# Nicholasli1995/SNVC

Measured on AMD Instinct MI355X. Metric: stereo-pairs/sec (cost-volume build + 3D CNN fwd), higher is better.
Workload: dtype f32 (split f16x3 operands, fp32 accumulate)

## Files before the change

snvc_amd/csrc/conv3d_f16.hip:

```cpp
#include <type_traits>

#include "common.hpp"
#include "elementwise_internal.hpp"
#include "snvc_fused.h"
#include "snvc_dedup.h"

namespace snvc {
namespace {

typedef _Float16 h8 __attribute__((ext_vector_type(8)));
typedef float f32x16 __attribute__((ext_vector_type(16)));
typedef float f32x4 __attribute__((ext_vector_type(4)));

__device__ const unsigned g_zero16h[4] __attribute__((aligned(16))) = {0u, 0u, 0u, 0u};

struct F16Args {
    const _Float16 *x;
    const _Float16 *wp;
    const float *scale, *bias;
    const _Float16 *res;
    _Float16 *y;
    float *y_f32;
    const _Float16 *x_lo, *res_lo;
    _Float16 *y_lo;
    const float *head;
    float *y_head;
    float head_mul;
    float res_mul;
    int *overflow;
    const _Float16 *tail_w;
    float *t_out;
    float tail_mul;
    int64_t t_bs;
    const float *res_f32;
    double *stats;
    const float *x_mul;
    int CGin;
    int Cout;
    int Din, Hin, Win;
    int Dout, Hout, Wout;
    int nd, nh, nw;
    int osd, osh, osw, offd, offh, offw;
    int pad_d, pad_h, pad_w;
    int isd, ish, iod, ioh;
    int tiles_d, tiles_h, tiles_w;
    int nchunks, flags;
    int N, cls_mode;
    int64_t cls_wstride;
    int64_t x_bs, y_bs, r_bs, yf_bs;
};

template <class I>
__host__ __device__ __forceinline__ I il_index(int mode, I oc, I C, I H, I pitch, I lp, I cls0, I h, I x) {
    const I cls = mode ? oc % 3 : oc / C, co = mode ? oc / 3 : oc % C, groups = (C + 7) / 8;
    return ((((cls0 + cls) * groups + (co >> 3)) * H + h) * pitch + lp + x) * 8 + (co & 7);
}

struct F16IlArgs : F16Args {
    float *y_il;
    int64_t il_bs;
    int il_mode, il_C, il_pitch, il_lp, il_cls0;
};

struct F16SrcArgs : F16Args {
    const float *gi;
    const float *p_il;
    const float *v_scale, *v_bias;
    int64_t gi_bs;
    int v_pitch, v_lp, v_q, v_m0, v_off, v_off2, v_flags;
};
constexpr int SRC_DEDUP = 1 << 30;

__host__ __device__ __forceinline__ bool wedge_tile_pure(int D, int W, int q, int m0, int off, int d0, int w0) {
    return d0 >= 2 && d0 + 3 <= D - 3 && w0 + 32 < W - 1 && q * (w0 + 32) - (d0 - 1) - m0 + off < 0;
}
__host__ __device__ __forceinline__ bool wedge_tile_duplicate(int D, int W, int q, int m0, int off, int d0, int w0) {
    return wedge_tile_pure(D, W, q, m0, off, d0, w0) && wedge_tile_pure(D, W, q, m0, off, d0 - 4, w0);
}


template <int KD_, int KH_, int KW_, int STRIDE_, int DIL_, int MI_, int TD_, int TH_, int KCG_, int MODE_, bool DB_, int OCC_,
          int DILW_ = DIL_, int PL_ = 1, bool DYN_ = false>
struct F16Cfg {
    static constexpr bool DYN = DYN_;
    static constexpr int PL = PL_;
    static constexpr bool SPLIT = PL_ >= 2, SERIAL = PL_ == 3;
    static constexpr int RES_PL = PL_ == 2 ? 2 : 1;
    static constexpr int PASSES = SERIAL ? 2 : 1;
    static constexpr int PF = DYN_ ? 2 : (SPLIT ? 3 : 6);
    static constexpr int KD = KD_, KH = KH_, KW = KW_, STRIDE = STRIDE_, DIL = DIL_, DILW = DILW_, MI = MI_, TD = TD_, TH = TH_;
    static constexpr int KCG = KCG_, MODE = MODE_, OCC = OCC_;
    static constexpr bool DB = DB_;
    static constexpr int IN_D = (TD - 1) * STRIDE + (KD - 1) * DIL + 1;
    static constexpr int IN_H = (TH - 1) * STRIDE + (KH - 1) * DIL + 1;
    static constexpr int IN_W = 31 * STRIDE + (KW - 1) * DILW + 1;
    static constexpr int VOX = IN_D * IN_H * IN_W;
    static constexpr int GB = VOX * 16;
    static constexpr int ITEMS = RES_PL * KCG * VOX;
    static constexpr int PLANE_BYTES = KCG * GB;
    static constexpr int NIT = (ITEMS + 255) / 256;
    static constexpr int IMG_BYTES = NIT * 256 * 16;
    static constexpr int LDS_BYTES = IMG_BYTES * (DB ? 2 : 1);
    static constexpr int NB = TD * TH / 4;
    static constexpr bool UNROLL_D = KD <= 3;
    static constexpr int SEGS = UNROLL_D ? 1 : KD;
    static constexpr int TSEG = UNROLL_D ? KD * KH * KW : KH * KW;
    static constexpr int NPS = (TSEG + 1) / 2;
    static constexpr int NS = MODE == 0 ? TSEG * (KCG / 2) : NPS * KCG;
    static constexpr int STEPS = SEGS * NS;
    static constexpr int SEG_BYTES = DIL * IN_H * IN_W * 16;
    static_assert(TD * TH % 4 == 0, "rows split over 4 waves");
    static_assert(MODE == 1 || KCG % 2 == 0, "MODE 0 pairs channel groups");
    static_assert(NIT <= 32, "validity mask is one register");
    static_assert((TD * TH / 4) * 4 == TD * TH, "whole rows per wave");
    static constexpr int tapoff(int t) {
        const int kd = UNROLL_D ? t / (KH * KW) : 0, kh = (t / KW) % KH, kw = t % KW;
        return ((kd * DIL) * IN_H + kh * DIL) * IN_W + kw * DILW;
    }
};

__host__ __device__ constexpr int f16_row_channel(int i) { return 16 * ((i >> 2) & 1) + 4 * (i >> 3) + (i & 3); }

__device__ __forceinline__ int xcd_remap16(int b, int n) {
    const int q = n >> 3, r = n & 7, xcd = b & 7, k = b >> 3;
    const int base = xcd < r ? xcd * (q + 1) : r * (q + 1) + (xcd - r) * q;
    return base + k;
}

template <class Cfg, int EPI>
__global__ void __launch_bounds__(256, Cfg::OCC)
conv3d_f16_kernel(const F16Args a_) {
    F16Args a = a_;
    int cls = blockIdx.z / a.N;
    int tile_raw = blockIdx.x, tiles_launch = a.tiles_d * a.tiles_h * a.tiles_w;
    if (a.cls_mode == 1) {
        tiles_launch *= 2;
        tile_raw = xcd_remap16(blockIdx.x, tiles_launch);
        cls = (cls << 1) | (tile_raw & 1);
        tile_raw >>= 1;
        a.offd = (cls >> 2) & 1; a.offh = (cls >> 1) & 1; a.offw = cls & 1;
        a.wp += cls * a.cls_wstride;
    } else if (a.cls_mode == 2) {
        const int pd = (cls >> 1) & 1, ph = cls & 1;
        a.offd = a.iod = pd; a.offh = a.ioh = ph;
        a.nd = (a.Dout - pd + 1) / 2; a.nh = (a.Hout - ph + 1) / 2;
    }
    constexpr int S = Cfg::STRIDE, MI = Cfg::MI, TD = Cfg::TD, TH = Cfg::TH, NB = Cfg::NB, KCG = Cfg::KCG;
    constexpr int IN_H = Cfg::IN_H, IN_W = Cfg::IN_W, VOX = Cfg::VOX, GB = Cfg::GB, NIT = Cfg::NIT, ITEMS = Cfg::ITEMS;
    constexpr int PF = Cfg::PF, PL = Cfg::PL;
    constexpr bool SPLIT = Cfg::SPLIT, SERIAL = Cfg::SERIAL;
    extern __shared__ __attribute__((aligned(16))) char lds[];

    const int tid = threadIdx.x, lane = tid & 63, wave = tid >> 6, half = lane >> 5;
    const int ntiles = a.tiles_d * a.tiles_h * a.tiles_w;
    const int t = a.cls_mode == 1 ? tile_raw : xcd_remap16(blockIdx.x, ntiles);
    const int tw = t % a.tiles_w, th = (t / a.tiles_w) % a.tiles_h, td = t / (a.tiles_w * a.tiles_h);
    const int cb = blockIdx.y;
    const int64_t n = blockIdx.z % a.N;
    const int od0 = td * TD, oh0 = th * TH, ow0 = tw * 32;
    if (od0 >= a.nd || oh0 >= a.nh) return;
    const int id0 = od0 * S - a.pad_d, ih0 = oh0 * S - a.pad_h, iw0 = ow0 * S - a.pad_w;

    f32x16 acc[NB][MI];
#pragma unroll
    for (int nb = 0; nb < NB; ++nb)
#pragma unroll
        for (int m = 0; m < MI; ++m)
#pragma unroll
            for (int r = 0; r < 16; ++r) acc[nb][m][r] = 0.0f;

    const int in_hw = a.Hin * a.Win, in_dhw = in_hw * a.Din;
    unsigned off[NIT];
    unsigned vmask = 0, gmask = 0, pmask = 0;
#pragma unroll
    for (int it = 0; it < NIT; ++it) {
        const int i = it * 256 + tid;
        const int pg = i / VOX, r = i - pg * VOX;
        const int plane = pg / KCG, g = pg - plane * KCG;
        gmask |= (unsigned)(g & 1) << it;
        pmask |= (unsigned)(plane & 1) << it;
        const int dd = r / (IN_H * IN_W), r2 = r - dd * (IN_H * IN_W);
        const int hh = r2 / IN_W, ww = r2 - hh * IN_W;
        const int gd = (id0 + dd) * a.isd + a.iod, gh = (ih0 + hh) * a.ish + a.ioh, gw = iw0 + ww;
        const bool ok = i < ITEMS && (unsigned)gd < (unsigned)a.Din && (unsigned)gh < (unsigned)a.Hin &&
                        (unsigned)gw < (unsigned)a.Win;
        off[it] = ok ? (unsigned)(g * in_dhw + gd * in_hw + gh * a.Win + gw) : 0u;
        vmask |= (ok ? 1u : 0u) << it;
    }
    static_assert(KCG <= 2, "gmask holds one bit per piece");
    const _Float16 *xn = a.x + n * a.x_bs, *xn_lo = SPLIT ? a.x_lo + n * a.x_bs : nullptr;
    const int wbase = tid & ~63;
    auto issue = [&](int pass, int buf) {
        const int chunk = SERIAL ? pass >> 1 : pass;
        const bool lo_pass = SERIAL && (pass & 1);
        const int64_t coff = (int64_t)chunk * KCG * in_dhw * 8;
        const int cg_left = a.CGin - chunk * KCG;
        char *const ibuf = lds + buf * Cfg::IMG_BYTES;
#pragma unroll
        for (int it = 0; it < NIT; ++it) {
            const int i = it * 256 + tid;
            const bool ok = ((vmask >> it) & 1u) && (KCG == 1 || (int)((gmask >> it) & 1u) < cg_left);
            const _Float16 *xc = (((PL == 2 && ((pmask >> it) & 1u)) || lo_pass) ? xn_lo : xn) + coff;
            const void *src = ok ? static_cast<const void *>(xc + (size_t)off[it] * 8) : static_cast<const void *>(g_zero16h);
            if (ITEMS % 256 == 0 || i < ITEMS)
                __builtin_amdgcn_global_load_lds(static_cast<const float *>(src),
                                                 reinterpret_cast<float *>(ibuf + (it * 256 + wbase) * 16), 16, 0, 0);
        }
    };

    const int lanebase = (lane & 31) * S * 16;
    int rowoff[NB];
#pragma unroll
    for (int nb = 0; nb < NB; ++nb) {
        const int row = wave * NB + nb;
        rowoff[nb] = ((row / TH) * S * IN_H + (row % TH) * S) * IN_W * 16;
    }
    constexpr int D_SAME = Cfg::DILW;
    constexpr int D_ROW = Cfg::DIL * IN_W - (Cfg::KW - 1) * Cfg::DILW;
    constexpr int D_SLICE = Cfg::DIL * IN_H * IN_W - (Cfg::KH - 1) * Cfg::DIL * IN_W - (Cfg::KW - 1) * Cfg::DILW;
    const int b_grp = lanebase + half * GB;
    const int b_same = lanebase + half * D_SAME * 16;
    const int b_row = lanebase + half * D_ROW * 16;
    const int b_slice = lanebase + half * D_SLICE * 16;
    const int b_none = lanebase;

    constexpr int MA = MI * (SPLIT ? 2 : 1);
    int dyn_np = 0, dyn_toff[4] = {0, 0, 0, 0}, dyn_base[4] = {0, 0, 0, 0};
    if constexpr (Cfg::DYN) {
        const int nw = 1 + (cls & 1), nh = 1 + ((cls >> 1) & 1), ndp = 1 + ((cls >> 2) & 1);
        const int T = nw * nh * ndp;
        dyn_np = T > 1 ? T / 2 : 1;
// ... 882 lines not shown
        const bool ok = i < ITEMS && (unsigned)gh < (unsigned)a.Hin && (unsigned)gw < (unsigned)a.Win;
        off[it] = ok ? (unsigned)(gh * a.Win + gw) : 0u;
        vmask |= (ok ? 1u : 0u) << it;
    }
    const _Float16 *xn = a.x + n * a.x_bs, *xn_lo = a.x_lo + n * a.x_bs;
    const int wbase = tid & ~63;
    auto issue = [&](int chunk, int buf) {
        const int64_t coff = (int64_t)chunk * in_hw * 8;
        char *const ibuf = lds + buf * Cfg::IMG_BYTES;
#pragma unroll
        for (int it = 0; it < NIT; ++it) {
            const _Float16 *xc = (((pmask >> it) & 1u) ? xn_lo : xn) + coff;
            const void *src = ((vmask >> it) & 1u) ? static_cast<const void *>(xc + (size_t)off[it] * 8) : static_cast<const void *>(g_zero16h);
            __builtin_amdgcn_global_load_lds(static_cast<const float *>(src), reinterpret_cast<float *>(ibuf + (it * 256 + wbase) * 16), 16, 0, 0);
        }
    };
    int qoff[NQ];
#pragma unroll
    for (int q = 0; q < NQ; ++q) {
        int tp = 4 * q + kb;
        tp = tp < Cfg::TAPS ? tp : Cfg::TAPS - 1;
        qoff[q] = ((tp / Cfg::KW) * IN_W + tp % Cfg::KW + col) * 16;
    }
    int rowoff[NB];
#pragma unroll
    for (int nb = 0; nb < NB; ++nb) rowoff[nb] = (wave * NB + nb) * IN_W * 16;
    const int64_t steps_total = (int64_t)a.nchunks * NQ;
    const h8 *wq = reinterpret_cast<const h8 *>(a.wp) + ((int64_t)cb * steps_total * 4) * 64 + lane;
    h8 q_[PF][4];
#pragma unroll
    for (int i = 0; i < PF; ++i) {
#pragma unroll
        for (int m = 0; m < 4; ++m) q_[i][m] = wq[m * 64];
        wq += 4 * 64;
    }

    const unsigned lds_base = (unsigned)(uintptr_t)(__attribute__((address_space(3))) char *)lds;
    issue(0, 0);
    __syncthreads();
    for (int chunk = 0; chunk < a.nchunks; ++chunk) {
        const unsigned img = lds_base + (unsigned)((chunk & 1) * Cfg::IMG_BYTES);
        const bool more = chunk + 1 < a.nchunks;
        h8 bfr[2][8];
        auto load_b = [&](int buf, int hs) {
#pragma unroll
            for (int rr = 0; rr < 2; ++rr) {
                const unsigned addr = img + (unsigned)(qoff[hs >> 1] + rowoff[2 * (hs & 1) + rr]);
                lds_read_b128_to<0>(bfr[buf][rr * 4 + 0], addr);
                lds_read_b128_to<Cfg::PLANE_BYTES>(bfr[buf][rr * 4 + 1], addr);
                lds_read_b128_to<256>(bfr[buf][rr * 4 + 2], addr);
                lds_read_b128_to<Cfg::PLANE_BYTES + 256>(bfr[buf][rr * 4 + 3], addr);
            }
        };
        load_b(0, 0);
        h8 af[4];
#pragma unroll
        for (int hs = 0; hs < 2 * NQ; ++hs) {
            const int cur = hs & 1, nx = cur ^ 1;
            if ((hs & 1) == 0) {
                if (hs == 2 * Cfg::FILL_STEP) {
#pragma unroll
                    for (int i = 0; i < PF; ++i) asm volatile("" ::"v"(q_[i][0]), "v"(q_[i][1]), "v"(q_[i][2]), "v"(q_[i][3]));
                    if (more) issue(chunk + 1, (chunk + 1) & 1);
                }
#pragma unroll
                for (int m = 0; m < 4; ++m) af[m] = q_[0][m];
#pragma unroll
                for (int i = 0; i + 1 < PF; ++i)
#pragma unroll
                    for (int m = 0; m < 4; ++m) q_[i][m] = q_[i + 1][m];
#pragma unroll
                for (int m = 0; m < 4; ++m) q_[PF - 1][m] = wq[m * 64];
                wq += 4 * 64;
            }
            if (hs + 1 < 2 * NQ) {
                load_b(nx, hs + 1);
                wait_lgkm_for<8>(bfr[cur]);
            } else {
                wait_lgkm_for<0>(bfr[cur]);
            }
            __builtin_amdgcn_sched_barrier(0);
#pragma unroll
            for (int term = 0; term < 3; ++term)
#pragma unroll
                for (int rr = 0; rr < 2; ++rr)
#pragma unroll
                    for (int ph = 0; ph < 2; ++ph)
#pragma unroll
                        for (int h = 0; h < 2; ++h) {
                            const h8 aw = term == 0 ? af[2 * h + 1] : af[2 * h];
                            const h8 bx = bfr[cur][rr * 4 + ph * 2 + (term == 1 ? 1 : 0)];
                            acc[2 * (hs & 1) + rr][ph][h] =
                                __builtin_amdgcn_mfma_f32_16x16x32_f16(aw, bx, acc[2 * (hs & 1) + rr][ph][h], 0, 0, 0);
                        }
            __builtin_amdgcn_sched_barrier(0);
        }
        __syncthreads();
    }

    const int64_t out_hw = (int64_t)a.Hout * a.Wout;
    const bool relu = (a.flags & SNVC_EPI_RELU) != 0;
    const int c0 = cb * 32 + 8 * kb;
    const float xm = a.x_mul ? a.head_mul / a.x_mul[0] : a.head_mul;
    float sc[8], bi[8];
#pragma unroll
    for (int e = 0; e < 8; ++e) {
        sc[e] = (a.scale ? a.scale[c0 + e] : 1.0f) * xm;
        bi[e] = a.scale ? a.bias[c0 + e] : 0.0f;
    }
    float *yn = a.y_f32 + n * a.yf_bs + (int64_t)c0 * out_hw;
#pragma unroll
    for (int nb = 0; nb < NB; ++nb) {
        const int phh = oh0 + wave * NB + nb;
#pragma unroll
        for (int ph = 0; ph < 2; ++ph) {
            const int pw = ow0 + 16 * ph + col;
            if (phh < a.nh && pw < a.nw) {
                float *yp = yn + (int64_t)phh * a.Wout + pw;
                float v8[8];
#pragma unroll
                for (int e = 0; e < 8; ++e) {
                    float v = __builtin_fmaf(acc[nb][ph][e >> 2][e & 3], sc[e], bi[e]);
                    if (relu) v = __builtin_fmaxf(v, 0.0f);
                    yp[e * out_hw] = v;
                    v8[e] = v;
                }
                if constexpr (IL == 1) {
                    float *il = a.y_il + n * a.il_bs;
                    if (a.il_mode == 0) {
                        float *dst = il + il_index<int>(0, c0, a.il_C, a.Hout, a.il_pitch, a.il_lp, a.il_cls0, phh, pw);
                        *reinterpret_cast<f32x4q *>(dst) = f32x4q{v8[0], v8[1], v8[2], v8[3]};
                        *reinterpret_cast<f32x4q *>(dst + 4) = f32x4q{v8[4], v8[5], v8[6], v8[7]};
                    } else {
#pragma unroll
                        for (int e = 0; e < 8; ++e) il[il_index<int>(1, c0 + e, a.il_C, a.Hout, a.il_pitch, a.il_lp, a.il_cls0, phh, pw)] = v8[e];
                    }
                }
            }
        }
    }
}

struct X3S2Cfg {
    static constexpr int TD = 2, TH = 4, NB = 2, IN_D = 5, IN_H = 9, IN_W = 65, VOX = IN_D * IN_H * IN_W;
    static constexpr int THREADS = 512, NIT = (VOX + THREADS - 1) / THREADS, SLOT_BYTES = NIT * THREADS * 16, LDS_BYTES = 3 * SLOT_BYTES;
    static constexpr int NQ = 7;
};

template <int N>
__device__ __forceinline__ void wait_lgkm_for4(h8 (&b)[4]) {
    asm volatile("s_waitcnt lgkmcnt(%4)" : "+v"(b[0]), "+v"(b[1]), "+v"(b[2]), "+v"(b[3]) : "n"(N) : "memory");
}

__global__ void __launch_bounds__(512, 1)
conv3d_x3s2q_kernel(const F16Args a, const int total_jobs) {
    using Cfg = X3S2Cfg;
    constexpr int NB = Cfg::NB, TH = Cfg::TH, IN_H = Cfg::IN_H, IN_W = Cfg::IN_W, VOX = Cfg::VOX, NIT = Cfg::NIT, NQ = Cfg::NQ;
    extern __shared__ __attribute__((aligned(16))) char lds[];
    const int tid = threadIdx.x, lane = tid & 63, wave = (tid >> 6) & 3, chalf = tid >> 8, kb = lane >> 4, col = lane & 15;
    const int ntiles = a.tiles_d * a.tiles_h * a.tiles_w, cblocks = a.Cout >> 6;
    const int in_hw = a.Hin * a.Win, in_dhw = in_hw * a.Din;
    const int wbase = tid & ~63;

    struct Job { int od0, oh0, ow0, cb; int64_t n; };
    auto decode = [&](int b) {
        const int j = xcd_remap16(b, total_jobs);
        const int cb = j % cblocks, r = j / cblocks, t = r % ntiles;
        Job jb;
        jb.n = r / ntiles; jb.cb = cb;
        const int tw = t % a.tiles_w, th = (t / a.tiles_w) % a.tiles_h, td = t / (a.tiles_w * a.tiles_h);
        jb.od0 = td * Cfg::TD; jb.oh0 = th * TH; jb.ow0 = tw * 32;
        return jb;
    };
    unsigned off[NIT];
    unsigned vmask = 0;
    auto geometry = [&](const Job &jb) {
        const int id0 = 2 * jb.od0 - a.pad_d, ih0 = 2 * jb.oh0 - a.pad_h, iw0 = 2 * jb.ow0 - a.pad_w;
        vmask = 0;
        int tid_ = tid;
        asm volatile("" : "+v"(tid_));
#pragma unroll
        for (int it = 0; it < NIT; ++it) {
            const int i = it * 512 + tid_;
            const int dd = i / (IN_H * IN_W), r2 = i - dd * (IN_H * IN_W);
            const int hh = r2 / IN_W, pp = r2 - hh * IN_W;
            const int blk = pp >> 5, rr_ = pp & 31;
            const int ww = pp == 64 ? 64 : (rr_ < 16 ? 2 * (16 * blk + rr_) : 2 * (16 * blk + rr_ - 16) + 1);
            const int gd = id0 + dd, gh = ih0 + hh, gw = iw0 + ww;
            const bool ok = i < VOX && (unsigned)gd < (unsigned)a.Din && (unsigned)gh < (unsigned)a.Hin && (unsigned)gw < (unsigned)a.Win;
            off[it] = ok ? (unsigned)(gd * in_hw + gh * a.Win + gw) : 0u;
            vmask |= (ok ? 1u : 0u) << it;
        }
    };
    auto issue = [&](int64_t n, int chunk, bool lo_plane, int slot) {
        const _Float16 *xc = (lo_plane ? a.x_lo : a.x) + n * a.x_bs + (int64_t)chunk * in_dhw * 8;
        char *const ibuf = lds + slot * Cfg::SLOT_BYTES;
#pragma unroll
        for (int it = 0; it < NIT; ++it) {
            const void *src = ((vmask >> it) & 1u) ? static_cast<const void *>(xc + (size_t)off[it] * 8) : static_cast<const void *>(g_zero16h);
            __builtin_amdgcn_global_load_lds(static_cast<const float *>(src), reinterpret_cast<float *>(ibuf + (it * 512 + wbase) * 16), 16, 0, 0);
        }
    };
    int qoff[NQ];
#pragma unroll
    for (int q = 0; q < NQ; ++q) {
        int tp = 4 * q + kb;
        tp = tp < 27 ? tp : 26;
        const int kd = tp / 9, kh = (tp / 3) % 3, kw = tp % 3;
        const int pos = kw == 0 ? col : (kw == 1 ? 16 + col : (col == 15 ? 32 : col + 1));
        qoff[q] = ((kd * IN_H + kh) * IN_W + pos) * 16;
    }
    int rowoff[NB];
#pragma unroll
    for (int nb = 0; nb < NB; ++nb) {
        const int row = wave * NB + nb;
        rowoff[nb] = ((2 * (row / TH)) * IN_H + 2 * (row % TH)) * IN_W * 16;
    }
    const h8 *const wall = reinterpret_cast<const h8 *>(a.wp);
    const int64_t wchunk = (int64_t)NQ * 8 * 64;

    int b = blockIdx.x;
    Job cur = decode(b);
    geometry(cur);
    h8 WH[NQ][2], WL[NQ][2];
    {
        const h8 *wc = wall + (int64_t)cur.cb * a.nchunks * wchunk;
#pragma unroll
        for (int q = 0; q < NQ; ++q)
#pragma unroll
            for (int h = 0; h < 2; ++h) {
                WH[q][h] = wc[(q * 8 + (2 * chalf + h) * 2) * 64 + lane];
                WL[q][h] = wc[(q * 8 + (2 * chalf + h) * 2 + 1) * 64 + lane];
            }
    }
    f32x4q acc[NB][2][2];
#pragma unroll
    for (int nb = 0; nb < NB; ++nb)
#pragma unroll
        for (int ph = 0; ph < 2; ++ph)
#pragma unroll
            for (int h = 0; h < 2; ++h) acc[nb][ph][h] = f32x4q{0.0f, 0.0f, 0.0f, 0.0f};

    const unsigned lds_base = (unsigned)(uintptr_t)(__attribute__((address_space(3))) char *)lds;
    int s_hi = 0, s_sp = 2;
    issue(cur.n, 0, false, 0);
    issue(cur.n, 0, true, 1);
    __syncthreads();
    const int gstride = gridDim.x;
    constexpr float kHalfMax = 65504.0f;
    const bool has_aff = a.scale != nullptr;
    float vmax = 0.0f;
    int chunk = 0;
    while (true) {
        const bool last_chunk = chunk + 1 == a.nchunks;
        const bool next_job = last_chunk && b + gstride < total_jobs;
        const bool more = !last_chunk || next_job;
        Job nxt = cur;
        if (next_job) {
            nxt = decode(b + gstride);
            geometry(nxt);
        }
        const int nchunk = last_chunk ? 0 : chunk + 1;
        if (more) issue(nxt.n, nchunk, false, s_sp);
        h8 bfr[2][4];
        auto load_b = [&](int buf, unsigned img, int q) {
#pragma unroll
            for (int rr = 0; rr < 2; ++rr) {
                const unsigned addr = img + (unsigned)(qoff[q] + rowoff[rr]);
                lds_read_b128_to<0>(bfr[buf][rr * 2 + 0], addr);
                lds_read_b128_to<512>(bfr[buf][rr * 2 + 1], addr);
            }
        };
        {
            const unsigned img = lds_base + (unsigned)Cfg::SLOT_BYTES;
            load_b(0, img, 0);
#pragma unroll
            for (int q = 0; q < NQ; ++q) {
                const int cb_ = q & 1, nx = cb_ ^ 1;
                if (q + 1 < NQ) {
                    load_b(nx, img, q + 1);
                    wait_lgkm_for4<4>(bfr[cb_]);
                } else {
                    wait_lgkm_for4<0>(bfr[cb_]);
                }
                __builtin_amdgcn_sched_barrier(0);
#pragma unroll
                for (int rr = 0; rr < 2; ++rr)
#pragma unroll
                    for (int ph = 0; ph < 2; ++ph)
#pragma unroll
                        for (int h = 0; h < 2; ++h)
                            acc[rr][ph][h] = __builtin_amdgcn_mfma_f32_16x16x32_f16(WH[q][h], bfr[cb_][rr * 2 + ph], acc[rr][ph][h], 0, 0, 0);
                __builtin_amdgcn_sched_barrier(0);
            }
        }
        asm volatile("s_waitcnt lgkmcnt(0)\n\ts_barrier" ::: "memory");
        if (more) issue(nxt.n, nchunk, true, 1);
        {
            const h8 *wn = wall + ((int64_t)nxt.cb * a.nchunks + nchunk) * wchunk;
            const unsigned img = lds_base + (unsigned)(s_hi * Cfg::SLOT_BYTES);
            load_b(0, img, 0);
#pragma unroll
            for (int q = 0; q < NQ; ++q) {
                const int cb_ = q & 1, nx = cb_ ^ 1;
                if (q + 1 < NQ) {
                    load_b(nx, img, q + 1);
                    wait_lgkm_for4<4>(bfr[cb_]);
                } else {
                    wait_lgkm_for4<0>(bfr[cb_]);
                }
                __builtin_amdgcn_sched_barrier(0);
#pragma unroll
                for (int term = 0; term < 2; ++term)
#pragma unroll
                    for (int rr = 0; rr < 2; ++rr)
#pragma unroll
                        for (int ph = 0; ph < 2; ++ph)
#pragma unroll
                            for (int h = 0; h < 2; ++h)
                                acc[rr][ph][h] = __builtin_amdgcn_mfma_f32_16x16x32_f16(term == 0 ? WL[q][h] : WH[q][h], bfr[cb_][rr * 2 + ph],
                                                                                        acc[rr][ph][h], 0, 0, 0);
                __builtin_amdgcn_sched_barrier(0);
                if (more) {
#pragma unroll
                    for (int h = 0; h < 2; ++h) {
                        WH[q][h] = wn[(q * 8 + (2 * chalf + h) * 2) * 64 + lane];
                        WL[q][h] = wn[(q * 8 + (2 * chalf + h) * 2 + 1) * 64 + lane];
                    }
                }
            }
        }
        __syncthreads();
        { const int o = s_hi; s_hi = s_sp; s_sp = o; }
        if (!last_chunk) { ++chunk; continue; }

        {
            const int out_hw = a.Hout * a.Wout;
            const int64_t out_dhw = (int64_t)out_hw * a.Dout;
            const bool relu = (a.flags & SNVC_EPI_RELU) != 0;
            const float lo_bound = relu ? 0.0f : -kHalfMax;
            {
                const int bb = chalf;
                const int c0 = cur.cb * 64 + bb * 32 + 8 * kb;
// ... 269 lines not shown
                    o[e] = (_Float16)v;
                    if constexpr (SPLIT) ol[e] = (_Float16)(v - (float)o[e]);
                }
                if (ok) {
                    *reinterpret_cast<h8 *>(yn + sp * 8) = o;
                    if constexpr (SPLIT) *reinterpret_cast<h8 *>(yn_lo + sp * 8) = ol;
                }
            }
        }
    }
    if constexpr (SPLIT) {
        if (vmax >= kHalfMax && a.overflow) atomicOr(a.overflow, 1);
    }
}

__global__ void pack_q16s_weights_kernel(const float *__restrict__ w, _Float16 *__restrict__ out, int Cout, int Cin, int K3, int NSEG, int NT,
                                         int NQ, int nchunks, int NH, int NPL, int PASSES, float wmul, int64_t total) {
    const int64_t i = (int64_t)blockIdx.x * blockDim.x + threadIdx.x;
    if (i >= total) return;
    int64_t r = i;
    const int e = (int)(r % 8); r /= 8;
    const int lane = (int)(r % 64); r /= 64;
    const int pl = (int)(r % NPL); r /= NPL;
    const int h = (int)(r % NH); r /= NH;
    const int q = (int)(r % NQ); r /= NQ;
    const int kd = (int)(r % NSEG); r /= NSEG;
    r /= PASSES;
    const int chunk = (int)(r % nchunks); r /= nchunks;
    const int cb = (int)r;
    const int row = lane & 15, kb = lane >> 4;
    const int co = (cb * (NH / 2) + (h >> 1)) * 32 + 8 * (row >> 2) + 4 * (h & 1) + (row & 3);
    const int ci = chunk * 8 + e;
    const int tp = 4 * q + kb;
    float v = 0.0f;
    if (tp < NT && kd * NT + tp < K3 && co < Cout && ci < Cin) v = w[((int64_t)co * Cin + ci) * K3 + kd * NT + tp] * wmul;
    const _Float16 hi = (_Float16)v;
    out[i] = pl == 0 ? hi : (_Float16)(v - (float)hi);
}

struct PackArgs {
    const float *w;
    _Float16 *out;
    int Cout, Cin, K;
    int transposed, pd, ph, pw;
    int KD, KH, KW, KCG, MODE, MI, SEGS, TSEG, NPS, NS, unroll_d;
    int nchunks, cblocks;
    int PL;
    int PASSES;
    int dyn;
    float wmul;
    int64_t total;
};

__global__ void pack_f16_weights_kernel(const PackArgs p) {
    const int64_t i = (int64_t)blockIdx.x * blockDim.x + threadIdx.x;
    if (i >= p.total) return;
    int64_t r = i;
    const int e = (int)(r % 8); r /= 8;
    const int lane = (int)(r % 64); r /= 64;
    const int npl = p.PL >= 2 ? 2 : 1;
    const int pl = (int)(r % npl); r /= npl;
    const int m = (int)(r % p.MI); r /= p.MI;
    const int s = (int)(r % p.NS); r /= p.NS;
    const int seg = (int)(r % p.SEGS); r /= p.SEGS;
    r /= p.PASSES;
    const int chunk = (int)(r % p.nchunks); r /= p.nchunks;
    const int cb = (int)r;
    const int half = lane >> 5;
    const int co = (cb * p.MI + m) * 32 + f16_row_channel(lane & 31);
    int tap, g;
    if (p.dyn) { g = s % p.KCG; tap = 2 * (s / p.KCG) + half; }
    else if (p.MODE == 0) { tap = s / (p.KCG / 2); g = 2 * (s % (p.KCG / 2)) + half; }
    else { g = s / p.NPS; tap = 2 * (s % p.NPS) + half; }
    const int ci = (chunk * p.KCG + g) * 8 + e;
    float v = 0.0f;
    if (p.dyn) {
        const int nw = 1 + p.pw, nh = 1 + p.ph, ndp = 1 + p.pd;
        if (tap < nw * nh * ndp && co < p.Cout && ci < p.Cin) {
            const int b[3] = {tap / (nw * nh), (tap / nw) % nh, tap % nw}, par[3] = {p.pd, p.ph, p.pw};
            int k3[3];
            for (int d = 0; d < 3; ++d) k3[d] = par[d] == 0 ? 1 : (b[d] == 0 ? 2 : 0);
            v = p.w[((((int64_t)ci * p.Cout + co) * 3 + k3[0]) * 3 + k3[1]) * 3 + k3[2]];
        }
    } else if (tap < p.TSEG && co < p.Cout && ci < p.Cin) {
        const int kd = p.unroll_d ? tap / (p.KH * p.KW) : seg, kh = (tap / p.KW) % p.KH, kw = tap % p.KW;
        if (!p.transposed) {
            v = p.w[((((int64_t)co * p.Cin + ci) * p.K + kd) * p.K + kh) * p.K + kw];
        } else {
            const int par[3] = {p.pd, p.ph, p.pw}, b[3] = {kd, kh, kw};
            int k3[3];
            bool ok = true;
            for (int d = 0; d < 3; ++d) {
                if (par[d] == 0) { ok = ok && b[d] == 0; k3[d] = 1; }
                else k3[d] = b[d] == 0 ? 2 : 0;
            }
            if (ok) v = p.w[((((int64_t)ci * p.Cout + co) * 3 + k3[0]) * 3 + k3[1]) * 3 + k3[2]];
        }
    }
    if (p.PL >= 2) {
        v *= p.wmul;
        const _Float16 hi = (_Float16)v;
        p.out[i] = pl ? (_Float16)(v - (float)hi) : hi;
    } else {
        p.out[i] = (_Float16)v;
    }
}

using F16K1   = F16Cfg<1, 1, 1, 1, 1, 2, 4, 4, 2, 0, true, 2>;
using F16K3   = F16Cfg<3, 3, 3, 1, 1, 2, 4, 4, 2, 0, true, 2>;
using F16K3H  = F16Cfg<3, 3, 3, 1, 1, 1, 4, 4, 2, 0, true, 2>;
using F16K3S2 = F16Cfg<3, 3, 3, 2, 1, 2, 2, 4, 1, 1, false, 2>;
using F16K5   = F16Cfg<5, 5, 5, 1, 1, 2, 4, 4, 1, 1, true, 2>;
using F16K5D2 = F16Cfg<5, 5, 5, 1, 1, 2, 4, 4, 1, 1, false, 2, 2>;
using F16K7   = F16Cfg<7, 7, 7, 1, 1, 2, 4, 4, 1, 1, false, 2>;
using F16DC   = F16Cfg<2, 2, 2, 1, 1, 2, 4, 4, 2, 0, true, 2>;
using F16K1N   = F16Cfg<1, 1, 1, 1, 1, 1, 4, 4, 2, 0, true, 2>;
using F16K3S2N = F16Cfg<3, 3, 3, 2, 1, 1, 2, 4, 1, 1, false, 2>;
using F16K5N   = F16Cfg<5, 5, 5, 1, 1, 1, 4, 4, 1, 1, true, 2>;
using F16K5D2N = F16Cfg<5, 5, 5, 1, 1, 1, 4, 4, 1, 1, false, 2, 2>;
using F16K7N   = F16Cfg<7, 7, 7, 1, 1, 1, 4, 4, 1, 1, false, 2>;
using F16DCN   = F16Cfg<2, 2, 2, 1, 1, 1, 4, 4, 2, 0, true, 2>;

using F16K3X  = F16Cfg<3, 3, 3, 1, 1, 1, 4, 4, 1, 1, false, 2, 1, 2>;
using F16K3X2 = F16Cfg<3, 3, 3, 1, 1, 2, 4, 4, 1, 1, false, 2, 1, 2>;
using F16K3XS  = F16Cfg<3, 3, 3, 1, 1, 1, 4, 4, 1, 1, true, 3, 1, 3>;
using F16K3XT  = F16Cfg<3, 3, 3, 1, 1, 1, 2, 4, 1, 1, false, 4, 1, 2>;
using F16K3X2S = F16Cfg<3, 3, 3, 1, 1, 2, 4, 4, 1, 1, true, 2, 1, 3>;
using F16K3S2X = F16Cfg<3, 3, 3, 2, 1, 2, 2, 4, 1, 1, false, 2, 1, 3>;
using F16DCX  = F16Cfg<2, 2, 2, 1, 1, 2, 4, 4, 2, 1, false, 2, 1, 2, true>;
using F16K3S2XT = F16Cfg<3, 3, 3, 2, 1, 2, 1, 4, 1, 1, false, 3, 1, 3>;
using F16DCXT   = F16Cfg<2, 2, 2, 1, 1, 2, 2, 4, 2, 1, false, 3, 1, 2, true>;

using F16K1X   = F16Cfg<1, 1, 1, 1, 1, 1, 4, 4, 2, 0, true, 3, 1, 2>;
using F16K5X   = F16Cfg<5, 5, 5, 1, 1, 1, 4, 4, 1, 1, false, 3, 1, 3>;
using F16K5D2X = F16Cfg<5, 5, 5, 1, 1, 1, 4, 4, 1, 1, false, 2, 2, 3>;
using F16K7X   = F16Cfg<7, 7, 7, 1, 1, 1, 4, 4, 1, 1, false, 2, 1, 3>;
using F16DCXN  = F16Cfg<2, 2, 2, 1, 1, 1, 4, 4, 2, 1, false, 3, 1, 2, true>;

__global__ void pack_tail_weights_kernel(const float *__restrict__ w, _Float16 *__restrict__ out, int Cin, float wmul, int total) {
    const int i = blockIdx.x * blockDim.x + threadIdx.x;
    if (i >= total) return;
    int r = i;
    const int e = r % 8; r /= 8;
    const int lane = r % 64; r /= 64;
    const int pl = r % 2; r /= 2;
    const int j = r % 2; r /= 2;
    const int m = r;
    const int tap = lane & 31, c = 32 * m + 16 * (lane >> 5) + 8 * j + e;
    const float v = (tap < 27 && c < Cin) ? w[c * 27 + tap] * wmul : 0.0f;
    const _Float16 hi = (_Float16)v;
    out[i] = pl == 0 ? hi : (_Float16)(v - (float)hi);
}

__global__ void __launch_bounds__(256)
deconv_tail_gather_kernel(const float *__restrict__ t, const float *__restrict__ bias, const float *__restrict__ res, float *__restrict__ y,
                          int nd, int nh, int nw, int64_t t_bs, int64_t y_bs, int64_t r_bs) {
    const int OD = 4 * nd, OH = 4 * nh;
    const int64_t total = (int64_t)OD * OH * nw;
    const int64_t i = (int64_t)blockIdx.x * 256 + threadIdx.x;
    if (i >= total) return;
    const int j = (int)(i % nw);
    const int64_t r0 = i / nw;
    const int oh = (int)(r0 % OH), od = (int)(r0 / OH);
    const int64_t n = blockIdx.y;
    const int64_t cls_vox = (int64_t)nd * nh * nw, tap_stride = 8 * cls_vox;
    const float *tn = t + n * t_bs;
    const float b = bias ? bias[0] : 0.0f;
    float o0 = b, o1 = b, o2 = b, o3 = b;
    const int ad = od >> 1, ah = oh >> 1;
    const int ndd = (od & 1) ? 2 : 1, nhh = (oh & 1) ? 2 : 1;
    const bool last_w = j + 1 >= nw;
    for (int a_ = 0; a_ < ndd; ++a_) {
        const int kd = (od & 1) ? (a_ ? 0 : 2) : 1, id = ad + a_;
        if (id >= 2 * nd) continue;
        for (int b_ = 0; b_ < nhh; ++b_) {
            const int kh = (oh & 1) ? (b_ ? 0 : 2) : 1, ih = ah + b_;
            if (ih >= 2 * nh) continue;
            const int cdh = ((id & 1) << 2) | ((ih & 1) << 1);
            const int64_t base = ((int64_t)(id >> 1) * nh + (ih >> 1)) * nw + j;
            const float *t0 = tn + (int64_t)((kd * 3 + kh) * 3) * tap_stride + base;
            const float *c0 = t0 + (int64_t)cdh * cls_vox, *c1 = t0 + (int64_t)(cdh | 1) * cls_vox;
            o0 += c0[tap_stride];
            o1 += c0[2 * tap_stride] + c1[0];
            o2 += c1[tap_stride];
            o3 += c1[2 * tap_stride] + (last_w ? 0.0f : c0[1]);
        }
    }
    const int64_t sp = ((int64_t)od * OH + oh) * (4 * nw) + 4 * j;
    if (res) {
        const f32x4 rv = *reinterpret_cast<const f32x4 *>(res + n * r_bs + sp);
        o0 += rv[0]; o1 += rv[1]; o2 += rv[2]; o3 += rv[3];
    }
    *reinterpret_cast<f32x4 *>(y + n * y_bs + sp) = f32x4{o0, o1, o2, o3};
}

__global__ void __launch_bounds__(256)
split_scale_kernel(const float *__restrict__ x, int64_t n, unsigned *__restrict__ scratch, float *__restrict__ out) {
    float m = 0.0f;
    const int64_t stride = (int64_t)gridDim.x * 256 * 4;
    const int64_t n4 = n & ~(int64_t)3;
    auto amax4 = [](const f32x4 v) {
        return __builtin_fmaxf(__builtin_fmaxf(__builtin_fabsf(v[0]), __builtin_fabsf(v[1])), __builtin_fmaxf(__builtin_fabsf(v[2]), __builtin_fabsf(v[3])));
    };
    int64_t i = ((int64_t)blockIdx.x * 256 + threadIdx.x) * 4;
    for (; i + 3 * stride < n4; i += 4 * stride) {
        const f32x4 v0 = *reinterpret_cast<const f32x4 *>(x + i), v1 = *reinterpret_cast<const f32x4 *>(x + i + stride);
        const f32x4 v2 = *reinterpret_cast<const f32x4 *>(x + i + 2 * stride), v3 = *reinterpret_cast<const f32x4 *>(x + i + 3 * stride);
        m = __builtin_fmaxf(m, __builtin_fmaxf(__builtin_fmaxf(amax4(v0), amax4(v1)), __builtin_fmaxf(amax4(v2), amax4(v3))));
    }
    for (; i < n4; i += stride) m = __builtin_fmaxf(m, amax4(*reinterpret_cast<const f32x4 *>(x + i)));
    if (blockIdx.x == 0 && threadIdx.x < (int)(n - n4)) m = __builtin_fmaxf(m, __builtin_fabsf(x[n4 + threadIdx.x]));
#pragma unroll
    for (int o = 32; o > 0; o >>= 1) m = __builtin_fmaxf(m, __shfl_xor(m, o, 64));
    __shared__ float part[4];
    if ((threadIdx.x & 63) == 0) part[threadIdx.x >> 6] = m;
    __syncthreads();
    if (threadIdx.x == 0) {
        m = __builtin_fmaxf(__builtin_fmaxf(part[0], part[1]), __builtin_fmaxf(part[2], part[3]));
        atomicMax(scratch, __builtin_bit_cast(unsigned, m));
        __threadfence();
        if (atomicAdd(scratch + 1, 1u) == gridDim.x - 1) {
            const float amax = __builtin_bit_cast(float, atomicExch(scratch, 0u));
            atomicExch(scratch + 1, 0u);
            float e = floorf(log2f(16384.0f / amax));
            e = (e == e && __builtin_fabsf(e) < 3.0e38f) ? __builtin_fminf(__builtin_fmaxf(e, -24.0f), 40.0f) : 0.0f;
            out[0] = exp2f(e);
        }
    }
}

struct F16Geom {
    int classes;
    int64_t ntiles;
    int64_t jobs;
    int64_t stats_slots;
    dim3 grid;
};
using F16Launch = void (*)(const F16Args &, const F16Geom &, hipStream_t);

enum F16Call { TO_SRC_HEAD, TO_SRC, TO_TAIL, TO_F32, TO_HEAD, TO_C8, TO_PLANE, F16_CALLS };
enum F16Classes { CLS_ONE = 0, CLS_TRANSPOSED = 1, CLS_SUBGRID = 2 };
enum F16Grid { GRID_TILES, GRID_JOBS, GRID_PERSISTENT };

struct Q16Layout { int K3, NSEG, NQ, NH, NPL, PASSES; };

struct F16Form {
    PackArgs pack;
    Q16Layout q16;
    int MI, KCG;
    int chunk_frags;
    int pad_frags;
    int cls_mode, TD, TH, grid;
    bool split_res, stats;
    const char *unsupported;
    F16Launch launch[F16_CALLS];

    constexpr F16Form on(F16Call c, F16Launch l) const { F16Form f = *this; f.launch[c] = l; return f; }
};

template <class Cfg, int EPI>
void launch_f16(const F16Args &a, const F16Geom &g, hipStream_t st) {
    launch_lds<conv3d_f16_kernel<Cfg, EPI>>(g.grid, 256, Cfg::LDS_BYTES, st, a);
}
template <class Cfg>
void launch_q16s(const F16Args &a, const F16Geom &g, hipStream_t st) {
    launch_lds<conv3d_q16s_kernel<Cfg>>(g.grid, 256, Cfg::LDS_BYTES, st, a);
}
template <int EPI>
void launch_x3q(const F16Args &a, const F16Geom &g, hipStream_t st) {
    launch_lds<conv3d_x3q_kernel<EPI>>(g.grid, 256, X3QCfg::LDS_BYTES, st, a);
}
template <int EPI>
void launch_x3q_src(const F16Args &a, const F16Geom &g, hipStream_t st) {
    launch_lds<conv3d_x3q_kernel<EPI, 1>>(g.grid, 256, X3QCfg::LDS_BYTES, st, static_cast<const F16SrcArgs &>(a));
}
struct WedgeRange { int64_t dups; int td0, td1, ntw; };
WedgeRange wedge_ranges(int D, int W, int q, int m0, int off, int64_t *first_td, int64_t *last_td, int max_tw) {
    WedgeRange r{0, -1, -1, 0};
    const int tiles_d = (D + X3QCfg::TD - 1) / X3QCfg::TD, tiles_w = (W + 31) / 32;
    for (int tw = 0; tw < tiles_w; ++tw) {
        int first = -1, last = -1;
        for (int td = 0; td < tiles_d; ++td) {
            if (!wedge_tile_pure(D, W, q, m0, off, td * X3QCfg::TD, tw * 32)) continue;
            if (first < 0) first = td;
            last = td;
        }
        if (last == first) first = last = -1;
        if (tw < max_tw && first_td && last_td) { first_td[tw] = first; last_td[tw] = last; }
        if (first < 0) continue;
        r.dups += last - first;
        r.ntw = tw + 1;
        if (tw == 0) { r.td0 = first + 1; r.td1 = last; }
    }
    return r;
}
void launch_wedge_copy(const F16SrcArgs &a, hipStream_t st) {
    const WedgeRange r = wedge_ranges(a.Din, a.Win, a.v_q, a.v_m0, a.v_off, nullptr, nullptr, 0);
    if (r.dups == 0) return;
    WedgeCopyArgs w{a.y, a.y_lo, a.y_head, a.y_bs, a.Cout / 8, a.Dout, a.Hout, a.Wout, a.v_q, a.v_m0, a.v_off, r.td0, r.ntw};
    wedge_copy_kernel<<<dim3((unsigned)((r.td1 - r.td0 + 1) * r.ntw), (unsigned)a.tiles_h, (unsigned)a.N), 256, 0, st>>>(w);
}

void launch_x3s2q(const F16Args &a, const F16Geom &g, hipStream_t st) {
    int wg = device_cu_count();
    if (wg <= 0) wg = 256;
    if (g.jobs < wg) wg = g.jobs >= 8 ? (int)(g.jobs & ~(int64_t)7) : (int)g.jobs;
    launch_lds<conv3d_x3s2q_kernel>(dim3((unsigned)wg), X3S2Cfg::THREADS, X3S2Cfg::LDS_BYTES, st, a, (int)g.jobs);
}

template <class Cfg, int... EPI>
constexpr F16Form f16_form(int cls_mode, bool stats = false) {
    constexpr F16Call call_of[5] = {TO_C8, TO_PLANE, TO_F32, TO_HEAD, TO_TAIL};
    constexpr int npl = Cfg::PL >= 2 ? 2 : 1;
    F16Form f{};
    f.pack.KD = Cfg::KD; f.pack.KH = Cfg::KH; f.pack.KW = Cfg::KW; f.pack.KCG = Cfg::KCG; f.pack.MODE = Cfg::MODE; f.pack.MI = Cfg::MI;
    f.pack.SEGS = Cfg::SEGS; f.pack.TSEG = Cfg::TSEG; f.pack.NPS = Cfg::NPS; f.pack.NS = Cfg::NS; f.pack.unroll_d = Cfg::UNROLL_D ? 1 : 0;
    f.pack.PL = Cfg::PL; f.pack.PASSES = Cfg::PASSES; f.pack.dyn = Cfg::DYN ? 1 : 0;
    f.MI = Cfg::MI; f.KCG = Cfg::KCG; f.TD = Cfg::TD; f.TH = Cfg::TH;
    f.chunk_frags = Cfg::PASSES * Cfg::STEPS * Cfg::MI * npl;
    f.pad_frags = Cfg::PF * Cfg::MI * npl;
    f.cls_mode = cls_mode; f.grid = GRID_TILES; f.split_res = true; f.stats = stats;
    f.unsupported = Cfg::PL >= 2 ? "snvc_f16x3_conv3d_forward: no kernel" : "snvc_f16_conv3d_forward: no kernel";
    ((f.launch[call_of[EPI]] = launch_f16<Cfg, EPI>), ...);
    return f;
}

constexpr F16Form q16_form(Q16Layout q, int TD, int TH, int pad_steps, int cls_mode, int grid, bool split_res, bool stats, const char *unsupported) {
    F16Form f{};
    f.q16 = q; f.MI = q.NH / 2; f.KCG = 1; f.TD = TD; f.TH = TH;
    f.chunk_frags = q.PASSES * q.NSEG * q.NQ * q.NH * q.NPL;
    f.pad_frags = pad_steps * q.NH * q.NPL;
    f.cls_mode = cls_mode; f.grid = grid; f.split_res = split_res; f.stats = stats; f.unsupported = unsupported;
    return f;
}
template <class C>
constexpr F16Form q16s_form(F16Call c, const char *unsupported) {
    return q16_form({C::K3, C::KSEG, C::NQ, C::NH, C::SPLIT ? 2 : 1, C::PASSES}, C::TD, C::TH, C::PF, C::DILW == 2 ? CLS_SUBGRID : CLS_ONE, GRID_TILES, true,
                    false, unsupported).on(c, launch_q16s<C>);
}

constexpr const char *kQ16C8 = "snvc_f16_conv3d_forward: the 16x16x32 form writes C8 tensors";
constexpr F16Form FORM_K7QN   = q16s_form<Q16SCfg<7, 1, 1, 1>>(TO_C8, kQ16C8);
constexpr F16Form FORM_K5QN   = q16s_form<Q16SCfg<5, 1, 1, 1>>(TO_C8, kQ16C8);
constexpr F16Form FORM_K5D2QN = q16s_form<Q16SCfg<5, 2, 1, 1>>(TO_C8, kQ16C8);
constexpr F16Form FORM_K7Q    = q16s_form<Q16SCfg<7, 1, 1, 2>>(TO_C8, kQ16C8);
constexpr F16Form FORM_K5Q    = q16s_form<Q16SCfg<5, 1, 1, 2>>(TO_C8, kQ16C8);
constexpr F16Form FORM_K5D2Q  = q16s_form<Q16SCfg<5, 2, 1, 2>>(TO_C8, kQ16C8);
constexpr F16Form FORM_K1     = f16_form<F16K1, 0>(CLS_ONE);
constexpr F16Form FORM_K3     = f16_form<F16K3, 0>(CLS_ONE);
constexpr F16Form FORM_K3H    = f16_form<F16K3H, 1>(CLS_ONE);
constexpr F16Form FORM_K3S2   = f16_form<F16K3S2, 0>(CLS_ONE);
constexpr F16Form FORM_K5     = f16_form<F16K5, 0>(CLS_ONE);
constexpr F16Form FORM_K5D2   = f16_form<F16K5D2, 0>(CLS_SUBGRID);
constexpr F16Form FORM_K7     = f16_form<F16K7, 0>(CLS_ONE);
constexpr F16Form FORM_DC     = f16_form<F16DC, 0>(CLS_TRANSPOSED);
constexpr F16Form FORM_K1N    = f16_form<F16K1N, 0>(CLS_ONE);
constexpr F16Form FORM_K3N    = f16_form<F16K3H, 0>(CLS_ONE);
constexpr F16Form FORM_K3S2N  = f16_form<F16K3S2N, 0>(CLS_ONE);
constexpr F16Form FORM_K5N    = f16_form<F16K5N, 0>(CLS_ONE);
constexpr F16Form FORM_K5D2N  = f16_form<F16K5D2N, 0>(CLS_SUBGRID);
constexpr F16Form FORM_K7N    = f16_form<F16K7N, 0>(CLS_ONE);
constexpr F16Form FORM_DCN    = f16_form<F16DCN, 0>(CLS_TRANSPOSED);
constexpr F16Form FORM_K3X    = f16_form<F16K3X, 0, 3, 2>(CLS_ONE, true);
constexpr F16Form FORM_K3X2   = f16_form<F16K3X2, 0, 2>(CLS_ONE, true);
constexpr F16Form FORM_K3XS   = f16_form<F16K3XS, 0, 3, 2>(CLS_ONE, true);
constexpr F16Form FORM_K3X2S  = f16_form<F16K3X2S, 0, 2>(CLS_ONE, true);
constexpr F16Form FORM_K3XT   = f16_form<F16K3XT, 0, 3, 2>(CLS_ONE, true);
constexpr F16Form FORM_K3S2X  = f16_form<F16K3S2X, 0, 2>(CLS_ONE, true);
constexpr F16Form FORM_K3S2XT = f16_form<F16K3S2XT, 0, 2>(CLS_ONE, true);
constexpr F16Form FORM_DCX    = f16_form<F16DCX, 0, 2, 4>(CLS_TRANSPOSED, true);
constexpr F16Form FORM_DCXT   = f16_form<F16DCXT, 0, 2, 4>(CLS_TRANSPOSED, true);
constexpr F16Form FORM_DCXN   = f16_form<F16DCXN, 0, 2, 4>(CLS_TRANSPOSED, true);
constexpr F16Form FORM_K1X    = f16_form<F16K1X, 0, 2>(CLS_ONE);
constexpr F16Form FORM_K5X    = f16_form<F16K5X, 0, 2>(CLS_ONE);
constexpr F16Form FORM_K5D2X  = f16_form<F16K5D2X, 0, 2>(CLS_SUBGRID);
constexpr F16Form FORM_K7X    = f16_form<F16K7X, 0, 2>(CLS_ONE);
constexpr F16Form FORM_K3XH   = f16_form<F16K3X, 1>(CLS_ONE);
constexpr const char *kQ16Split = "snvc_f16x3_conv3d_forward: the 16x16x32 form writes a split C8 tensor, no side head";
constexpr F16Form FORM_K5XQ   = q16s_form<Q16SCfg<5, 1>>(TO_C8, kQ16Split);
constexpr F16Form FORM_K5D2XQ = q16s_form<Q16SCfg<5, 2>>(TO_C8, kQ16Split);
constexpr F16Form FORM_K7XQ   = q16s_form<Q16SCfg<7, 1>>(TO_C8, kQ16Split);
constexpr F16Form FORM_K3S2XQ =
    q16_form({27, 1, X3S2Cfg::NQ, 4, 2, 1}, X3S2Cfg::TD, X3S2Cfg::TH, X3S2Cfg::NQ, CLS_ONE, GRID_PERSISTENT, false, false,
             "snvc_f16x3_conv3d_forward: the stride-2 16x16x32 form writes a split C8 tensor, no residual / head")
        .on(TO_C8, launch_x3s2q);
constexpr F16Form FORM_K3XQ =
    q16_form({27, 1, X3QCfg::NQ, 2, 2, 1}, X3QCfg::TD, X3QCfg::TH, X3QCfg::PF, CLS_ONE, GRID_JOBS, false, true,
             "snvc_f16x3_conv3d_forward: the 16x16x32 form has no split residual, no side head beside a float32 result")
        .on(TO_SRC_HEAD, launch_x3q_src<3>).on(TO_SRC, launch_x3q_src<0>).on(TO_F32, launch_x3q<2>).on(TO_HEAD, launch_x3q<3>).on(TO_C8, launch_x3q<0>);

struct F16Plan {
    const F16Form *form;
    int nchunks, cblocks;
    int64_t block_halves;
    int64_t class_stride() const { return block_halves + (int64_t)form->pad_frags * 64 * 8; }
};

const F16Form *plain_form(int key, int Cout, int algo) {
    const bool narrow = Cout == 32;
    if (algo & SNVC_ALGO_X3_Q16) {
        const bool two = Cout % 64 == 0;
        if (key == 711) return two ? &FORM_K7Q : &FORM_K7QN;
        if (key == 512) return two ? &FORM_K5D2Q : &FORM_K5D2QN;
        if (key == 511) return two ? &FORM_K5Q : &FORM_K5QN;
    }
    switch (key) {
        case 111: return narrow ? &FORM_K1N : &FORM_K1;
        case 311: return narrow ? &FORM_K3N : &FORM_K3;
        case 321: return narrow ? &FORM_K3S2N : &FORM_K3S2;
        case 511: return narrow ? &FORM_K5N : &FORM_K5;
        case 512: return narrow ? &FORM_K5D2N : &FORM_K5D2;
        case 711: return narrow ? &FORM_K7N : &FORM_K7;
        default: return nullptr;
    }
}

const F16Form *split_form(int key, int Cout, int algo) {
    const bool q16 = algo & SNVC_ALGO_X3_Q16;
    switch (key) {
        case 111: return &FORM_K1X;
        case 321: return q16 ? &FORM_K3S2XQ : (algo & SNVC_ALGO_X3_SMALL) ? &FORM_K3S2XT : &FORM_K3S2X;
        case 511: return q16 ? &FORM_K5XQ : &FORM_K5X;
        case 512: return q16 ? &FORM_K5D2XQ : &FORM_K5D2X;
        case 711: return q16 ? &FORM_K7XQ : &FORM_K7X;
        case 311:
            if (q16) return &FORM_K3XQ;
            if (algo & SNVC_ALGO_X3_SMALL) return &FORM_K3XT;
            if (algo & SNVC_ALGO_X3_NARROW) return &FORM_K3X;
            if (algo & SNVC_ALGO_X3_SERIAL) return Cout == 32 ? &FORM_K3XS : &FORM_K3X2S;
            return Cout == 32 ? &FORM_K3X : &FORM_K3X2;
        default: return nullptr;
    }
}

int make_f16_plan(const snvc_conv3d_desc &d, F16Plan &p, bool split = false) {
#define SNVC_F16_WHO(msg) (split ? "snvc_f16x3_conv3d: " msg : "snvc_f16_conv3d: " msg)
    if (d.N < 0 || d.Cin <= 0 || d.Cout <= 0 || d.Din <= 0 || d.Hin <= 0 || d.Win <= 0)
        return fail(SNVC_ERR_INVALID_ARGUMENT, "snvc_f16_conv3d: sizes must be positive");
    if (d.Cin % 8 != 0) return fail(SNVC_ERR_UNSUPPORTED, "snvc_f16_conv3d: Cin must be a multiple of 8 (C8 layout)");
    if (!split && d.Cout != 1 && d.Cout % 32 != 0)
        return fail(SNVC_ERR_UNSUPPORTED, "snvc_f16_conv3d: Cout must be a multiple of 32, or 1 (fp32 plane output)");
    const F16Form *f;
    if (d.transposed) {
        if (d.ksize != 3 || d.stride != 2 || d.pad != 1 || d.dilation != 1 || (split && d.Cout % 32 != 0))
            return fail(SNVC_ERR_UNSUPPORTED, split ? "snvc_f16x3_conv3d: transposed layers: k3,s2,p1,op1 with Cout % 32 == 0"
                                                    : "snvc_f16_conv3d: transposed conv supports k3,s2,p1,op1 only");
        if (d.Dout != 2 * d.Din || d.Hout != 2 * d.Hin || d.Wout != 2 * d.Win)
            return fail(SNVC_ERR_INVALID_ARGUMENT, SNVC_F16_WHO("transposed output must be 2x the input"));
        if (d.Cout == 1) return fail(SNVC_ERR_UNSUPPORTED, "snvc_f16_conv3d: transposed conv to one channel");
        if (split) f = d.Cout % 64 == 0 ? ((d.algo & SNVC_ALGO_X3_SMALL) ? &FORM_DCXT : &FORM_DCX) : &FORM_DCXN;
        else f = d.Cout == 32 ? &FORM_DCN : &FORM_DC;
    } else {
        if (d.pad != d.dilation * (d.ksize - 1) / 2) return fail(SNVC_ERR_UNSUPPORTED, SNVC_F16_WHO("pad must equal dilation*(ksize-1)/2"));
        const int eff = d.dilation * (d.ksize - 1) + 1;
        if (d.Dout != (d.Din + 2 * d.pad - eff) / d.stride + 1 || d.Hout != (d.Hin + 2 * d.pad - eff) / d.stride + 1 ||
            d.Wout != (d.Win + 2 * d.pad - eff) / d.stride + 1)
            return fail(SNVC_ERR_INVALID_ARGUMENT, SNVC_F16_WHO("output size does not match the convolution arithmetic"));
        const int key = d.ksize * 100 + d.stride * 10 + d.dilation;
        if (d.Cout == 1) {
            if (key != 311) return fail(SNVC_ERR_UNSUPPORTED, SNVC_F16_WHO("one-channel output is built for k3/s1 only"));
// ... 33 lines not shown
        a.osd = a.osh = a.osw = 1;
        a.pad_d = a.pad_h = a.pad_w = d.pad;
    }
    a.tiles_d = ceil_div(a.nd, f.TD); a.tiles_h = ceil_div(a.nh, f.TH); a.tiles_w = ceil_div(a.nw, 32);
    F16Geom g{};
    g.classes = transposed ? 8 : (subgrid ? 4 : 1);
    g.ntiles = (int64_t)a.tiles_d * a.tiles_h * a.tiles_w;
    const int64_t gx = transposed ? 2 * g.ntiles : g.ntiles, gz = transposed ? 4 : g.classes;
    g.grid = dim3((unsigned)gx, (unsigned)p.cblocks, (unsigned)(d.N * gz));
    g.stats_slots = gz * gx * 4;
    if (f.grid == GRID_JOBS) {
        g.jobs = g.ntiles * p.cblocks;
        g.grid = dim3((unsigned)g.jobs, 1, (unsigned)d.N);
        g.stats_slots = g.ntiles * 4;
    } else if (f.grid == GRID_PERSISTENT) {
        g.jobs = g.ntiles * p.cblocks * d.N;
    }
    return g;
}

void pack_q16(const Q16Layout &q, const float *w, void *packed, int Cout, int Cin, float wmul, int64_t total, hipStream_t st) {
    pack_q16s_weights_kernel<<<(unsigned)ceil_div<int64_t>(total, 256), 256, 0, st>>>(w, reinterpret_cast<_Float16 *>(packed), Cout, Cin, q.K3, q.NSEG, 4 * q.NQ,
                                                                                    q.NQ, Cin / 8, q.NH, q.NPL, q.PASSES, wmul, total);
}

}
}

extern "C" {

static int64_t f16_packed_bytes(const snvc_conv3d_desc *d, bool split) {
    snvc::F16Plan p;
    if (!d || snvc::make_f16_plan(*d, p, split) != SNVC_OK) return -1;
    return 2 * p.class_stride() * (d->transposed ? 8 : 1);
}

int64_t snvc_f16_conv3d_packed_weight_bytes(const snvc_conv3d_desc *d) { return f16_packed_bytes(d, false); }
int64_t snvc_f16x3_conv3d_packed_weight_bytes(const snvc_conv3d_desc *d) { return f16_packed_bytes(d, true); }

static int f16_pack_common(const snvc_conv3d_desc *d, const float *weight, void *packed, bool split, float wmul, void *stream,
                           const char *who) {
    using namespace snvc;
    F16Plan p;
    if (!d) return fail(SNVC_ERR_INVALID_ARGUMENT, "snvc_f16_conv3d_pack_weights: null desc");
    int rc = make_f16_plan(*d, p, split);
    if (rc) return rc;
    if (!weight || !packed) return fail(SNVC_ERR_INVALID_ARGUMENT, "snvc_f16_conv3d_pack_weights: null pointer");
    const F16Form &f = *p.form;
    const int classes = d->transposed ? 8 : 1;
    if (hipMemsetAsync(packed, 0, (size_t)(2 * p.class_stride() * classes), as_stream(stream)) != hipSuccess)
        return fail(SNVC_ERR_HIP, "snvc_f16_conv3d_pack_weights: hipMemsetAsync failed");
    if (f.q16.NQ) {
        pack_q16(f.q16, weight, packed, d->Cout, d->Cin, wmul, p.block_halves, as_stream(stream));
        return check_launch(who);
    }
    for (int c = 0; c < classes; ++c) {
        PackArgs a = f.pack;
        a.w = weight;
        a.out = reinterpret_cast<_Float16 *>(packed) + c * p.class_stride();
        a.Cout = d->Cout; a.Cin = d->Cin; a.K = d->ksize;
        a.transposed = d->transposed; a.pd = (c >> 2) & 1; a.ph = (c >> 1) & 1; a.pw = c & 1;
        a.nchunks = p.nchunks; a.cblocks = p.cblocks; a.total = p.block_halves;
        a.wmul = wmul;
        if (a.dyn) {
            const int T = (1 + a.pd) * (1 + a.ph) * (1 + a.pw);
            a.NS = 2 * (T > 1 ? T / 2 : 1);
            a.total = (int64_t)p.cblocks * p.nchunks * a.NS * a.MI * 2 * 64 * 8;
        }
        pack_f16_weights_kernel<<<(unsigned)ceil_div<int64_t>(a.total, 256), 256, 0, as_stream(stream)>>>(a);
    }
    return check_launch(who);
}

int snvc_f16_conv3d_pack_weights(const snvc_conv3d_desc *d, const float *weight, void *packed, void *stream) {
    return f16_pack_common(d, weight, packed, false, 1.0f, stream, "snvc_f16_conv3d_pack_weights");
}

int snvc_f16x3_conv3d_pack_weights(const snvc_conv3d_desc *d, const float *weight, void *packed, float wmul, void *stream) {
    return f16_pack_common(d, weight, packed, true, wmul, stream, "snvc_f16x3_conv3d_pack_weights");
}

int snvc_f16_conv3d_forward(const snvc_conv3d_desc *d, const void *x, const void *packed_weight, const float *scale,
                            const float *bias, const void *residual, void *y, float *y_f32, void *stream) {
    using namespace snvc;
    F16Plan p;
    if (!d) return fail(SNVC_ERR_INVALID_ARGUMENT, "snvc_f16_conv3d_forward: null desc");
    int rc = make_f16_plan(*d, p);
    if (rc) return rc;
    if (d->N == 0) return SNVC_OK;
    const bool plane = d->Cout == 1;
    if (!x || !packed_weight || (plane ? !y_f32 : !y))
        return fail(SNVC_ERR_INVALID_ARGUMENT, "snvc_f16_conv3d_forward: null pointer");
    if ((scale == nullptr) != (bias == nullptr))
        return fail(SNVC_ERR_INVALID_ARGUMENT, "snvc_f16_conv3d_forward: scale and bias must both be given or both be NULL");
    const int resflags = d->flags & (SNVC_EPI_ADD_PRE | SNVC_EPI_ADD_POST);
    if (resflags && (!residual || plane))
        return fail(SNVC_ERR_INVALID_ARGUMENT, "snvc_f16_conv3d_forward: residual flag without a C8 residual");
    if (resflags == (SNVC_EPI_ADD_PRE | SNVC_EPI_ADD_POST))
        return fail(SNVC_ERR_INVALID_ARGUMENT, "snvc_f16_conv3d_forward: ADD_PRE and ADD_POST are exclusive");
    if (!plane && (d->flags & SNVC_EPI_SIGMOID))
        return fail(SNVC_ERR_UNSUPPORTED, "snvc_f16_conv3d_forward: Sigmoid is built for the one-channel fp32 output only");
    const int64_t in_sp = (int64_t)d->Din * d->Hin * d->Win, out_sp = (int64_t)d->Dout * d->Hout * d->Wout;
    if ((int64_t)(d->Cin / 8 + 2) * in_sp >= ((int64_t)1 << 31) || out_sp >= ((int64_t)1 << 31))
        return fail(SNVC_ERR_UNSUPPORTED, "snvc_f16_conv3d_forward: one sample must stay below 2^31 pieces");
    if ((reinterpret_cast<uintptr_t>(x) | reinterpret_cast<uintptr_t>(y) | reinterpret_cast<uintptr_t>(residual) |
         reinterpret_cast<uintptr_t>(packed_weight)) & 15)
        return fail(SNVC_ERR_INVALID_ARGUMENT, "snvc_f16_conv3d_forward: C8 tensors must be 16-byte aligned");
    if ((d->x_batch_stride | d->y_batch_stride | d->res_batch_stride) % 8)
        return fail(SNVC_ERR_INVALID_ARGUMENT, "snvc_f16_conv3d_forward: batch strides must be multiples of 8 elements");

    F16Args a{};
    a.x = reinterpret_cast<const _Float16 *>(x);
    a.wp = reinterpret_cast<const _Float16 *>(packed_weight);
    a.scale = scale; a.bias = bias;
    a.res = resflags ? reinterpret_cast<const _Float16 *>(residual) : nullptr;
    a.y = reinterpret_cast<_Float16 *>(y); a.y_f32 = y_f32;
    a.res_mul = 1.0f;
    a.CGin = d->Cin / 8;
    a.Cout = d->Cout;
    a.Din = d->Din; a.Hin = d->Hin; a.Win = d->Win;
    a.Dout = d->Dout; a.Hout = d->Hout; a.Wout = d->Wout;
    a.nchunks = p.nchunks; a.flags = d->flags;
    a.x_bs = d->x_batch_stride ? d->x_batch_stride : (int64_t)d->Cin * in_sp;
    a.y_bs = d->y_batch_stride ? d->y_batch_stride : (int64_t)d->Cout * out_sp;
    a.r_bs = d->res_batch_stride ? d->res_batch_stride : (int64_t)d->Cout * out_sp;
    a.yf_bs = out_sp;
    const F16Geom g = f16_geometry(*d, p, a);
    if (g.ntiles >= ((int64_t)1 << 30) || (int64_t)d->N * g.classes > 65535)
        return fail(SNVC_ERR_UNSUPPORTED, "snvc_f16_conv3d_forward: too many tiles or samples");
    const F16Launch launch = p.form->launch[plane ? TO_PLANE : TO_C8];
    if (!launch) return fail(SNVC_ERR_UNSUPPORTED, p.form->unsupported);
    launch(a, g, as_stream(stream));
    return check_launch("snvc_f16_conv3d_forward");
}

struct F16x3Call {
    const void *x_hi = nullptr, *x_lo = nullptr, *packed_weight = nullptr;
    const float *scale = nullptr, *bias = nullptr;
    const void *res_hi = nullptr, *res_lo = nullptr;
    const float *res_f32 = nullptr;
    void *y_hi = nullptr, *y_lo = nullptr;
    float *y_f32 = nullptr;
    const float *head = nullptr;
    float *y_head = nullptr;
    float head_mul = 0.0f, res_mul = 0.0f;
    int *overflow = nullptr;
    const void *tail_w = nullptr;
    float *t_out = nullptr;
    float tail_mul = 0.0f;
    double *stats = nullptr;
    int64_t *stats_slots = nullptr;
    const float *x_mul = nullptr;
    const snvc::F16SrcArgs *src = nullptr;
    void *stream = nullptr;
};

static int f16x3_forward(const snvc_conv3d_desc *d, const F16x3Call &c) {
    using namespace snvc;
    F16Plan p;
    if (!d) return fail(SNVC_ERR_INVALID_ARGUMENT, "snvc_f16x3_conv3d_forward: null desc");
    int rc = make_f16_plan(*d, p, true);
    if (rc) return rc;
    if (d->N == 0) return SNVC_OK;
    const F16Form &f = *p.form;
    const bool tail = c.tail_w != nullptr;
    if (tail && (!c.t_out || !f.launch[TO_TAIL] || p.cblocks != 1 || d->Cout != 32 * f.MI || (reinterpret_cast<uintptr_t>(c.tail_w) & 15)))
        return fail(SNVC_ERR_UNSUPPORTED, "snvc_f16x3_deconv3d_tail_forward: a transposed split layer whose 32 or 64 output channels sit in one block");
    const bool plane = d->Cout == 1;
    const bool to_f32 = c.y_f32 != nullptr;
    if (plane && !to_f32) return fail(SNVC_ERR_INVALID_ARGUMENT, "snvc_f16x3_conv3d_forward: a one-channel layer writes y_f32");
    if ((!c.src && (!c.x_hi || !c.x_lo)) || !c.packed_weight || (!tail && !to_f32 && (!c.y_hi || !c.y_lo)))
        return fail(SNVC_ERR_INVALID_ARGUMENT, "snvc_f16x3_conv3d_forward: null pointer");
    if ((c.scale == nullptr) != (c.bias == nullptr))
        return fail(SNVC_ERR_INVALID_ARGUMENT, "snvc_f16x3_conv3d_forward: scale and bias must both be given or both be NULL");
    const int flags = c.res_f32 ? (d->flags & ~SNVC_EPI_ADD_POST) : d->flags;
    const int resflags = flags & (SNVC_EPI_ADD_PRE | SNVC_EPI_ADD_POST);
    if (c.res_f32 && !plane && d->res_batch_stride && d->res_batch_stride != (d->y_batch_stride ? d->y_batch_stride : (int64_t)d->Cout * d->Dout * d->Hout * d->Wout))
        return fail(SNVC_ERR_INVALID_ARGUMENT, "snvc_f16x3_conv3d_forward: a float32 residual shares the result's batch stride");
    if ((resflags && (!c.res_hi || !c.res_lo)) || ((resflags || c.res_f32) && plane))
        return fail(SNVC_ERR_INVALID_ARGUMENT, "snvc_f16x3_conv3d_forward: residual flag without a split residual");
    if (resflags == (SNVC_EPI_ADD_PRE | SNVC_EPI_ADD_POST))
        return fail(SNVC_ERR_INVALID_ARGUMENT, "snvc_f16x3_conv3d_forward: ADD_PRE and ADD_POST are exclusive");
    if (d->flags & ~(SNVC_EPI_RELU | SNVC_EPI_ADD_PRE | SNVC_EPI_ADD_POST | (plane ? SNVC_EPI_SIGMOID : 0)))
        return fail(SNVC_ERR_UNSUPPORTED, "snvc_f16x3_conv3d_forward: RELU / ADD_PRE / ADD_POST only (SIGMOID with the one-channel output)");
    if ((c.head != nullptr) != (c.y_head != nullptr))
        return fail(SNVC_ERR_INVALID_ARGUMENT, "snvc_f16x3_conv3d_forward: head and y_head go together");
    if (c.head && (!f.launch[TO_HEAD] || d->Cout != 32 || to_f32))
        return fail(SNVC_ERR_UNSUPPORTED, "snvc_f16x3_conv3d_forward: the side head is built for 32-channel stride-1 layers with a split output");
    const int64_t in_sp = (int64_t)d->Din * d->Hin * d->Win, out_sp = (int64_t)d->Dout * d->Hout * d->Wout;
    if ((int64_t)(d->Cin / 8 + 2) * in_sp >= ((int64_t)1 << 31) || out_sp >= ((int64_t)1 << 31))
        return fail(SNVC_ERR_UNSUPPORTED, "snvc_f16x3_conv3d_forward: one sample must stay below 2^31 pieces");
    if ((reinterpret_cast<uintptr_t>(c.x_hi) | reinterpret_cast<uintptr_t>(c.x_lo) | reinterpret_cast<uintptr_t>(c.y_hi) |
         reinterpret_cast<uintptr_t>(c.y_lo) | reinterpret_cast<uintptr_t>(c.res_hi) | reinterpret_cast<uintptr_t>(c.res_lo) |
         reinterpret_cast<uintptr_t>(c.packed_weight) | reinterpret_cast<uintptr_t>(c.scale) | reinterpret_cast<uintptr_t>(c.bias) |
         reinterpret_cast<uintptr_t>(c.head)) & 15)
        return fail(SNVC_ERR_INVALID_ARGUMENT, "snvc_f16x3_conv3d_forward: C8 tensors and the per-channel vectors must be 16-byte aligned");
    if ((d->x_batch_stride | (c.res_f32 ? 0 : d->res_batch_stride)) % 8 || (!to_f32 && d->y_batch_stride % 8))
        return fail(SNVC_ERR_INVALID_ARGUMENT, "snvc_f16x3_conv3d_forward: batch strides must be multiples of 8 elements");
    F16SrcArgs b{};
    if (c.src) b = *c.src;
    F16Args &a = b;
    a = F16Args{};
    a.x = reinterpret_cast<const _Float16 *>(c.x_hi); a.x_lo = reinterpret_cast<const _Float16 *>(c.x_lo);
    a.wp = reinterpret_cast<const _Float16 *>(c.packed_weight);
    a.scale = c.scale; a.bias = c.bias;
    a.res = resflags ? reinterpret_cast<const _Float16 *>(c.res_hi) : nullptr;
    a.res_lo = resflags ? reinterpret_cast<const _Float16 *>(c.res_lo) : nullptr;
    a.y = reinterpret_cast<_Float16 *>(c.y_hi); a.y_lo = reinterpret_cast<_Float16 *>(c.y_lo); a.y_f32 = c.y_f32;
    a.head = c.head; a.y_head = c.y_head; a.head_mul = c.head_mul; a.res_mul = c.res_mul; a.overflow = c.overflow;
    a.res_f32 = c.res_f32;
    a.stats = c.stats;
    a.x_mul = to_f32 ? c.x_mul : nullptr;
    a.tail_w = reinterpret_cast<const _Float16 *>(c.tail_w); a.t_out = c.t_out; a.tail_mul = c.tail_mul;
    a.t_bs = (int64_t)27 * 8 * d->Din * d->Hin * d->Win;
    a.CGin = d->Cin / 8; a.Cout = d->Cout;
    a.Din = d->Din; a.Hin = d->Hin; a.Win = d->Win;
    a.Dout = d->Dout; a.Hout = d->Hout; a.Wout = d->Wout;
    a.nchunks = p.nchunks; a.flags = flags;
    a.x_bs = d->x_batch_stride ? d->x_batch_stride : 2 * (int64_t)d->Cin * in_sp;
    a.y_bs = d->y_batch_stride ? d->y_batch_stride : 2 * (int64_t)d->Cout * out_sp;
    a.r_bs = d->res_batch_stride ? d->res_batch_stride : 2 * (int64_t)d->Cout * out_sp;
    a.yf_bs = plane ? out_sp : (d->y_batch_stride ? d->y_batch_stride : (int64_t)d->Cout * out_sp);
    const F16Geom g = f16_geometry(*d, p, a);
    if (g.ntiles >= ((int64_t)1 << 30) || (int64_t)d->N * g.classes > 65535)
        return fail(SNVC_ERR_UNSUPPORTED, "snvc_f16x3_conv3d_forward: too many tiles or samples");
    hipStream_t st = as_stream(c.stream);
    if (c.stats_slots) {
        if (!(to_f32 && !plane && !tail && f.stats))
            return fail(SNVC_ERR_UNSUPPORTED, "snvc_f16x3_conv3d_forward_stats: this layer's kernel form has no statistics epilogue");
        *c.stats_slots = g.stats_slots;
        if (!c.stats) return fail(SNVC_ERR_INVALID_ARGUMENT, "snvc_f16x3_conv3d_forward_stats: null workspace");
        if (g.classes > 1) {
            const hipError_t e = hipMemsetAsync(c.stats, 0, (size_t)d->N * g.stats_slots * ((d->Cout + 31) / 32) * 64 * sizeof(double), st);
            if (e != hipSuccess) return fail(SNVC_ERR_HIP, "snvc_f16x3_conv3d_forward_stats: hipMemsetAsync failed");
        }
    }
    if (c.src && !f.launch[TO_SRC])
        return fail(SNVC_ERR_UNSUPPORTED, "snvc_fused_first_conv3d_forward: a 3x3x3 stride-1 layer on the 16x16x32 form (SNVC_ALGO_X3_Q16)");
    const F16Call call = tail ? TO_TAIL : plane ? TO_PLANE : to_f32 ? TO_F32 : c.head ? (c.src ? TO_SRC_HEAD : TO_HEAD) : (c.src ? TO_SRC : TO_C8);
    if (!f.launch[call] || (resflags && !f.split_res)) return fail(SNVC_ERR_UNSUPPORTED, f.unsupported);
    if (g.jobs >= ((int64_t)1 << 30)) return fail(SNVC_ERR_UNSUPPORTED, "snvc_f16x3_conv3d_forward: too many tiles");
    if (c.src && to_f32) return fail(SNVC_ERR_UNSUPPORTED, "snvc_fused_first_conv3d_forward: a split C8 output");
    if ((b.v_flags & SRC_DEDUP) && ((c.y_head && (d->Wout % 4 || (reinterpret_cast<uintptr_t>(c.y_head) & 15))) ||
                                    wedge_ranges(a.Din, a.Win, b.v_q, b.v_m0, b.v_off, nullptr, nullptr, 0).dups == 0))
        b.v_flags &= ~SRC_DEDUP;
    f.launch[call](b, g, st);
    if (b.v_flags & SRC_DEDUP) launch_wedge_copy(b, st);
    return check_launch("snvc_f16x3_conv3d_forward");
}

int snvc_f16x3_conv3d_forward(const snvc_conv3d_desc *d, const void *x_hi, const void *x_lo, const void *packed_weight,
                              const float *scale, const float *bias, const void *res_hi, const void *res_lo, void *y_hi,
                              void *y_lo, float *y_f32, const float *head, float *y_head, float head_mul, float res_mul,
                              int *overflow, void *stream) {
    F16x3Call c;
    c.x_hi = x_hi; c.x_lo = x_lo; c.packed_weight = packed_weight; c.scale = scale; c.bias = bias;
    c.res_hi = res_hi; c.res_lo = res_lo; c.y_hi = y_hi; c.y_lo = y_lo; c.y_f32 = y_f32;
    c.head = head; c.y_head = y_head; c.head_mul = head_mul; c.res_mul = res_mul; c.overflow = overflow; c.stream = stream;
    if (d && (d->flags & (SNVC_EPI_ADD_PRE | SNVC_EPI_ADD_POST)) == SNVC_EPI_ADD_POST && y_f32 && d->Cout != 1 && res_hi && !res_lo) {
        c.res_f32 = static_cast<const float *>(res_hi);
        c.res_hi = nullptr;
    }
    return f16x3_forward(d, c);
}

static int fused_first_forward(const snvc_conv3d_desc *d, const void *packed_weight, const float *scale, const float *bias, void *y_hi,
                               void *y_lo, const float *head, float *y_head, float head_mul, int *overflow, const float *gi,
                               int64_t pitch, int64_t lp, const float *p_il, const float *v_scale, const float *v_bias, int q, int m0,
                               int off, int off2, int v_flags, bool dedup, void *stream) {
    using namespace snvc;
    if (!d || !gi || !p_il || !v_scale || !v_bias) return fail(SNVC_ERR_INVALID_ARGUMENT, "snvc_fused_first_conv3d_forward: null pointer");
    if (d->transposed || d->ksize != 3 || d->stride != 1 || d->pad != 1 || d->dilation != 1 || d->Cin % 8 || d->Din < 1 || d->Hin < 1 || d->Win < 1 ||
        (q != 1 && q != 2) || (v_flags & ~SNVC_EPI_RELU))
        return fail(SNVC_ERR_UNSUPPORTED, "snvc_fused_first_conv3d_forward: a 3x3x3 / stride 1 / pad 1 layer, Cin % 8 == 0, q = 1 | 2");
    if ((reinterpret_cast<uintptr_t>(gi) | reinterpret_cast<uintptr_t>(p_il) | reinterpret_cast<uintptr_t>(v_scale) | reinterpret_cast<uintptr_t>(v_bias)) & 31)
        return fail(SNVC_ERR_INVALID_ARGUMENT, "snvc_fused_first_conv3d_forward: gi / p_il / v_scale / v_bias must be 32-byte aligned");
    const int64_t D = d->Din, H = d->Hin, W = d->Win, CG = d->Cin / 8;
    const int64_t lo_g = -(D - 1) - m0 + off, hi_g = (int64_t)q * (W - 2) - m0 + off;
    const int64_t lo_c = (int64_t)q * (W - 1) - (D - 1) - m0 + off2, hi_c = (int64_t)q * (W - 1) - m0 + off2;
    if (lp < 0 || pitch <= 0 || lp + lo_c < 0 || lp + hi_c >= pitch || (W > 1 && (lp + lo_g < 0 || lp + hi_g >= pitch)))
        return fail(SNVC_ERR_INVALID_ARGUMENT, "snvc_fused_first_conv3d_forward: pitch / lp do not cover the G indices of this shape");
    if (6 * CG * H * pitch * 32 >= ((int64_t)1 << 31) || 3 * CG * H * W * 32 >= ((int64_t)1 << 31))
        return fail(SNVC_ERR_UNSUPPORTED, "snvc_fused_first_conv3d_forward: one sample of gi / p_il must stay below 2 GiB");
    F16SrcArgs s{};
    s.gi = gi; s.p_il = p_il; s.v_scale = v_scale; s.v_bias = v_bias; s.gi_bs = 6 * CG * H * pitch * 8;
    s.v_pitch = (int)pitch; s.v_lp = (int)lp; s.v_q = q; s.v_m0 = m0; s.v_off = off; s.v_off2 = off2;
    s.v_flags = v_flags | (dedup ? SRC_DEDUP : 0);
    F16x3Call c;
    c.packed_weight = packed_weight; c.scale = scale; c.bias = bias; c.y_hi = y_hi; c.y_lo = y_lo;
    c.head = head; c.y_head = y_head; c.head_mul = head_mul; c.res_mul = 1.0f; c.overflow = overflow; c.src = &s; c.stream = stream;
    return f16x3_forward(d, c);
}

int snvc_fused_first_conv3d_forward(const snvc_conv3d_desc *d, const void *packed_weight, const float *scale, const float *bias, void *y_hi,
                                    void *y_lo, const float *head, float *y_head, float head_mul, int *overflow, const float *gi,
                                    int64_t pitch, int64_t lp, const float *p_il, const float *v_scale, const float *v_bias, int q, int m0,
                                    int off, int off2, int v_flags, void *stream) {
    return fused_first_forward(d, packed_weight, scale, bias, y_hi, y_lo, head, y_head, head_mul, overflow, gi, pitch, lp, p_il, v_scale, v_bias,
                               q, m0, off, off2, v_flags, false, stream);
}

int snvc_dedup_abi_version(void) { return 1; }

int snvc_dedup_fused_first_conv3d_forward(const snvc_conv3d_desc *d, const void *packed_weight, const float *scale, const float *bias,
                                          void *y_hi, void *y_lo, const float *head, float *y_head, float head_mul, int *overflow,
                                          const float *gi, int64_t pitch, int64_t lp, const float *p_il, const float *v_scale,
                                          const float *v_bias, int q, int m0, int off, int off2, int v_flags, void *stream) {
    return fused_first_forward(d, packed_weight, scale, bias, y_hi, y_lo, head, y_head, head_mul, overflow, gi, pitch, lp, p_il, v_scale, v_bias,
                               q, m0, off, off2, v_flags, true, stream);
}

int64_t snvc_dedup_fused_first_tiles(const snvc_conv3d_desc *d, int q, int m0, int off, int64_t *first_td, int64_t *last_td, int max_tw) {
    using namespace snvc;
    if (!d || d->Din < 1 || d->Win < 1 || (q != 1 && q != 2) || max_tw < 0 || (max_tw > 0 && (!first_td || !last_td))) {
        fail(SNVC_ERR_INVALID_ARGUMENT, "snvc_dedup_fused_first_tiles: a desc, q = 1 | 2, and max_tw entries to write");
        return -1;
    }
    for (int tw = 0; tw < max_tw; ++tw) first_td[tw] = last_td[tw] = -1;
    return wedge_ranges((int)d->Din, (int)d->Win, q, m0, off, first_td, last_td, max_tw).dups;
}

int64_t snvc_f16x3_conv3d_stats_workspace_bytes(const snvc_conv3d_desc *d) {
    using namespace snvc;
    F16Plan p;
    if (!d || d->N < 0 || make_f16_plan(*d, p, true)) return -1;
    const int64_t groups = (d->Cout + 31) / 32;
    F16Args a{};
    const int64_t slots = f16_geometry(*d, p, a).stats_slots;
    return (d->N * slots * groups * 64 + conv_stats_fold_scratch_doubles(d->N, (int)groups, slots) + d->N * (int64_t)d->Cout * 2) * (int64_t)sizeof(double);
}

int snvc_f16x3_conv3d_forward_f32(const snvc_conv3d_desc *d, const void *x_hi, const void *x_lo, const void *packed_weight,
                                  const float *scale, const float *bias, const float *x_mul, const float *res_f32, float *y_f32,
                                  float out_mul, void *stream) {
    using namespace snvc;
    if (!d || !y_f32) return fail(SNVC_ERR_INVALID_ARGUMENT, "snvc_f16x3_conv3d_forward_f32: null pointer");
    if (d->flags & (SNVC_EPI_ADD_PRE | SNVC_EPI_ADD_POST)) return fail(SNVC_ERR_INVALID_ARGUMENT, "snvc_f16x3_conv3d_forward_f32: the residual is res_f32 (added after the activation), no flag");
    F16x3Call c;
    c.x_hi = x_hi; c.x_lo = x_lo; c.packed_weight = packed_weight; c.scale = scale; c.bias = bias; c.x_mul = x_mul;
    c.res_f32 = res_f32; c.y_f32 = y_f32; c.head_mul = out_mul; c.res_mul = 1.0f; c.stream = stream;
    return f16x3_forward(d, c);
}

int snvc_f16x3_conv3d_forward_stats(const snvc_conv3d_desc *d, const void *x_hi, const void *x_lo, const void *packed_weight,
                                    const float *scale, const float *bias, const float *x_mul, float *y_f32, float head_mul, const float *gamma,
                                    const float *beta, float *bn_scale, float *bn_shift, float *mean, float *var, void *workspace,
                                    float eps, void *stream) {
    using namespace snvc;
    if (!d || !y_f32 || !bn_scale || !bn_shift || !workspace)
        return fail(SNVC_ERR_INVALID_ARGUMENT, "snvc_f16x3_conv3d_forward_stats: null pointer");
    if (d->N <= 0 || d->flags || d->Cout % 32) return fail(SNVC_ERR_UNSUPPORTED, "snvc_f16x3_conv3d_forward_stats: whole 32-channel groups, no epilogue flags");
    double *stats = static_cast<double *>(workspace);
    int64_t slots = 0;
    F16x3Call c;
    c.x_hi = x_hi; c.x_lo = x_lo; c.packed_weight = packed_weight; c.scale = scale; c.bias = bias; c.x_mul = x_mul;
    c.y_f32 = y_f32; c.head_mul = head_mul; c.res_mul = 1.0f; c.stats = stats; c.stats_slots = &slots; c.stream = stream;
    int rc = f16x3_forward(d, c);
    if (rc) return rc;
    const int groups = d->Cout / 32;
    double *scratch = stats + d->N * slots * groups * 64;
    double *partial = scratch + conv_stats_fold_scratch_doubles(d->N, groups, slots);
    launch_conv_stats_fold(stats, scratch, partial, d->N, d->Cout, groups, slots, as_stream(stream));
    rc = check_launch("snvc_f16x3_conv3d_forward_stats(fold)");
    if (rc) return rc;
    launch_norm_finalize(partial, gamma, beta, bn_scale, bn_shift, mean, var, d->N, d->Cout, (int64_t)d->Dout * d->Hout * d->Wout, 1, eps,
                         as_stream(stream));
    return check_launch("snvc_f16x3_conv3d_forward_stats(finalize)");
}

int snvc_f16x3_split_scale(const float *x, int64_t n, void *scratch8, float *out_mul, void *stream) {
    using namespace snvc;
    if (n < 0) return fail(SNVC_ERR_INVALID_ARGUMENT, "snvc_f16x3_split_scale: negative size");
    if (!out_mul || !scratch8 || (n > 0 && !x)) return fail(SNVC_ERR_INVALID_ARGUMENT, "snvc_f16x3_split_scale: null pointer");
    if (reinterpret_cast<uintptr_t>(x) & 15) return fail(SNVC_ERR_INVALID_ARGUMENT, "snvc_f16x3_split_scale: x must be 16-byte aligned");
    int blocks = (int)ceil_div<int64_t>(n > 0 ? n : 1, 256 * 4 * 16);
    blocks = blocks < 1 ? 1 : (blocks > 48 ? 48 : blocks);
    split_scale_kernel<<<blocks, 256, 0, as_stream(stream)>>>(x, n, reinterpret_cast<unsigned *>(scratch8), out_mul);
    return check_launch("snvc_f16x3_split_scale");
}

static int x2q_nq(int kh, int kw) { return (kh * kw + 3) / 4; }

int64_t snvc_f16x3_conv2d_packed_weight_bytes(int cout, int cin, int kh, int kw) {
    if (cout <= 0 || cin <= 0 || cout % 32 || cin % 8 || kh != 3 || (kw != 3 && kw != 7)) return -1;
    return 2 * ((int64_t)(cout / 32) * (cin / 8) * x2q_nq(kh, kw) + 2) * 4 * 64 * 8;
}

int snvc_f16x3_conv2d_pack_weights(const float *weight, int cout, int cin, int kh, int kw, void *packed, float wmul, void *stream) {
    using namespace snvc;
    const int64_t bytes = snvc_f16x3_conv2d_packed_weight_bytes(cout, cin, kh, kw);
    if (bytes < 0) return fail(SNVC_ERR_UNSUPPORTED, "snvc_f16x3_conv2d: 3x7 or 3x3 kernels, Cin % 8 == 0, Cout % 32 == 0");
    if (!weight || !packed) return fail(SNVC_ERR_INVALID_ARGUMENT, "snvc_f16x3_conv2d_pack_weights: null pointer");
    if (hipMemsetAsync(packed, 0, (size_t)bytes, as_stream(stream)) != hipSuccess)
        return fail(SNVC_ERR_HIP, "snvc_f16x3_conv2d_pack_weights: hipMemsetAsync failed");
    const int nq = x2q_nq(kh, kw);
    const int64_t total = (int64_t)(cout / 32) * (cin / 8) * nq * 4 * 64 * 8;
    pack_q16({kh * kw, 1, nq, 2, 2, 1}, weight, packed, cout, cin, wmul, total, as_stream(stream));
    return check_launch("snvc_f16x3_conv2d_pack_weights");
}

struct snvc_il_out {
    float *y_il;
    int64_t bs, pitch, lp, cls0, classes;
    int mode;
};

static int f16x3_conv2d_forward(const void *x_hi, const void *x_lo, const void *packed_weight, const float *scale, const float *bias,
                                float *y, int64_t N, int64_t Cin, int64_t Cout, int64_t H, int64_t W, int kh, int kw, float out_mul,
                                const float *x_mul_dev, int flags, void *stream, const snvc_il_out *il) {
    using namespace snvc;
    if (N < 0 || H <= 0 || W <= 0 || snvc_f16x3_conv2d_packed_weight_bytes((int)Cout, (int)Cin, kh, kw) < 0)
        return fail(SNVC_ERR_UNSUPPORTED, "snvc_f16x3_conv2d_forward: 3x7 or 3x3 kernels, Cin % 8 == 0, Cout % 32 == 0");
    if (N == 0) return SNVC_OK;
    if (!x_hi || !x_lo || !packed_weight || !y) return fail(SNVC_ERR_INVALID_ARGUMENT, "snvc_f16x3_conv2d_forward: null pointer");
    if ((scale == nullptr) != (bias == nullptr))
        return fail(SNVC_ERR_INVALID_ARGUMENT, "snvc_f16x3_conv2d_forward: scale and bias must both be given or both be NULL");
    if (flags & ~SNVC_EPI_RELU) return fail(SNVC_ERR_UNSUPPORTED, "snvc_f16x3_conv2d_forward: only SNVC_EPI_RELU");
    if ((reinterpret_cast<uintptr_t>(x_hi) | reinterpret_cast<uintptr_t>(x_lo) | reinterpret_cast<uintptr_t>(packed_weight)) & 15)
        return fail(SNVC_ERR_INVALID_ARGUMENT, "snvc_f16x3_conv2d_forward: C8 tensors must be 16-byte aligned");
    const int64_t hw = H * W;
    if ((Cin / 8 + 2) * hw >= ((int64_t)1 << 31) || N > 65535) return fail(SNVC_ERR_UNSUPPORTED, "snvc_f16x3_conv2d_forward: tensor too large");
    F16Args a{};
    a.x = reinterpret_cast<const _Float16 *>(x_hi); a.x_lo = reinterpret_cast<const _Float16 *>(x_lo);
    a.wp = reinterpret_cast<const _Float16 *>(packed_weight);
    a.scale = scale; a.bias = bias; a.y_f32 = y; a.head_mul = out_mul; a.x_mul = x_mul_dev;
    a.CGin = (int)(Cin / 8); a.Cout = (int)Cout; a.nchunks = (int)(Cin / 8); a.flags = flags;
    a.Din = a.Dout = 1; a.Hin = a.Hout = (int)H; a.Win = a.Wout = (int)W;
    a.nd = 1; a.nh = (int)H; a.nw = (int)W;
    a.pad_d = 0; a.pad_h = (kh - 1) / 2; a.pad_w = (kw - 1) / 2;
    a.tiles_d = 1; a.tiles_h = (int)ceil_div<int64_t>(H, 16); a.tiles_w = (int)ceil_div<int64_t>(W, 32);
    a.x_bs = 2 * Cin * hw; a.yf_bs = Cout * hw; a.N = (int)N;
    const int64_t jobs = (int64_t)a.tiles_h * a.tiles_w * (Cout / 32);
    if (jobs >= ((int64_t)1 << 30)) return fail(SNVC_ERR_UNSUPPORTED, "snvc_f16x3_conv2d_forward: too many tiles");
    const dim3 grid((unsigned)jobs, 1, (unsigned)N);
    hipStream_t st = as_stream(stream);
    if (il) {
        const int64_t C = Cout / 3, need = il->classes * ((C + 7) / 8) * H * il->pitch * 8;
        if (!il->y_il || Cout % 3 || (il->mode == 0 && C % 8) || il->lp < 0 || il->lp + W > il->pitch || il->cls0 < 0 || il->cls0 + 3 > il->classes ||
            need > il->bs || need >= ((int64_t)1 << 31) || (reinterpret_cast<uintptr_t>(il->y_il) & 31) || il->bs % 8)
            return fail(SNVC_ERR_INVALID_ARGUMENT, "snvc_fused: the interleaved output does not hold the layer's result");
        F16IlArgs b{};
        static_cast<F16Args &>(b) = a;
        b.y_il = il->y_il; b.il_bs = il->bs; b.il_mode = il->mode; b.il_C = (int)C; b.il_pitch = (int)il->pitch; b.il_lp = (int)il->lp;
        b.il_cls0 = (int)il->cls0;
        if (kw == 7) {
            using C7 = X2QCfg<3, 7>;
            launch_lds<conv2d_x3q_kernel<C7, 1>>(grid, 256, C7::LDS_BYTES, st, b);
        } else {
            using C3 = X2QCfg<3, 3>;
            launch_lds<conv2d_x3q_kernel<C3, 1>>(grid, 256, C3::LDS_BYTES, st, b);
        }
    } else if (kw == 7) {
        using C = X2QCfg<3, 7>;
        launch_lds<conv2d_x3q_kernel<C>>(grid, 256, C::LDS_BYTES, st, a);
    } else {
        using C = X2QCfg<3, 3>;
        launch_lds<conv2d_x3q_kernel<C>>(grid, 256, C::LDS_BYTES, st, a);
    }
    return check_launch("snvc_f16x3_conv2d_forward");
}

int snvc_f16x3_conv2d_forward(const void *x_hi, const void *x_lo, const void *packed_weight, const float *scale, const float *bias,
                              float *y, int64_t N, int64_t Cin, int64_t Cout, int64_t H, int64_t W, int kh, int kw, float out_mul,
                              const float *x_mul_dev, int flags, void *stream) {
    return f16x3_conv2d_forward(x_hi, x_lo, packed_weight, scale, bias, y, N, Cin, Cout, H, W, kh, kw, out_mul, x_mul_dev, flags, stream, nullptr);
}

static int sheared_prep_x3(const float *right, int64_t N, int64_t C, int64_t H, int64_t W, int q, int64_t WU, int off, int64_t WU2, int off2,
                           const void *packed_g, const void *packed_col, int64_t Cout3, float out_mul_g, float out_mul_col, void *rq_split,
                           void *rq2_split, void *scratch8, float *mul_dev, float *g, float *gcol, void *stream, float *gi, int64_t pitch,
                           int64_t lp) {
    using namespace snvc;
    const int64_t gi_bs = 6 * (C / 8) * H * pitch * 8;
    const snvc_il_out il_g{gi, gi_bs, pitch, lp, 0, 6, 0}, il_col{gi, gi_bs, pitch, lp, 3, 6, 0};
    if (!right || !packed_g || !packed_col || !rq_split || !rq2_split || !scratch8 || !mul_dev || !g || !gcol)
        return fail(SNVC_ERR_INVALID_ARGUMENT, "snvc_sheared_prep_x3: null pointer");
    if (N <= 0 || C % 8 || Cout3 % 32) return fail(SNVC_ERR_UNSUPPORTED, "snvc_sheared_prep_x3: C % 8 == 0, 3 * Cout % 32 == 0");
    int rc = snvc_f16x3_split_scale(right, N * C * H * W, scratch8, mul_dev, stream);
    if (rc) return rc;
    const int64_t G = C / 8;
    _Float16 *a = reinterpret_cast<_Float16 *>(rq_split), *b = reinterpret_cast<_Float16 *>(rq2_split);
    rc = snvc_sheared_upsample_split(right, a, a + G * H * WU * 8, mul_dev, N, C, H, W, q, WU, off, stream);
    if (rc) return rc;
    rc = f16x3_conv2d_forward(a, a + G * H * WU * 8, packed_g, nullptr, nullptr, g, N, C, Cout3, H, WU, 3, 7, out_mul_g, mul_dev, 0, stream,
                              gi ? &il_g : nullptr);
    if (rc) return rc;
    rc = snvc_sheared_upsample_split(right, b, b + G * H * WU2 * 8, mul_dev, N, C, H, W, q, WU2, off2, stream);
    if (rc) return rc;
    return f16x3_conv2d_forward(b, b + G * H * WU2 * 8, packed_col, nullptr, nullptr, gcol, N, C, Cout3, H, WU2, 3, 7, out_mul_col, mul_dev, 0,
                                stream, gi ? &il_col : nullptr);
}

int snvc_sheared_prep_x3(const float *right, int64_t N, int64_t C, int64_t H, int64_t W, int q, int64_t WU, int off, int64_t WU2, int off2,
                         const void *packed_g, const void *packed_col, int64_t Cout3, float out_mul_g, float out_mul_col, void *rq_split,
                         void *rq2_split, void *scratch8, float *mul_dev, float *g, float *gcol, void *stream) {
    return sheared_prep_x3(right, N, C, H, W, q, WU, off, WU2, off2, packed_g, packed_col, Cout3, out_mul_g, out_mul_col, rq_split, rq2_split,
                           scratch8, mul_dev, g, gcol, stream, nullptr, 0, 0);
}

int snvc_fused_sheared_prep_x3(const float *right, int64_t N, int64_t C, int64_t H, int64_t W, int q, int64_t WU, int off, int64_t WU2,
                               int off2, const void *packed_g, const void *packed_col, int64_t Cout3, float out_mul_g, float out_mul_col,
                               void *rq_split, void *rq2_split, void *scratch8, float *mul_dev, float *g, float *gcol, float *gi,
                               int64_t pitch, int64_t lp, void *stream) {
    if (!gi || Cout3 != 3 * C) return snvc::fail(SNVC_ERR_INVALID_ARGUMENT, "snvc_fused_sheared_prep_x3: gi is NULL or Cout3 != 3 * C");
    return sheared_prep_x3(right, N, C, H, W, q, WU, off, WU2, off2, packed_g, packed_col, Cout3, out_mul_g, out_mul_col, rq_split, rq2_split,
                           scratch8, mul_dev, g, gcol, stream, gi, pitch, lp);
}

int snvc_fused_abi_version(void) { return 1; }

int64_t snvc_fused_il_index(int mode, int64_t oc, int64_t C, int64_t H, int64_t pitch, int64_t lp, int64_t cls0, int64_t h, int64_t x) {
    if ((mode != 0 && mode != 1) || C <= 0 || oc < 0 || oc >= 3 * C || H <= 0 || h < 0 || h >= H || lp < 0 || x < 0 || lp + x >= pitch || cls0 < 0)
        return -1;
    return snvc::il_index<int64_t>(mode, oc, C, H, pitch, lp, cls0, h, x);
}

int snvc_fused_planes_from_f32(const float *x, int64_t N, int64_t C, int64_t H, int64_t W, const void *packed, int64_t cout, float out_mul,
                               float *y, float *p_il, void *ws_split, void *scratch8, float *mul_dev, void *stream) {
    using namespace snvc;
    if (!x || !packed || !y || !p_il || !ws_split || !scratch8 || !mul_dev)
        return fail(SNVC_ERR_INVALID_ARGUMENT, "snvc_fused_planes_from_f32: null pointer");
    if (N <= 0 || C % 8 || cout != 3 * C) return fail(SNVC_ERR_UNSUPPORTED, "snvc_fused_planes_from_f32: C % 8 == 0, cout == 3 * C");
    int rc = snvc_f16x3_split_scale(x, N * C * H * W, scratch8, mul_dev, stream);
    if (rc) return rc;
    _Float16 *a = reinterpret_cast<_Float16 *>(ws_split);
    rc = snvc_f16x3_from_ncdhw(x, a, a + C * H * W, N, C, H * W, 0, 0, 1.0f, mul_dev, stream);
    if (rc) return rc;
    const snvc_il_out il{p_il, 3 * (C / 8) * H * W * 8, W, 0, 0, 3, 1};
    return f16x3_conv2d_forward(a, a + C * H * W, packed, nullptr, nullptr, y, N, C, cout, H, W, 3, 3, out_mul, mul_dev, 0, stream, &il);
}

int snvc_f16x3_conv2d_from_f32(const float *x, int64_t N, int64_t C, int64_t H, int64_t W, int kh, int kw, int n_layers,
                               const void *const *packed, const int64_t *cout, const float *out_mul, float *const *y, void *ws_split,
                               void *scratch8, float *mul_dev, void *stream) {
    using namespace snvc;
    if (!x || !packed || !cout || !out_mul || !y || !ws_split || !scratch8 || !mul_dev || n_layers < 1 || n_layers > 8)
        return fail(SNVC_ERR_INVALID_ARGUMENT, "snvc_f16x3_conv2d_from_f32: null pointer or layer count outside 1..8");
    if (N <= 0 || C % 8) return fail(SNVC_ERR_UNSUPPORTED, "snvc_f16x3_conv2d_from_f32: C % 8 == 0");
    int rc = snvc_f16x3_split_scale(x, N * C * H * W, scratch8, mul_dev, stream);
    if (rc) return rc;
    _Float16 *a = reinterpret_cast<_Float16 *>(ws_split);
    rc = snvc_f16x3_from_ncdhw(x, a, a + C * H * W, N, C, H * W, 0, 0, 1.0f, mul_dev, stream);
    if (rc) return rc;
    for (int i = 0; i < n_layers; ++i) {
        rc = snvc_f16x3_conv2d_forward(a, a + C * H * W, packed[i], nullptr, nullptr, y[i], N, C, cout[i], H, W, kh, kw, out_mul[i], mul_dev, 0, stream);
        if (rc) return rc;
    }
    return SNVC_OK;
}

int64_t snvc_f16x3_tail_packed_weight_bytes(int cin) {
    return cin > 0 && cin % 32 == 0 ? (int64_t)(cin / 32) * 2 * 2 * 64 * 8 * 2 : -1;
}

int snvc_f16x3_tail_pack_weights(const float *weight, int cin, void *packed, float wmul, void *stream) {
    using namespace snvc;
    if (!weight || !packed || cin <= 0 || cin % 32 != 0)
        return fail(SNVC_ERR_INVALID_ARGUMENT, "snvc_f16x3_tail_pack_weights: weight [Cin][27] with Cin % 32 == 0");
    const int total = (cin / 32) * 2 * 2 * 64 * 8;
    pack_tail_weights_kernel<<<(unsigned)ceil_div(total, 256), 256, 0, as_stream(stream)>>>(weight, reinterpret_cast<_Float16 *>(packed), cin, wmul, total);
    return check_launch("snvc_f16x3_tail_pack_weights");
}

int snvc_f16x3_deconv3d_tail_forward(const snvc_conv3d_desc *d, const void *x_hi, const void *x_lo, const void *packed_weight,
                                     const float *scale, const float *bias, const void *res_hi, const void *res_lo, float res_mul,
                                     const void *tail_packed, float *t_out, float tail_mul, int *overflow, void *stream) {
    using namespace snvc;
    if (!tail_packed || !t_out) return fail(SNVC_ERR_INVALID_ARGUMENT, "snvc_f16x3_deconv3d_tail_forward: null pointer");
    F16x3Call c;
    c.x_hi = x_hi; c.x_lo = x_lo; c.packed_weight = packed_weight; c.scale = scale; c.bias = bias; c.res_hi = res_hi; c.res_lo = res_lo;
    c.head_mul = 1.0f; c.res_mul = res_mul; c.overflow = overflow; c.tail_w = tail_packed; c.t_out = t_out; c.tail_mul = tail_mul; c.stream = stream;
    return f16x3_forward(d, c);
}

int snvc_deconv_tail_gather(const float *t, const float *bias, const float *residual, float *y, int64_t n, int64_t nd, int64_t nh,
                            int64_t nw, void *stream) {
    using namespace snvc;
    if (n < 0 || nd <= 0 || nh <= 0 || nw <= 0) return fail(SNVC_ERR_INVALID_ARGUMENT, "snvc_deconv_tail_gather: sizes must be positive");
    if (n == 0) return SNVC_OK;
    if (!t || !y) return fail(SNVC_ERR_INVALID_ARGUMENT, "snvc_deconv_tail_gather: null pointer");
    if ((reinterpret_cast<uintptr_t>(y) | reinterpret_cast<uintptr_t>(residual)) & 15)
        return fail(SNVC_ERR_INVALID_ARGUMENT, "snvc_deconv_tail_gather: y / residual must be 16-byte aligned");
    const int64_t threads = 16 * nd * nh * nw, out_vox = 64 * nd * nh * nw;
    if (threads >= ((int64_t)1 << 31) * 255 || n > 65535 || 27 * 8 * nd * nh * nw >= ((int64_t)1 << 40))
        return fail(SNVC_ERR_UNSUPPORTED, "snvc_deconv_tail_gather: tensor too large");
    const dim3 grid((unsigned)ceil_div<int64_t>(threads, 256), (unsigned)n);
    deconv_tail_gather_kernel<<<grid, 256, 0, as_stream(stream)>>>(t, bias, residual, y, (int)nd, (int)nh, (int)nw, 27 * 8 * nd * nh * nw,
                                                                   out_vox, out_vox);
    return check_launch("snvc_deconv_tail_gather");
}

}
```

snvc_amd/models/stereo_volume.py:

```python
import dataclasses
import itertools
import warnings
import weakref

import torch
import torch.nn as nn

from ..extension.build_cost_volume import _BuildCostVolume, build_cost_volume
from .. import ops
from .._derived import derived, fresh, stamp
from .submodule import (_ROUTES, SCRATCH_ATTRS, WORKSPACE_ATTRS, X3_GROUP_NORM, ConvBNReLU3d, HipConv3d, SplitModePolicy, SplitOverflow,
                        SplitT, _FactoredFirstConvFn, _ShearedFirstConvBNFn, _ShearedFirstConvFn, _folded_bn,
                        _is_channel_head as _is_head_conv, _Plan, convbn_3d, folded_head_weights, hourglass, overflow_guard, plan_for,
                        sheared_geometry, sheared_kernels, x3_exponent, x3_norm_bound, EPI_RELU, SHEAR_CLASS_KDS)

_PREP_EPOCH = itertools.count(1)
_X3_KEY = {ops.Conv3dLayer: "", ops.Conv2dLayerX3: "_x3"}
_ASK = object()


@dataclasses.dataclass
class _Prep:
    plans: dict
    c: int
    weight: torch.Tensor
    st: dict = None
    scale: torch.Tensor = None
    bias: torch.Tensor = None
    split_prep: bool = False
    fuse: bool = False
    prep_ws: dict = None
    planes: torch.Tensor = None
    p_il: torch.Tensor = None


def _factored_plans(conv: nn.Module, c: int) -> dict:
    plans = conv.__dict__.get("_snvc_factored")
    if plans is None or not fresh(plans["stamp"], (conv.weight,)):
        w = conv.weight
        plans = conv.__dict__["_snvc_factored"] = {"stamp": stamp((w,)), "plan": _Plan(),
                                                   "right": ops.Conv3dLayer(w.detach()[:, c:].contiguous(), 3, 1, 1, 1, False)}
    return plans


def _mark(timing, name, which):
    if timing is not None and name in timing:
        timing[name][which].record()


def _run(gen):
    try:
        while True:
            next(gen)
    except StopIteration as done:
        return done.value


class GlobalStack(SplitModePolicy, nn.Module):
    def __init__(self, c=32, gn=False):
        super().__init__()
        self.conv1 = ConvBNReLU3d(convbn_3d(2 * c, c, 3, 1, 1, gn=gn), nn.ReLU(inplace=True))
        self.conv2 = ConvBNReLU3d(convbn_3d(c, c, 3, 1, 1, gn=gn), nn.ReLU(inplace=True))
        self.hg_conv3d = hourglass(c, gn=gn)
        self.classifier = HipConv3d(c, 1, kernel_size=1, padding=0, stride=1, bias=False)
        for m in self.modules():
            if isinstance(m, nn.Conv3d):
                nn.init.kaiming_normal_(m.weight, mode="fan_out", nonlinearity="relu")
            elif isinstance(m, nn.BatchNorm3d):
                nn.init.constant_(m.weight, 1)
                nn.init.constant_(m.bias, 0)

    def _buffer(self, name, shape, device, dtype=torch.float32):
        ws = self.__dict__.setdefault("_snvc_ws", {})
        key = (name, tuple(shape), device)
        buf = ws.get(key)
        if buf is None:
            for k in [k for k in ws if k[0] == name and k[2] == device]:
                del ws[k]
            buf = ws[key] = torch.empty(shape, dtype=dtype, device=device)
        return buf

    def _v1(self, shape, device):
        self.__dict__["_snvc_last_v1"] = "v1"
        return self._buffer("v1", shape, device)

    def _v1s(self, shape, device, last="v1s", lazy=None):
        def pair():
            return self._buffer("v1s", (shape[0], 2, shape[1] // 8) + tuple(shape[2:]) + (8,), device, torch.float16)
        if lazy is not None:
            self.__dict__.setdefault("_snvc_ws", {})[("v1s_lazy", (), None)] = lambda: lazy(pair())
            self.__dict__["_snvc_last_v1"] = "v1s_lazy"
            return None
        self.__dict__["_snvc_last_v1"] = last
        return pair()

    def last_first_layer(self) -> torch.Tensor:
        ws = self.__dict__.get("_snvc_ws", {})
        which = self.__dict__.get("_snvc_last_v1", "v1")
        if which == "v1s_lazy":
            return ops.from_split(ws[("v1s_lazy", (), None)](), self.__dict__["_snvc_x3"]["exp"]["v1"])
        for k, v in ws.items():
            if k[0] == which == "v1s":
                st = self.__dict__.get("_snvc_x3")
                return ops.from_split(v, st["exp"]["v1"] if st is not None else
                                      x3_exponent(x3_norm_bound(self.conv1[0][1], plan_for(self.conv1[0][0], "_x3", v.device))))
            if k[0] == which:
                return v
        raise RuntimeError("no first-layer result in the workspace")

    def release_workspace(self):
        for name in WORKSPACE_ATTRS:
            self.__dict__.pop(name, None)

    def train(self, mode: bool = True):
        if mode:
            self.release_workspace()
        return super().train(mode)

    def __getstate__(self):
        state = self.__dict__.copy()
        for name in SCRATCH_ATTRS:
            state.pop(name, None)
        return state

    arithmetic = "auto"
    stream_out = False
    fused_first = True
    dedup_wedge = True
    split_prep = True
    fused_tail = True

    def _x3_state(self, device):
        hg = self.hg_conv3d
        seqs = {"conv2": self.conv2[0], "h1": hg.conv1[0], "h2": hg.conv2, "h3": hg.conv3[0], "h4": hg.conv4[0], "h5": hg.conv5}
        c = self.conv2[0][0].out_channels
        if c != 32 or self.conv2[0][0].in_channels != 32 or not _is_head_conv(self.classifier, c):
            return None
        norms = [self.conv1[0][1]] + [sq[1] for sq in seqs.values()]
        for nm in norms:
            if not isinstance(nm, nn.BatchNorm3d) or nm.training or nm.running_mean is None:
                return None
        tensors = [t for sq in list(seqs.values()) + [hg.conv6] for t in (sq[0].weight, sq[1].weight, sq[1].bias, sq[1].running_mean, sq[1].running_var)]
        tensors.append(self.classifier.weight)
        tensors += [self.conv1[0][1].weight, self.conv1[0][1].bias, self.conv1[0][1].running_mean, self.conv1[0][1].running_var]
        st = self.__dict__.get("_snvc_x3")
        if st is not None and fresh(st["stamp"], tensors, (device,)):
            return st
        e = {k: x3_exponent(x3_norm_bound(sq[1], plan_for(sq[0], "_x3", device))) for k, sq in [("v1", self.conv1[0])] + list(seqs.items())}
        st = {"stamp": stamp(tensors, (device,)), "exp": e, "layers": {}, "affine": {}}
        geo = {"conv2": (1, False), "h1": (2, False), "h2": (1, False), "h3": (2, False), "h4": (1, False), "h5": (2, True)}
        for k, sq in seqs.items():
            w = sq[0].weight.detach().to(device)
            st["layers"][k] = ops.Conv3dLayerX3(w, 3, geo[k][0], 1, 1, geo[k][1])
            st["affine"][k] = _folded_bn(sq[1], plan_for(sq[0], "", device))
        w5 = hg.conv5[0].weight.detach().double().abs()
        sets = ([1], [0, 2])
        l1 = None
        for pd in range(2):
            for ph in range(2):
                for pw in range(2):
                    t = w5[:, :, sets[pd]][:, :, :, sets[ph]][:, :, :, :, sets[pw]].sum(dim=(0, 2, 3, 4))
                    l1 = t if l1 is None else torch.maximum(l1, t)
        sc5, bi5 = st["affine"]["h5"]
        hard = float(((sc5.double().abs() * l1.to(sc5.device) * (65504.0 / 2.0 ** st["exp"]["h4"]) + bi5.double().abs()).max()
                      + 65504.0 / 2.0 ** st["exp"]["h2"]).item())
        st["exp"]["post"] = min(x3_exponent(hard), st["exp"]["h2"])
        st["tail"] = st["tail_bias"] = None
        if isinstance(hg.conv6[1], nn.BatchNorm3d) and not hg.conv6[1].training and hg.conv6[0].in_channels % 32 == 0:
            wf, fb = folded_head_weights(hg.conv6[0], hg.conv6[1], self.classifier)
            st["tail"] = ops.TailWeightsX3(wf.float().to(device))
            st["tail_bias"] = fb.float().reshape(1).to(device)
        st["guard"] = overflow_guard(self, device)
        st["flag"] = st["guard"].flag
        self.__dict__["_snvc_x3"] = st
        return st

    @staticmethod
    def _x3_v1_affine(st, scale, bias):
        e1 = st["exp"]["v1"]
        return derived(st, "v1_affine", (scale, bias), lambda: ((scale * 2.0 ** e1).contiguous(), (bias * 2.0 ** e1).contiguous()))

    def _x3_select(self, device, arithmetic=None):
        mode = arithmetic or self.arithmetic
        if mode == "fp32" or torch.is_grad_enabled() or self.training or self.split_off:
            if mode == "x3":
                raise RuntimeError("arithmetic='x3' needs inference (no autograd, eval mode) and no earlier overflow")
            return None
        st = self._x3_state(device)
        if st is None:
            if mode == "x3":
                raise RuntimeError("arithmetic='x3': the stack does not qualify (32 channels, eval-mode BatchNorm3d everywhere)")
            return None
        return st if self.split_guard(device, mode) is not None else None

    def _tail_x3(self, st, v1s, timing=None, fused=None):
        L, A, E, flag = st["layers"], st["affine"], st["exp"], st["flag"]
        if fused is not None:
            (n, _, d, h, w), dev = fused[0], fused[1]
        else:
            n, dev = v1s.size(0), v1s.device
            d, h, w = v1s.shape[3:6]
        hg = self.hg_conv3d
        _mark(timing, "conv2", 0)
        v2_out = self._buffer("v2s", (n, 2, 4, d, h, w, 8), dev, torch.float16)
        if fused is not None:
            v2s, hv = L["conv2"].forward_fused_first(n=n, in_sp=(d, h, w), x_exp=E["v1"], scale=A["conv2"][0], bias=A["conv2"][1], flags=EPI_RELU,
                                                     out_exp=E["conv2"], head=self.classifier.weight, overflow=flag, out=v2_out,
                                                     dedup=bool(self.dedup_wedge), **fused[2])
            _ROUTES["fused_first_conv"] += 1
        else:
            v2s, hv = L["conv2"](v1s, E["v1"], *A["conv2"], flags=EPI_RELU, out_exp=E["conv2"], head=self.classifier.weight, overflow=flag,
                                 out=v2_out)
        _mark(timing, "conv2", 1)
        _ROUTES["side_head"] += 1
        o = L["h1"](v2s, E["conv2"], *A["h1"], flags=EPI_RELU, out_exp=E["h1"], overflow=flag)
        pre = L["h2"](o, E["h1"], *A["h2"], flags=EPI_RELU, out_exp=E["h2"], overflow=flag)
        o = L["h3"](pre, E["h2"], *A["h3"], flags=EPI_RELU, out_exp=E["h3"], overflow=flag)
        o = L["h4"](o, E["h3"], *A["h4"], flags=EPI_RELU, out_exp=E["h4"], overflow=flag)
        st["guard"].post()
        if st["tail"] is not None and self.fused_tail:
            t = L["h5"].forward_tail(o, E["h4"], *A["h5"], st["tail"], residual=pre, res_exp=E["h2"], flags=EPI_RELU | ops.EPI_ADD_PRE,
                                     out_exp=E["post"], overflow=flag, out=self._buffer("tail_t", (n, 27, 8) + tuple(o.shape[3:6]), dev))
            cost = ops.deconv_tail_gather(t, st["tail_bias"], hv)
            _ROUTES["x3_fused_tail"] += 1
        else:
            post = L["h5"](o, E["h4"], *A["h5"], residual=pre, flags=EPI_RELU | ops.EPI_ADD_PRE, out_exp=E["h2"], to_f32=True)
            cost = hg.conv6.fused(post, residual=None, head=self.classifier, head_residual=hv)
        _ROUTES["x3_tail"] += 1
        if self.overflow_check == "call" and st["guard"].wait():
            raise SplitOverflow()
        return cost

    def _tail(self, v, hv=None):
        cost, _, _ = self.hg_conv3d(v, None, None, residual=v, head=self.classifier, head_residual=hv)
        return cost

    def _gn_qualifies(self, device, arithmetic=None):
        mode = arithmetic or self.arithmetic
        norms = [m for m in self.modules() if isinstance(m, (nn.GroupNorm, nn.modules.batchnorm._BatchNorm))]
        if (not norms or not all(isinstance(m, nn.GroupNorm) for m in norms) or not X3_GROUP_NORM[0] or mode == "fp32"
                or torch.is_grad_enabled() or self.training or self.split_off or device.type != "cuda"
                or self.conv1[0][0].out_channels % 32 != 0):
            return None
        return self.split_guard(device, mode)

    def _gn_tail_x3(self, v1, timing=None, arithmetic=None):
        if isinstance(v1, SplitT):
            v1s, guard = v1, self.__dict__["_snvc_x3_guard"][v1.t.device]
        else:
            if not (v1.is_cuda and v1.dtype == torch.float32):
                return None
            guard = self._gn_qualifies(v1.device, arithmetic)
            if guard is None:
                return None
            norm1 = self.conv1[0][1]
            b1 = x3_norm_bound(norm1, plan_for(self.conv1[0][0], "_x3", v1.device))
            e1 = x3_exponent(b1)
            v1s = SplitT(ops.to_split(v1, e1, out=self._v1s(v1.shape, v1.device, last="v1")), e1, b1)
        _mark(timing, "conv2", 0)
        v2 = self.conv2.fused_x3(v1s, flag=guard.flag)
        _mark(timing, "conv2", 1)
        out, _, _ = self.hg_conv3d.forward_x3(v2, residual=v2, flag=guard.flag)
        guard.post()
        cost = self.classifier(ops.from_split(out.t, out.exp))
        _ROUTES["x3_gn_tail"] += 1
        if self.overflow_check == "call" and guard.wait():
            raise SplitOverflow()
        return cost

    @staticmethod
    def _sheared_geometry4(m0: int, d: int, w: int):
        off = 8
        wu = (off + 4 * (w - 1) + 1 + 5 + 5 + 3) // 4 * 4
        u_lo = 4 * (w - 1) - (d - 1) - m0 - 5
        return off, wu, 8 - u_lo, (d + 10 + 8 + 3) // 4 * 4

    @staticmethod
    def _sheared_layer4(plans, wr):
        def fold():
            w = wr.detach().double()
            cout, c = w.shape[0], w.shape[1]
            k = torch.zeros((3, 3, cout, c, 3, 3), dtype=torch.float64, device=w.device)
            for cls, kds in enumerate(SHEAR_CLASS_KDS):
                for kd in kds:
                    for kw in (-1, 0, 1):
                        k[kw + 1, cls, :, :, :, 1 - kd] += w[:, :, kd + 1, :, kw + 1]
            return [k.reshape(9 * cout, c, 3, 3)]
        return GlobalStack._layers(plans, "sheared4", ops.Conv3dLayer, fold)[0]

    def _sheared4_inputs(self, plans, wr, rq_src, q_up, m0, d, w):
        lay = self._sheared_layer4(plans, wr)
        off, wu, off_col, wu_col = self._sheared_geometry4(m0, d, w)
        out = []
        for width, o_, last in ((wu, off, False), (wu_col, off_col, True)):
            p = lay(ops.sheared_upsample(rq_src, q_up, width, o_).unsqueeze(2)).squeeze(2)
            n, c9, h, _ = p.shape
            p = p.view(n, 3, c9 // 3, h, width)
            g = p[:, 1].clone()
            g[..., 4:] += p[:, 0][..., :-4]
            if not last:
                g[..., :-4] += p[:, 2][..., 4:]
            out.append(g.contiguous())
        return out[0], out[1], off, off_col

    def _ds_sheared_first_layer(self, left, right, shift, ds, arithmetic=None):
        conv, bn = self.conv1[0][0], self.conv1[0][1]
        nonneg, structure = self._shift_structure(shift)
        assert nonneg
        if structure is None or structure[0] * ds not in (2, 4):
            return None
        q_up, m0 = structure
        phases = q_up * ds
        n, c = left.size(0), left.size(1)
        h, w, d = left.size(2) // ds, left.size(3) // ds, shift.size(1)
        if w % 8 or w > 512:
            return None
        if phases == 2:
            if not self._sheared_fits(2, m0, d, w, False):
                return None
        else:
            _, wu4, _, _ = self._sheared_geometry4(m0, d, w)
            if 4 * ((wu4 + 3) // 4 * 4 + 16 + d) > 150 * 1024:
                return None
        st = self._x3_select(left.device, arithmetic)
        left_s = left[:, :, ::ds, ::ds].contiguous()
        right_r = right[:, :, ::ds, :].contiguous()
        plans = _factored_plans(conv, c)
        scale, bias = _folded_bn(bn, plans["plan"])
        prep = _Prep(plans, c, conv.weight, st, scale, bias)
        self._left_planes(prep, left_s)
        if phases == 2:
            g, gcol, off, off_col, _ = self._sheared_inputs(prep, right_r, 2, m0, d, w, up=1)
        else:
            g, gcol, off, off_col = self._sheared4_inputs(plans, conv.weight.detach()[:, c:], right_r, q_up, m0, d, w)
        planes = prep.planes
        return self._finish_first_layer(
            prep, (n, c, d, h, w), left.device, None, arithmetic, "ds_sheared_first_conv",
            lambda v1s, sc, bi: ops.sheared_expand_split(g, gcol, planes, sc, bi, v1s, phases, m0, off, off_col, ops.EPI_RELU, st["flag"]),
            lambda v: ops.sheared_expand(g, gcol, planes, scale, bias, v, phases, m0, off, off_col, ops.EPI_RELU))

    def _gn_sheared_first_layer(self, left, right, shift, arithmetic=None):
        conv, norm = self.conv1[0][0], self.conv1[0][1]
        guard = self._gn_qualifies(left.device, arithmetic)
        if guard is None:
            return None
        nonneg, structure = self._shift_structure(shift)
        assert nonneg
        n, c, h, w = left.shape
        d = shift.size(1)
        if structure is None or not self._sheared_fits(structure[0], structure[1], d, w, True):
            return None
        q, m0 = structure
        prep = _Prep(_factored_plans(conv, c), c, conv.weight)
        self._left_planes(prep, left)
        g, gcol, off, off_col, _ = self._sheared_inputs(prep, right, q, m0, d, w)
        planes = prep.planes
        b1 = x3_norm_bound(norm, plan_for(conv, "_x3", left.device))
        e1 = x3_exponent(b1)
        v1s = self._v1s((n, c, d, h, w), left.device)
        gam = norm.weight.detach() if norm.weight is not None else None
        bet = norm.bias.detach() if norm.bias is not None else None
        try:
            for i in range(n):
                sc, sh, _, _ = ops.sheared_expand_stats(g[i:i + 1], gcol[i:i + 1], planes[i:i + 1], gam, bet, (1, c, d, h, w), q, m0, off,
                                                        off_col, norm.eps)
                ops.sheared_expand_split(g[i:i + 1], gcol[i:i + 1], planes[i:i + 1], (sc * 2.0 ** e1).reshape(-1).contiguous(),
                                         (sh * 2.0 ** e1).reshape(-1).contiguous(), v1s[i:i + 1], q, m0, off, off_col, ops.EPI_RELU, guard.flag)
        except ops.Unsupported:
            return None
        _ROUTES["gn_sheared_first_conv"] += 1
        return self._gn_tail_x3(SplitT(v1s, e1, b1), None, arithmetic)

    def _conv2_tail(self, v1, shape, timing=None, arithmetic=None, st=_ASK):
        gn_cost = self._gn_tail_x3(v1, timing, arithmetic)
        if gn_cost is not None:
            return gn_cost
        if st is _ASK:
            st = self._x3_select(v1.device, arithmetic) if (v1.is_cuda and v1.dtype == torch.float32) else None
        if st is not None:
            return self._tail_x3(st, ops.to_split(v1, st["exp"]["v1"], out=self._v1s(v1.shape, v1.device, last="v1")), timing)
        _mark(timing, "conv2", 0)
        v, hv = self.conv2.fused(v1, out=self._buffer("v2", shape, v1.device), side_head=self.classifier)
        _mark(timing, "conv2", 1)
        return self._tail(v, hv)
# ... 374 lines not shown
```

snvc_amd/ops.py:

```python
import contextlib
import ctypes
import math
import threading
import time
from typing import Optional, Tuple

import torch

from . import _dedup, _derived, _fused, _lib
from ._lib import (EPI_ADD_POST, EPI_ADD_PRE, EPI_RELU, EPI_SIGMOID, EPI_STREAM_OUT, F32, F64, Conv3dDesc,
                   Unsupported, check)

__all__ = [
    "cost_volume_forward", "cost_volume_forward_right", "cost_volume_backward", "cost_volume_backward_right", "depth_class_sums", "voxel_gather_forward", "voxel_gather_backward",
    "Conv3dLayer", "conv_variant", "conv3d_wgrad", "Conv3dLayerF16", "to_c8", "from_c8", "voxel_gather_forward_f16",
    "mul_broadcast_c8", "avgpool_depth4_c8", "volume_resample", "rect_to_psv_grid", "act_backward_reduce", "act_backward_apply", "bn_backward_coefs", "norm_stats", "affine_act", "mul_broadcast", "avgpool_depth4", "zero_stuff2x",
    "disparity_regression", "argmax_rows", "roiaware_pool3d_forward", "roiaware_pool3d_backward",
    "points_in_boxes_gpu", "points_in_boxes_cpu",
    "EPI_RELU", "EPI_ADD_PRE", "EPI_ADD_POST", "EPI_SIGMOID", "EPI_STREAM_OUT",
]


_variant_bits = 0


@contextlib.contextmanager
def conv_variant(algo_bits: int):
    global _variant_bits
    prev = _variant_bits
    _variant_bits = int(algo_bits)
    try:
        yield
    finally:
        _variant_bits = prev


def _algo(exact: bool = False) -> int:
    return (_variant_bits | _lib.ALGO_DIRECT) if exact else _variant_bits


def _gpu(t: torch.Tensor, name: str):
    if not t.is_cuda:
        raise RuntimeError(f"{name} must be a GPU tensor: Not implemented on the CPU")


def _ptr(t: Optional[torch.Tensor]):
    return ctypes.c_void_p(t.data_ptr()) if t is not None and t.numel() > 0 else ctypes.c_void_p(0)


def _stream(t: torch.Tensor):
    return ctypes.c_void_p(torch.cuda.current_stream(t.device).cuda_stream)


def _dtype_tag(t: torch.Tensor, what: str) -> int:
    if t.dtype == torch.float32:
        return F32
    if t.dtype == torch.float64:
        return F64
    raise RuntimeError(f'"{what}" not implemented for {t.dtype}')


def cost_volume_forward(left, right, shift, downsample: int):
    _gpu(left, "left"); _gpu(right, "right"); _gpu(shift, "shift")
    if left.dim() != 4 or tuple(left.shape) != tuple(right.shape):
        raise RuntimeError("Left image and right image should match their size.")
    if shift.dim() != 2 or left.size(0) != shift.size(0):
        raise RuntimeError("Image and shift should of same batch.")
    tag = _dtype_tag(left, "BuildCostVolume_forward")
    if right.dtype != left.dtype or shift.dtype != left.dtype:
        raise RuntimeError("left, right and shift must share one dtype")
    downsample = int(downsample)
    if downsample < 1:
        raise RuntimeError("downsample must be >= 1")
    n, c, hi, wi = left.shape
    d = shift.size(1)
    if hi % downsample or wi % downsample:
        raise RuntimeError("feature height and width must be multiples of downsample")
    out = torch.empty((n, 2 * c, d, hi // downsample, wi // downsample), dtype=left.dtype, device=left.device)
    if out.numel() == 0:
        return out
    left, right, shift = left.contiguous(), right.contiguous(), shift.contiguous()
    with torch.cuda.device(left.device):
        check(_lib.lib().snvc_cost_volume_forward(_ptr(left), _ptr(right), _ptr(shift), _ptr(out), n, c, hi, wi, d,
                                                  downsample, tag, _stream(left)), "build_cost_volume_forward")
    return out


def cost_volume_forward_right(right, shift, out=None):
    _gpu(right, "right"); _gpu(shift, "shift")
    if right.dtype != torch.float32 or shift.dtype != torch.float32:
        raise RuntimeError("cost_volume_forward_right is fp32 only")
    n, c, h, w = right.shape
    d = shift.size(1)
    if out is None:
        out = torch.empty((n, c, d, h, w), dtype=torch.float32, device=right.device)
    elif tuple(out.shape) != (n, c, d, h, w) or out.dtype != torch.float32 or not out.is_contiguous():
        raise RuntimeError("cost_volume_forward_right `out` must be a contiguous float32 [N,C,D,H,W] tensor")
    else:
        _written(out)
    if out.numel() == 0:
        return out
    right, shift = right.contiguous(), shift.contiguous()
    with torch.cuda.device(right.device):
        check(_lib.lib().snvc_cost_volume_forward_right(_ptr(right), _ptr(shift), _ptr(out), n, c, h, w, d, 1,
                                                        _stream(right)), "snvc_cost_volume_forward_right")
    return out


def cost_volume_backward(grad, shift, downsample: int):
    _gpu(grad, "grad"); _gpu(shift, "shift")
    tag = _dtype_tag(grad, "BuildCostVolume_backward")
    if shift.dtype != grad.dtype:
        raise RuntimeError("grad and shift must share one dtype")
    downsample = int(downsample)
    n, c2, _, h, w = grad.shape
    c, d = c2 // 2, shift.size(1)
    if grad.numel() != n * c * 2 * d * h * w:
        raise RuntimeError("grad shape is wrong")
    gl = torch.empty((n, c, h * downsample, w * downsample), dtype=grad.dtype, device=grad.device)
    gr = torch.empty_like(gl)
    if gl.numel() == 0:
        return gl, gr
    grad, shift = grad.contiguous(), shift.contiguous()
    with torch.cuda.device(grad.device):
        check(_lib.lib().snvc_cost_volume_backward(_ptr(grad), _ptr(shift), _ptr(gl), _ptr(gr), n, c, h, w, d,
                                                   downsample, tag, _stream(grad)), "build_cost_volume_backward")
    return gl, gr


def cost_volume_backward_right(grad_r, shift):
    _gpu(grad_r, "grad"); _gpu(shift, "shift")
    if grad_r.dtype != torch.float32 or shift.dtype != torch.float32 or grad_r.dim() != 5:
        raise RuntimeError("cost_volume_backward_right needs float32 [N,C,D,H,W]")
    grad_r, shift = grad_r.contiguous(), shift.contiguous()
    n, c, d, h, w = grad_r.shape
    out = torch.empty((n, c, h, w), dtype=torch.float32, device=grad_r.device)
    with torch.cuda.device(grad_r.device):
        check(_lib.lib().snvc_cost_volume_backward_right(_ptr(grad_r), _ptr(shift), _ptr(out), n, c, h, w, d, _stream(grad_r)),
              "snvc_cost_volume_backward_right")
    return out


def depth_class_sums(g):
    _gpu(g, "g")
    g = g.contiguous()
    n, c, d, h, w = g.shape
    out = torch.empty((n, c, 3, h, w), dtype=torch.float32, device=g.device)
    with torch.cuda.device(g.device):
        check(_lib.lib().snvc_depth_class_sums(_ptr(g), _ptr(out), n * c, d, h * w, _stream(g)), "snvc_depth_class_sums")
    return out


def _check_gather(left, right, l_pts, r_pts):
    for t, nm in ((left, "left"), (right, "right"), (l_pts, "grid_proj_left"), (r_pts, "grid_proj_right")):
        _gpu(t, nm)
        if t.dtype != torch.float32:
            raise RuntimeError(f"{nm} must be float32")
    if left.dim() != 4 or tuple(left.shape) != tuple(right.shape):
        raise RuntimeError("left and right feature maps must have the same [N,F,H,W] shape")
    if l_pts.dim() != 3 or l_pts.size(1) != 2 or tuple(l_pts.shape) != tuple(r_pts.shape) or l_pts.size(0) != left.size(0):
        raise RuntimeError("grid projections must be [N,2,V] for the same batch as the features")

# ... 1122 lines not shown
            int(flags), float(2.0 ** out_exp), float(2.0 ** -res_exp), _stream(raw)), "snvc_f16x3_affine_from_ncdhw")
    return out


def split_scale_for(*tensors) -> torch.Tensor:
    if tensors and all(t.is_cuda and t.dtype == torch.float32 and t.is_contiguous() and t.data_ptr() % 16 == 0 and t.numel() > 0
                       for t in tensors):
        out = None
        for t in tensors:
            s_ = split_scale_of(t.detach())
            out = s_ if out is None else torch.minimum(out, s_)
        return out
    amax = None
    for t in tensors:
        lo, hi = torch.aminmax(t.detach())
        a = torch.maximum(-lo, hi)
        amax = a if amax is None else torch.maximum(amax, a)
    amax = amax.float().reshape(1)
    e = torch.floor(torch.log2(16384.0 / amax))
    e = torch.where(torch.isfinite(e), e, torch.zeros_like(e)).clamp_(-24, 40)
    return torch.exp2(e)


_SCALE_SCRATCH = {}
_SCALE_SCRATCH_LOCK = threading.Lock()


def _scale_scratch(device) -> torch.Tensor:
    key = (device, torch.cuda.current_stream(device).cuda_stream)
    scratch = _SCALE_SCRATCH.get(key)
    if scratch is None:
        with _SCALE_SCRATCH_LOCK:
            scratch = _SCALE_SCRATCH.get(key)
            if scratch is None:
                scratch = _SCALE_SCRATCH[key] = torch.zeros(2, dtype=torch.int32, device=device)
    return scratch


def split_scale_of(t: torch.Tensor) -> torch.Tensor:
    _gpu(t, "t")
    if t.dtype != torch.float32 or not t.is_contiguous() or t.data_ptr() % 16:
        return split_scale_for(t)
    scratch = _scale_scratch(t.device)
    out = torch.empty(1, dtype=torch.float32, device=t.device)
    with torch.cuda.device(t.device):
        check(_lib.lib().snvc_f16x3_split_scale(_ptr(t), t.numel(), _ptr(scratch), _ptr(out), _stream(t)), "snvc_f16x3_split_scale")
    return out


def sheared_upsample_split(right, q: int, wu: int, off: int, mul_dev: torch.Tensor):
    _gpu(right, "right")
    if right.dtype != torch.float32 or right.dim() != 4:
        raise RuntimeError("sheared_upsample_split needs a float32 [N,C,H,W] tensor")
    right = right.contiguous()
    n, c, h, w = right.shape
    out = torch.empty((n, 2, (c + 7) // 8, 1, h, wu, 8), dtype=torch.float16, device=right.device)
    if out.numel():
        with torch.cuda.device(right.device):
            check(_lib.lib().snvc_sheared_upsample_split(_ptr(right), _ptr(out), _lo_ptr(out), _ptr(mul_dev), n, c, h, w, int(q), int(wu), int(off),
                                                         _stream(right)), "snvc_sheared_upsample_split")
    return out


class Conv2dLayerX3:

    def __init__(self, weight: torch.Tensor):
        _gpu(weight, "weight")
        if weight.dtype != torch.float32 or weight.dim() != 4:
            raise RuntimeError("Conv2dLayerX3 needs a float32 [Cout,Cin,kh,kw] weight")
        self.cout, self.cin, self.kh, self.kw = (int(v) for v in weight.shape)
        nbytes = _lib.lib().snvc_f16x3_conv2d_packed_weight_bytes(self.cout, self.cin, self.kh, self.kw)
        if nbytes < 0:
            raise Unsupported("Conv2dLayerX3: 3x7 or 3x3 kernels, Cin % 8 == 0, Cout % 32 == 0")
        w = weight.detach().contiguous()
        wmax = float(w.abs().max().item()) if w.numel() else 1.0
        self.w_exp = 14 - math.frexp(wmax)[1] if wmax > 0 and math.isfinite(wmax) else 0
        self.packed = torch.empty(nbytes, dtype=torch.uint8, device=w.device)
        with torch.cuda.device(w.device):
            check(_lib.lib().snvc_f16x3_conv2d_pack_weights(_ptr(w), self.cout, self.cin, self.kh, self.kw, _ptr(self.packed),
                                                            float(2.0 ** self.w_exp), _stream(w)), "snvc_f16x3_conv2d_pack_weights")

    def __call__(self, x, x_mul_dev=None, scale=None, bias=None, flags: int = 0, x_exp: int = 0):
        _split_check(x, "x")
        if x.size(2) * 8 != self.cin or x.size(3) != 1:
            raise RuntimeError(f"Conv2dLayerX3 input must be a split pair [N,2,{self.cin // 8},1,H,W,8]")
        n, h, w = x.size(0), x.size(4), x.size(5)
        y = torch.empty((n, self.cout, h, w), dtype=torch.float32, device=x.device)
        if y.numel():
            with torch.cuda.device(x.device):
                check(_lib.lib().snvc_f16x3_conv2d_forward(_ptr(x), _lo_ptr(x), _ptr(self.packed), _ptr(scale), _ptr(bias), _ptr(y), n, self.cin,
                                                           self.cout, h, w, self.kh, self.kw, float(2.0 ** -(self.w_exp + x_exp)), _ptr(x_mul_dev),
                                                           int(flags), _stream(x)), "snvc_f16x3_conv2d_forward")
        return y


def sheared_prep_x3(right, q: int, wu: int, off: int, wu_col: int, off_col: int, lay_g: "Conv2dLayerX3", lay_col: "Conv2dLayerX3", ws: dict):
    _gpu(right, "right")
    right = right.contiguous()
    n, c, h, w = right.shape
    key = (n, c, h, w, wu, wu_col, right.device)
    if ws.get("key") != key:
        dev = right.device
        ws.clear()
        ws.update(key=key, rq=torch.empty(n * 2 * c * h * wu, dtype=torch.float16, device=dev),
                  rq2=torch.empty(n * 2 * c * h * wu_col, dtype=torch.float16, device=dev), mul=torch.empty(1, dtype=torch.float32, device=dev),
                  g=torch.empty((n, lay_g.cout, h, wu), dtype=torch.float32, device=dev),
                  gcol=torch.empty((n, lay_col.cout, h, wu_col), dtype=torch.float32, device=dev))
    scratch = _scale_scratch(right.device)
    with torch.cuda.device(right.device):
        check(_lib.lib().snvc_sheared_prep_x3(_ptr(right), n, c, h, w, int(q), int(wu), int(off), int(wu_col), int(off_col), _ptr(lay_g.packed),
                                              _ptr(lay_col.packed), lay_g.cout, float(2.0 ** -lay_g.w_exp), float(2.0 ** -lay_col.w_exp),
                                              _ptr(ws["rq"]), _ptr(ws["rq2"]), _ptr(scratch), _ptr(ws["mul"]), _ptr(ws["g"]), _ptr(ws["gcol"]),
                                              _stream(right)), "snvc_sheared_prep_x3")
    return ws["g"], ws["gcol"]


def conv2d_x3_from_f32(x, layers, ws: dict):
    _gpu(x, "x")
    x = x.contiguous()
    if x.dtype != torch.float32 or x.dim() != 4:
        raise RuntimeError("conv2d_x3_from_f32 needs a float32 [N,C,H,W] tensor")
    n, c, h, w = x.shape
    key = (n, c, h, w, tuple(id(l) for l in layers), x.device)
    if ws.get("key") != key:
        ws.clear()
        ws.update(key=key, split=torch.empty(n * 2 * c * h * w, dtype=torch.float16, device=x.device),
                  mul=torch.empty(1, dtype=torch.float32, device=x.device),
                  y=[torch.empty((n, l.cout, h, w), dtype=torch.float32, device=x.device) for l in layers])
        k = len(layers)
        ws["c_packed"] = (ctypes.c_void_p * k)(*[l.packed.data_ptr() for l in layers])
        ws["c_cout"] = (ctypes.c_int64 * k)(*[l.cout for l in layers])
        ws["c_mul"] = (ctypes.c_float * k)(*[2.0 ** -l.w_exp for l in layers])
        ws["c_y"] = (ctypes.c_void_p * k)(*[t.data_ptr() for t in ws["y"]])
        ws["layers"] = list(layers)
    scratch = _scale_scratch(x.device)
    with torch.cuda.device(x.device):
        check(_lib.lib().snvc_f16x3_conv2d_from_f32(_ptr(x), n, c, h, w, layers[0].kh, layers[0].kw, len(layers), ws["c_packed"], ws["c_cout"],
                                                    ws["c_mul"], ws["c_y"], _ptr(ws["split"]), _ptr(scratch), _ptr(ws["mul"]), _stream(x)),
              "snvc_f16x3_conv2d_from_f32")
    return ws["y"]



def il_index(mode: int, oc: int, c: int, h_dim: int, pitch: int, lp: int, cls0: int, h: int, x: int) -> int:
    return int(_fused.lib().snvc_fused_il_index(mode, oc, c, h_dim, pitch, lp, cls0, h, x))


def fused_il_geometry(q: int, m0: int, d: int, w: int, wu: int, off: int, wu_col: int, off_col: int):
    lo = min(0, q * (w - 1) - (d - 1) - m0 + off_col, -(d - 1) - m0 + off if w > 1 else 0)
    hi = max(wu - 1, wu_col - 1, q * (w - 1) - m0 + off_col, q * (w - 2) - m0 + off if w > 1 else 0)
    return hi - lo + 1, -lo


def fused_first_wedge_tiles(d: int, w: int, q: int, m0: int, off: int):
    desc = _lib.Conv3dDesc()
    desc.Din, desc.Win = int(d), int(w)
    ntw = (int(w) + 31) // 32
    first, last = (ctypes.c_int64 * ntw)(), (ctypes.c_int64 * ntw)()
    dups = int(_dedup.lib().snvc_dedup_fused_first_tiles(ctypes.byref(desc), int(q), int(m0), int(off), first, last, ntw))
    if dups < 0:
        raise ValueError(_lib.lib().snvc_last_error_string().decode())
    return dups, list(first), list(last)


def sheared_prep_x3_il(right, q: int, wu: int, off: int, wu_col: int, off_col: int, lay_g: "Conv2dLayerX3", lay_col: "Conv2dLayerX3", ws: dict,
                       pitch: int, lp: int):
    _gpu(right, "right")
    right = right.contiguous()
    n, c, h, w = right.shape
    key = (n, c, h, w, wu, wu_col, pitch, lp, right.device)
    if ws.get("key") != key:
        dev = right.device
        ws.clear()
        ws.update(key=key, rq=torch.empty(n * 2 * c * h * wu, dtype=torch.float16, device=dev),
                  rq2=torch.empty(n * 2 * c * h * wu_col, dtype=torch.float16, device=dev), mul=torch.empty(1, dtype=torch.float32, device=dev),
                  g=torch.empty((n, lay_g.cout, h, wu), dtype=torch.float32, device=dev),
                  gcol=torch.empty((n, lay_col.cout, h, wu_col), dtype=torch.float32, device=dev),
                  gi=torch.zeros((n, 6, c // 8, h, pitch, 8), dtype=torch.float32, device=dev))
    scratch = _scale_scratch(right.device)
    with torch.cuda.device(right.device):
        check(_fused.lib().snvc_fused_sheared_prep_x3(_ptr(right), n, c, h, w, int(q), int(wu), int(off), int(wu_col), int(off_col),
                                                      _ptr(lay_g.packed), _ptr(lay_col.packed), lay_g.cout, float(2.0 ** -lay_g.w_exp),
                                                      float(2.0 ** -lay_col.w_exp), _ptr(ws["rq"]), _ptr(ws["rq2"]), _ptr(scratch), _ptr(ws["mul"]),
                                                      _ptr(ws["g"]), _ptr(ws["gcol"]), _ptr(ws["gi"]), int(pitch), int(lp), _stream(right)),
              "snvc_fused_sheared_prep_x3")
    return ws["g"], ws["gcol"], ws["gi"]


def planes_x3_il(x, layer: "Conv2dLayerX3", ws: dict):
    _gpu(x, "x")
    x = x.contiguous()
    if x.dtype != torch.float32 or x.dim() != 4:
        raise RuntimeError("planes_x3_il needs a float32 [N,C,H,W] tensor")
    n, c, h, w = x.shape
    key = (n, c, h, w, id(layer), "il", x.device)
    if ws.get("key") != key:
        ws.clear()
        ws.update(key=key, split=torch.empty(n * 2 * c * h * w, dtype=torch.float16, device=x.device),
                  mul=torch.empty(1, dtype=torch.float32, device=x.device),
                  y=[torch.empty((n, layer.cout, h, w), dtype=torch.float32, device=x.device)],
                  p_il=torch.empty((n, 3, c // 8, h, w, 8), dtype=torch.float32, device=x.device), layers=[layer])
    scratch = _scale_scratch(x.device)
    with torch.cuda.device(x.device):
        check(_fused.lib().snvc_fused_planes_from_f32(_ptr(x), n, c, h, w, _ptr(layer.packed), layer.cout, float(2.0 ** -layer.w_exp),
                                                      _ptr(ws["y"][0]), _ptr(ws["p_il"]), _ptr(ws["split"]), _ptr(scratch), _ptr(ws["mul"]),
                                                      _stream(x)), "snvc_fused_planes_from_f32")
    return ws["y"][0], ws["p_il"]


def from_split(x: torch.Tensor, exp: int = 0, channels: Optional[int] = None) -> torch.Tensor:
    _split_check(x, "x")
    n, g = x.shape[0], x.shape[2]
    sp = tuple(x.shape[3:6])
    c = channels if channels is not None else 8 * g
    y = torch.empty((n, c) + sp, dtype=torch.float32, device=x.device)
    if y.numel() == 0:
        return y
    with torch.cuda.device(x.device):
        check(_lib.lib().snvc_f16x3_to_ncdhw(_ptr(x), _lo_ptr(x), _ptr(y), n, c, math.prod(sp), _batch_stride(x), 0, float(2.0 ** -exp),
                                             _stream(x)), "snvc_f16x3_to_ncdhw")
    return y


X3_SMALL_BELOW = {"stride2": 0, "transposed": 4096}


_ONES_ZEROS = {}


def _ones_zeros(c: int, device):
    key = (c, device)
    hit = _ONES_ZEROS.get(key)
    if hit is None:
        hit = _ONES_ZEROS[key] = (torch.ones(c, device=device), torch.zeros(c, device=device))
    return hit


def x3_form(cout: int, ksize: int, stride: int, dilation: int, transposed: bool, n: int, out_sp, plain: bool, split_out: bool,
            forced: Optional[int]) -> int:
    if forced is None and stride == 1 and not transposed and ksize in (5, 7) and cout % 32 == 0:
        tiles5 = n * -(-out_sp[0] // 4) * -(-out_sp[1] // 4) * -(-out_sp[2] // 32) * (cout // 32)
        q16 = X3_Q16[0] and split_out and tiles5 >= 512 and (ksize == 7 or dilation == 2 or X3_Q16_K5[0])
        return _lib.ALGO_X3_Q16 if q16 else 0
    if forced is None and ksize == 3 and cout % 64 == 0 and (stride == 2 or transposed):
        if transposed:
            wgs = 8 * n * -(-out_sp[0] // 8) * -(-out_sp[1] // 8) * -(-out_sp[2] // 64)
            return _lib.ALGO_X3_SMALL if wgs < X3_SMALL_BELOW["transposed"] else 0
        wgs = n * -(-out_sp[0] // 2) * -(-out_sp[1] // 4) * -(-out_sp[2] // 32)
        if X3_Q16_S2[0] and plain and split_out:
            return _lib.ALGO_X3_Q16
        return _lib.ALGO_X3_SMALL if wgs < X3_SMALL_BELOW["stride2"] else 0
    if forced is not None or stride != 1 or transposed or ksize != 3 or cout == 1:
        return forced if forced is not None else 0
    tiles = n * -(-out_sp[0] // 4) * -(-out_sp[1] // 4) * -(-out_sp[2] // 32)
    if plain and X3_Q16[0] and cout % 32 == 0 and tiles * (cout // 32) >= X3_Q16_MIN_JOBS[0]:
        return _lib.ALGO_X3_Q16
    if cout % 64 == 0 and tiles * (cout // 64) >= 1024:
        return _lib.ALGO_X3_SERIAL
    if tiles * (cout // 32) >= 1024 or cout == 32 and tiles >= 512:
        return _lib.ALGO_X3_NARROW if cout != 32 else 0
    return _lib.ALGO_X3_SMALL


def _residual_f32_check(residual_f32, y) -> None:
    if (residual_f32.dtype != torch.float32 or tuple(residual_f32.shape) != tuple(y.shape) or not _dense_inner(residual_f32)
            or _batch_stride(residual_f32) != _batch_stride(y)):
        raise RuntimeError("residual_f32 must be a float32 tensor of the result's shape and layout")


class Conv3dLayerX3(_ConvGeometry):

    def __init__(self, weight: torch.Tensor, ksize: int = 3, stride: int = 1, pad: int = 1, dilation: int = 1, transposed: bool = False,
                 algo: Optional[int] = None, w_mul_dev: Optional[torch.Tensor] = None):
        _gpu(weight, "weight")
        if weight.dtype != torch.float32:
            raise RuntimeError("conv3d weights must be float32")
        super().__init__(weight, ksize, stride, pad, dilation, transposed)
        self.forced_algo = algo
        self.algo = int(algo or 0)
        self.w_mul_dev = w_mul_dev
        self._sc_w = self._bi_0 = None
        if w_mul_dev is not None:
            self.weight = (weight.detach() * w_mul_dev).contiguous()
            self.w_exp = 0
        else:
            self.weight = weight.detach().contiguous()
            wmax = float(self.weight.abs().max().item()) if weight.numel() else 1.0
            self.w_exp = 14 - math.frexp(wmax)[1] if wmax > 0 and math.isfinite(wmax) else 0
        self._packed = {}
        self.packed = self._pack(self.algo) if w_mul_dev is None else None
        self._affine = {}

    def _pack(self, algo: int):
        hit = self._packed.get(algo)
        if hit is None:
            probe = self._desc(1, (16, 16, 32), 0, algo)
            nbytes = _lib.lib().snvc_f16x3_conv3d_packed_weight_bytes(ctypes.byref(probe))
            if nbytes < 0:
                check(2, "snvc_f16x3_conv3d_packed_weight_bytes")
            hit = torch.empty(nbytes, dtype=torch.uint8, device=self.weight.device)
            with torch.cuda.device(self.weight.device):
                check(_lib.lib().snvc_f16x3_conv3d_pack_weights(ctypes.byref(probe), _ptr(self.weight), _ptr(hit), float(2.0 ** self.w_exp),
                                                                _stream(self.weight)), "snvc_f16x3_conv3d_pack_weights")
            self._packed[algo] = hit
        return hit

    def _launch(self, x, plain: bool = False, split_out: bool = False):
        n, in_sp = x.size(0), tuple(x.shape[3:6])
        out_sp = self.out_spatial(in_sp)
        algo = self.algo = x3_form(self.cout, self.ksize, self.stride, self.dilation, self.transposed, n, out_sp, plain, split_out,
                                   self.forced_algo)
        return n, in_sp, out_sp, algo, self._pack(algo)

    def _unit_affine(self, device):
        if self._sc_w is None:
            self._sc_w, self._bi_0 = _ones_zeros(self.cout, device)[0] / self.w_mul_dev, _ones_zeros(self.cout, device)[1]
        return self._sc_w, self._bi_0

    def folded(self, scale, bias, x_exp: int, out_exp: int):
        def build():
            dev = self.weight.device
            sc = (scale.detach().float() if scale is not None else torch.ones(self.cout, device=dev)) * (2.0 ** (out_exp - x_exp - self.w_exp))
            bi = (bias.detach().float() if bias is not None else torch.zeros(self.cout, device=dev)) * (2.0 ** out_exp)
            return sc.contiguous(), bi.contiguous()
        return _derived.derived(self._affine, (x_exp, out_exp), (scale, bias), build)

    def __call__(self, x, x_exp: int = 0, scale=None, bias=None, residual=None, flags: int = 0, out=None, out_exp: int = 0,
                 out_f32=None, to_f32: bool = False, head=None, overflow=None, x_mul_dev=None, res_exp: Optional[int] = None,
                 residual_f32: Optional[torch.Tensor] = None):
        _split_check(x, "x")
        if x.size(2) * 8 != self.cin:
            raise RuntimeError(f"conv3d input must have {self.cin} channels (split C8), got {x.size(2) * 8}")
        f32 = to_f32 or out_f32 is not None or self.cout == 1
        n, in_sp, out_sp, algo, packed = self._launch(x, plain=residual is None and (not f32 or (self.w_mul_dev is not None and head is None)),
                                                      split_out=not f32 and head is None)
        split_shape = (n, 2, self.cout // 8) + out_sp + (8,)
        if f32:
            out_f32 = _result(out_f32, (n, self.cout) + out_sp, torch.float32, x.device,
                              "out_f32 must be a float32 [N,Cout,D,H,W] tensor, dense below dim 0")
        else:
            out = _result(out, split_shape, torch.float16, x.device, "conv3d `out` must be a split C8 tensor of the output shape", _split_check)
        residual = _residual(residual, split_shape, "residual must have the output's shape (split C8)", _split_check)
        if residual_f32 is not None:
            if not f32 or residual is not None or flags & (EPI_ADD_PRE | EPI_ADD_POST) or self.cout == 1:
                raise RuntimeError("residual_f32 goes with a float32 result and no other residual")
            _residual_f32_check(residual_f32, out_f32)
            flags = flags | EPI_ADD_POST
        y_head = None
        if head is not None:
            head = head.detach().reshape(-1).float().contiguous()
            y_head = torch.empty((n, 1) + out_sp, dtype=torch.float32, device=x.device)
        if self.w_mul_dev is not None and scale is None and bias is None and x_exp == 0 and out_exp == 0:
            sc, bi = self._unit_affine(x.device)
            if x_mul_dev is not None:
                sc = sc / x_mul_dev
        else:
            sc, bi = self.folded(scale, bias, x_exp, out_exp)
            if x_mul_dev is not None:
                sc = (sc / x_mul_dev).contiguous()
            if self.w_mul_dev is not None:
                sc = (sc / self.w_mul_dev).contiguous()
        if n == 0:
            return out_f32 if f32 else ((out, y_head) if head is not None else out)
        d = self._desc(n, in_sp, flags, algo, _batch_stride(x), _batch_stride(out_f32 if f32 else out),
                       _batch_stride(residual) if residual is not None else 0)
        null = ctypes.c_void_p(0)
        with torch.cuda.device(x.device):
            check(_lib.lib().snvc_f16x3_conv3d_forward(ctypes.byref(d), _ptr(x), _lo_ptr(x), _ptr(packed), _ptr(sc), _ptr(bi),
                                                       _ptr(residual if residual_f32 is None else residual_f32),
                                                       _lo_ptr(residual) if residual is not None else null,
                                                       null if f32 else _ptr(out), null if f32 else _lo_ptr(out),
                                                       _ptr(out_f32) if f32 else null, _ptr(head), _ptr(y_head), float(2.0 ** -out_exp),
                                                       float(2.0 ** (out_exp - (out_exp if res_exp is None else res_exp))),
                                                       _ptr(overflow), _stream(x)), "snvc_f16x3_conv3d_forward")
        if f32:
            return out_f32
        return (out, y_head) if head is not None else out

    def fused_first_form(self, n: int, sp) -> bool:
        return (self.ksize == 3 and self.stride == 1 and not self.transposed and self.w_mul_dev is None and self.cin % 8 == 0
                and x3_form(self.cout, 3, 1, self.dilation, False, n, tuple(sp), True, False, self.forced_algo) == _lib.ALGO_X3_Q16)

    def forward_fused_first(self, gi, pitch: int, lp: int, p_il, v_scale, v_bias, q: int, m0: int, off: int, off_col: int, v_flags: int,
                            n: int, in_sp, x_exp: int = 0, scale=None, bias=None, flags: int = 0, out=None, out_exp: int = 0, head=None,
                            overflow=None, dedup: bool = False):
        in_sp = tuple(int(v) for v in in_sp)
        if not self.fused_first_form(n, in_sp):
            raise Unsupported("forward_fused_first: the layer does not run on the 16x16x32 form at this size")
        algo = self.algo = _lib.ALGO_X3_Q16
        packed = self._pack(algo)
        out_sp = self.out_spatial(in_sp)
        out = _result(out, (n, 2, self.cout // 8) + out_sp + (8,), torch.float16, gi.device,
                      "conv3d `out` must be a split C8 tensor of the output shape", _split_check)
        y_head = None
        if head is not None:
            head = head.detach().reshape(-1).float().contiguous()
            y_head = torch.empty((n, 1) + out_sp, dtype=torch.float32, device=gi.device)
        sc, bi = self.folded(scale, bias, x_exp, out_exp)
        if n == 0:
            return (out, y_head) if head is not None else out
        d = self._desc(n, in_sp, flags, algo, 0, _batch_stride(out), 0)
        entry = (_dedup.lib().snvc_dedup_fused_first_conv3d_forward if dedup else _fused.lib().snvc_fused_first_conv3d_forward)
        with torch.cuda.device(gi.device):
            check(entry(ctypes.byref(d), _ptr(packed), _ptr(sc), _ptr(bi), _ptr(out), _lo_ptr(out), _ptr(head), _ptr(y_head),
                        float(2.0 ** -out_exp), _ptr(overflow), _ptr(gi), int(pitch), int(lp), _ptr(p_il), _ptr(v_scale), _ptr(v_bias), int(q),
                        int(m0), int(off), int(off_col), int(v_flags), _stream(gi)),
                  "snvc_dedup_fused_first_conv3d_forward" if dedup else "snvc_fused_first_conv3d_forward")
        return (out, y_head) if head is not None else out

    def forward_f32(self, x, x_mul_dev, residual_f32: Optional[torch.Tensor] = None, relu: bool = False):
        _split_check(x, "x")
        if self.w_mul_dev is None or x.size(2) * 8 != self.cin:
            raise RuntimeError("forward_f32: a device-scaled layer (w_mul_dev) and an input of its channel count")
        n, in_sp, out_sp, algo, packed = self._launch(x, plain=True, split_out=False)
        sc, bi = self._unit_affine(x.device)
        y = torch.empty((n, self.cout) + out_sp, dtype=torch.float32, device=x.device)
        if residual_f32 is not None:
            _residual_f32_check(residual_f32, y)
        if n == 0:
            return y
        d = self._desc(n, in_sp, EPI_RELU if relu else 0, algo, _batch_stride(x), _batch_stride(y), 0)
        with torch.cuda.device(x.device):
            check(_lib.lib().snvc_f16x3_conv3d_forward_f32(ctypes.byref(d), _ptr(x), _lo_ptr(x), _ptr(packed), _ptr(sc), _ptr(bi),
                                                           _ptr(x_mul_dev), _ptr(residual_f32), _ptr(y), 1.0, _stream(x)),
                  "snvc_f16x3_conv3d_forward_f32")
        return y

    def forward_stats(self, x, x_mul_dev, gamma, beta, eps: float):
        _split_check(x, "x")
        if self.w_mul_dev is None or x.size(2) * 8 != self.cin or self.cout % 32:
            return None
        n, in_sp, out_sp, algo, packed = self._launch(x, plain=True, split_out=False)
        sc, bi = self._unit_affine(x.device)
        raw = torch.empty((n, self.cout) + out_sp, dtype=torch.float32, device=x.device)
        d = self._desc(n, in_sp, 0, algo, _batch_stride(x), _batch_stride(raw), 0)
        nbytes = _lib.lib().snvc_f16x3_conv3d_stats_workspace_bytes(ctypes.byref(d))
        if nbytes < 0:
            return None
        ws = torch.empty(nbytes, dtype=torch.uint8, device=x.device)
        out = torch.empty((4, self.cout), dtype=torch.float32, device=x.device)
        with torch.cuda.device(x.device):
            rc = _lib.lib().snvc_f16x3_conv3d_forward_stats(ctypes.byref(d), _ptr(x), _lo_ptr(x), _ptr(packed), _ptr(sc), _ptr(bi),
                                                            _ptr(x_mul_dev), _ptr(raw), 1.0, _ptr(gamma), _ptr(beta), _ptr(out[0]), _ptr(out[1]), _ptr(out[2]),
                                                            _ptr(out[3]), _ptr(ws), float(eps), _stream(x))
        if rc == 2:
            return None
        check(rc, "snvc_f16x3_conv3d_forward_stats")
        return raw, out[0:1], out[1:2], out[2:3], out[3:4]

    def forward_tail(self, x, x_exp: int, scale, bias, tail: "TailWeightsX3", residual=None, flags: int = 0, out_exp: int = 0,
                     overflow=None, res_exp: Optional[int] = None, out=None):
        _split_check(x, "x")
        if not self.transposed or self.stride != 2 or x.size(2) * 8 != self.cin or tail.cin != self.cout:
            raise RuntimeError("forward_tail: a ConvTranspose3d(k3,s2,p1,op1) layer whose Cout equals the tail's Cin")
        n, in_sp, out_sp, algo, packed = self._launch(x)
        shape = (n, 27, 8) + in_sp
        if out is None:
            out = torch.empty(shape, dtype=torch.float32, device=x.device)
        elif tuple(out.shape) != shape or out.dtype != torch.float32 or not out.is_contiguous():
            raise RuntimeError("forward_tail `out` must be a contiguous float32 [N, 27, 8, Din, Hin, Win] tensor")
        else:
            _written(out)
        residual = _residual(residual, (n, 2, self.cout // 8) + out_sp + (8,), "residual must have the layer's output shape (split C8)", _split_check)
        sc, bi = self.folded(scale, bias, x_exp, out_exp)
        if n == 0:
            return out
        d = self._desc(n, in_sp, flags, algo, _batch_stride(x), 0, _batch_stride(residual) if residual is not None else 0)
        null = ctypes.c_void_p(0)
        with torch.cuda.device(x.device):
            check(_lib.lib().snvc_f16x3_deconv3d_tail_forward(
                ctypes.byref(d), _ptr(x), _lo_ptr(x), _ptr(packed), _ptr(sc), _ptr(bi), _ptr(residual),
                _lo_ptr(residual) if residual is not None else null, float(2.0 ** (out_exp - (out_exp if res_exp is None else res_exp))),
                _ptr(tail.packed), _ptr(out), float(2.0 ** -(out_exp + tail.w_exp)), _ptr(overflow), _stream(x)),
                "snvc_f16x3_deconv3d_tail_forward")
        return out


class TailWeightsX3:

    def __init__(self, weight: torch.Tensor):
        _gpu(weight, "weight")
        w = weight.detach().reshape(weight.shape[0], -1).float().contiguous()
        if w.shape[1] != 27 or w.shape[0] % 32 != 0:
            raise RuntimeError("tail weights must be [Cin, 27] (or [Cin, 1, 3, 3, 3]) with Cin % 32 == 0")
        self.cin = int(w.shape[0])
        wmax = float(w.abs().max().item()) if w.numel() else 1.0
        self.w_exp = 14 - math.frexp(wmax)[1] if wmax > 0 and math.isfinite(wmax) else 0
        nbytes = _lib.lib().snvc_f16x3_tail_packed_weight_bytes(self.cin)
        self.packed = torch.empty(nbytes, dtype=torch.uint8, device=w.device)
        with torch.cuda.device(w.device):
            check(_lib.lib().snvc_f16x3_tail_pack_weights(_ptr(w), self.cin, _ptr(self.packed), float(2.0 ** self.w_exp), _stream(w)),
                  "snvc_f16x3_tail_pack_weights")


def deconv_tail_gather(t: torch.Tensor, bias: Optional[torch.Tensor] = None, residual: Optional[torch.Tensor] = None, out=None):
    _gpu(t, "t")
    if t.dtype != torch.float32 or t.dim() != 6 or t.size(1) != 27 or t.size(2) != 8 or not t.is_contiguous():
        raise RuntimeError("t must be a contiguous float32 [N, 27, 8, nd, nh, nw] tensor")
    n, nd, nh, nw = t.size(0), t.size(3), t.size(4), t.size(5)
    shape = (n, 1, 4 * nd, 4 * nh, 4 * nw)
    if out is None:
        out = torch.empty(shape, dtype=torch.float32, device=t.device)
    elif tuple(out.shape) != shape or out.dtype != torch.float32 or not out.is_contiguous():
        raise RuntimeError("out must be a contiguous float32 tensor of the output shape")
    else:
        _written(out)
    if residual is not None:
        _gpu(residual, "residual")
        if residual.dtype != torch.float32 or residual.numel() != out.numel() or not residual.is_contiguous():
            raise RuntimeError("residual must be a contiguous float32 tensor of the output shape")
    if bias is not None:
        bias = bias.detach().reshape(-1)[:1].float().contiguous()
    with torch.cuda.device(t.device):
        check(_lib.lib().snvc_deconv_tail_gather(_ptr(t), _ptr(bias), _ptr(residual), _ptr(out), n, nd, nh, nw, _stream(t)),
              "snvc_deconv_tail_gather")
    return out


def mul_broadcast_split(feat, occ, out=None):
    _split_check(feat, "feat")
    _gpu(occ, "occ")
    occ = occ.contiguous()
    n, g = feat.shape[0], feat.shape[2]
    s_ = math.prod(feat.shape[3:6])
    if occ.dtype != torch.float32 or occ.numel() != n * s_:
        raise RuntimeError("occupancy must be float32 [N,1,D,H,W] matching the feature volume")
    if out is None:
        out = torch.empty(feat.shape, dtype=torch.float16, device=feat.device)
    else:
        _split_check(out, "out")
        if tuple(out.shape) != tuple(feat.shape):
            raise RuntimeError("mul_broadcast_split `out` must have feat's shape")
        _written(out)
    if feat.numel() == 0:
        return out
    with torch.cuda.device(feat.device):
        check(_lib.lib().snvc_f16x3_mul_broadcast(_ptr(feat), _lo_ptr(feat), _ptr(occ), _ptr(out), _lo_ptr(out), n, 8 * g, s_,
                                                  _batch_stride(feat), _batch_stride(out), _stream(feat)), "snvc_f16x3_mul_broadcast")
    return out


def mul_broadcast_c8(feat, occ, out=None):
    _c8_check(feat, "feat")
    _gpu(occ, "occ")
    occ = occ.contiguous()
    n, g = feat.shape[0], feat.shape[1]
    s = math.prod(feat.shape[2:5])
    if occ.dtype != torch.float32 or occ.numel() != n * s:
        raise RuntimeError("occupancy must be float32 [N,1,D,H,W] matching the feature volume")
    if out is None:
        out = torch.empty_like(feat)
    else:
        _c8_check(out, "out")
        if tuple(out.shape) != tuple(feat.shape):
            raise RuntimeError("mul_broadcast_c8 `out` must have feat's shape")
        _written(out)
    if feat.numel() == 0:
        return out
    with torch.cuda.device(feat.device):
        check(_lib.lib().snvc_f16_mul_broadcast(_ptr(feat), _ptr(occ), _ptr(out), n, 8 * g, s, _batch_stride(feat),
                                                _batch_stride(out), _stream(feat)), "snvc_f16_mul_broadcast")
    return out


def avgpool_depth4_c8(x):
    _c8_check(x, "x")
    n, g, d, h, w, _ = x.shape
    y = torch.empty((n, 8 * g, d // 4, h, w), dtype=torch.float32, device=x.device)
    if y.numel() == 0:
        return y
    with torch.cuda.device(x.device):
        check(_lib.lib().snvc_f16_avgpool_depth4(_ptr(x), _ptr(y), n, 8 * g, d, h * w, _batch_stride(x), _stream(x)),
              "snvc_f16_avgpool_depth4")
    return y


def roiaware_pool3d_forward(rois, pts, pts_feature, argmax, pts_idx_of_voxels, pooled_features, pool_method: int):
    for t, nm in ((rois, "rois"), (pts, "pts"), (pts_feature, "pts_feature"), (argmax, "argmax"),
                  (pts_idx_of_voxels, "pts_idx_of_voxels"), (pooled_features, "pooled_features")):
        _gpu(t, nm)
        if not t.is_contiguous():
            raise RuntimeError(f"{nm} must be contiguous")
    b, p, c = rois.size(0), pts.size(0), pts_feature.size(1)
    _, ox, oy, oz, max_pts = pts_idx_of_voxels.shape
    if not (ox < 256 and oy < 256 and oz < 256):
        raise AssertionError("we encode index with 8bit")
    ws = torch.empty((max(b * p, 1),), dtype=torch.int32, device=rois.device)
    with torch.cuda.device(rois.device):
        check(_lib.lib().snvc_roiaware_pool3d_forward(_ptr(rois), _ptr(pts), _ptr(pts_feature), _ptr(argmax),
                                                      _ptr(pts_idx_of_voxels), _ptr(pooled_features), _ptr(ws), b, p,
                                                      c, max_pts, ox, oy, oz, int(pool_method), _stream(rois)),
              "roiaware_pool3d forward")
    return 1


def roiaware_pool3d_backward(pts_idx_of_voxels, argmax, grad_out, grad_in, pool_method: int):
    for t, nm in ((pts_idx_of_voxels, "pts_idx_of_voxels"), (argmax, "argmax"), (grad_out, "grad_out"), (grad_in, "grad_in")):
        _gpu(t, nm)
        if not t.is_contiguous():
            raise RuntimeError(f"{nm} must be contiguous")
    b, ox, oy, oz, max_pts = pts_idx_of_voxels.shape
    c = grad_out.size(4)
    with torch.cuda.device(grad_out.device):
        check(_lib.lib().snvc_roiaware_pool3d_backward(_ptr(pts_idx_of_voxels), _ptr(argmax), _ptr(grad_out),
                                                       _ptr(grad_in), b, c, max_pts, ox, oy, oz, int(pool_method),
                                                       _stream(grad_out)), "roiaware_pool3d backward")
    return 1


def points_in_boxes_gpu(boxes, pts, box_idx_of_points):
    for t, nm in ((boxes, "boxes"), (pts, "pts"), (box_idx_of_points, "box_idx_of_points")):
        _gpu(t, nm)
        if not t.is_contiguous():
            raise RuntimeError(f"{nm} must be contiguous")
    bs, t_, m = boxes.size(0), boxes.size(1), pts.size(1)
    with torch.cuda.device(boxes.device):
        check(_lib.lib().snvc_points_in_boxes_gpu(_ptr(boxes), _ptr(pts), _ptr(box_idx_of_points), bs, t_, m,
                                                  _stream(boxes)), "points_in_boxes_gpu")
    return 1


def points_in_boxes_cpu(boxes, pts, pts_indices):
    for t, nm in ((boxes, "boxes"), (pts, "pts"), (pts_indices, "pts_indices")):
        if t.is_cuda:
            raise RuntimeError(f"{nm} must be a CPU tensor")
        if not t.is_contiguous():
            raise RuntimeError(f"{nm} must be contiguous")
    check(_lib.lib().snvc_points_in_boxes_cpu(ctypes.c_void_p(boxes.data_ptr()), ctypes.c_void_p(pts.data_ptr()),
                                              ctypes.c_void_p(pts_indices.data_ptr()), boxes.size(0), pts.size(0)),
          "points_in_boxes_cpu")
    return 1
```

Before: 544.4.

## Alias duplicated wedge tiles instead of copying them in fused-first conv

Adds an aliased path in which the fused first conv skips the wedge copy kernel for duplicated tiles. Downstream consumers remap depth to the first pure tile when reading instead: the stride-2 x3 conv geometry and the deconv tail gather residual. This removes a copy kernel launch and its memory traffic. In exchange it adds index arithmetic in the loaders and new ABI entry points, and it runs only when the model enables alias_wedge together with dedup and the fused tail.

```diff
diff --git a/include/snvc_alias.h b/include/snvc_alias.h
--- /dev/null
+++ b/include/snvc_alias.h
@@ -0,0 +1,37 @@
+#ifndef SNVC_ALIAS_H
+#define SNVC_ALIAS_H
+
+#include <stdint.h>
+
+#include "snvc_hip.h"
+
+#ifdef __cplusplus
+extern "C" {
+#endif
+
+typedef struct snvc_wedge_desc {
+    int32_t D, W;
+    int32_t q, m0, off;
+} snvc_wedge_desc;
+
+SNVC_API int snvc_alias_abi_version(void);
+
+SNVC_API int64_t snvc_alias_depth(const snvc_wedge_desc *desc, int64_t d, int64_t w);
+
+SNVC_API int snvc_alias_fused_first_conv3d_forward(const snvc_conv3d_desc *desc, const void *packed_weight, const float *scale,
+                                                   const float *bias, void *y_hi, void *y_lo, const float *head, float *y_head,
+                                                   float head_mul, int *overflow, const float *gi, int64_t pitch, int64_t lp,
+                                                   const float *p_il, const float *v_scale, const float *v_bias, int q, int m0, int off,
+                                                   int off2, int v_flags, void *stream);
+
+SNVC_API int snvc_alias_f16x3_conv3d_forward(const snvc_conv3d_desc *desc, const void *x_hi, const void *x_lo, const void *packed_weight,
+                                             const float *scale, const float *bias, void *y_hi, void *y_lo, int *overflow,
+                                             const snvc_wedge_desc *in_alias, void *stream);
+
+SNVC_API int snvc_alias_deconv_tail_gather(const float *t, const float *bias, const float *residual, float *y, int64_t n, int64_t nd,
+                                           int64_t nh, int64_t nw, const snvc_wedge_desc *res_alias, void *stream);
+
+#ifdef __cplusplus
+}
+#endif
+#endif
diff --git a/snvc_amd/_alias.py b/snvc_amd/_alias.py
--- /dev/null
+++ b/snvc_amd/_alias.py
@@ -0,0 +1,39 @@
+import ctypes
+
+from . import _fused, _lib
+
+_ABI = 1
+
+c_i64 = ctypes.c_int64
+c_int = ctypes.c_int
+c_p = ctypes.c_void_p
+
+
+class WedgeDesc(ctypes.Structure):
+    _fields_ = [(n, ctypes.c_int32) for n in ("D", "W", "q", "m0", "off")]
+
+
+SIGNATURES = {
+    "snvc_alias_abi_version": (c_int, []),
+    "snvc_alias_depth": (c_i64, [ctypes.POINTER(WedgeDesc), c_i64, c_i64]),
+    "snvc_alias_fused_first_conv3d_forward": _fused.SIGNATURES["snvc_fused_first_conv3d_forward"],
+    "snvc_alias_f16x3_conv3d_forward": (c_int, [ctypes.POINTER(_lib.Conv3dDesc), c_p, c_p, c_p, c_p, c_p, c_p, c_p, c_p,
+                                                ctypes.POINTER(WedgeDesc), c_p]),
+    "snvc_alias_deconv_tail_gather": (c_int, [c_p, c_p, c_p, c_p, c_i64, c_i64, c_i64, c_i64, ctypes.POINTER(WedgeDesc), c_p]),
+}
+
+_bound = None
+
+
+def lib() -> ctypes.CDLL:
+    global _bound
+    if _bound is None:
+        handle = _lib.lib()
+        for name, (res, args) in SIGNATURES.items():
+            fn = getattr(handle, name)
+            fn.restype = res
+            fn.argtypes = args
+        if handle.snvc_alias_abi_version() != _ABI:
+            raise RuntimeError("libsnvc_hip.so aliased wedge ABI version mismatch; rebuild it")
+        _bound = handle
+    return _bound
diff --git a/snvc_amd/csrc/conv3d_f16.hip b/snvc_amd/csrc/conv3d_f16.hip
--- a/snvc_amd/csrc/conv3d_f16.hip
+++ b/snvc_amd/csrc/conv3d_f16.hip
@@ -4,6 +4,7 @@
 #include "elementwise_internal.hpp"
 #include "snvc_fused.h"
 #include "snvc_dedup.h"
+#include "snvc_alias.h"
 
 namespace snvc {
 namespace {
@@ -77,6 +78,20 @@
 __host__ __device__ __forceinline__ bool wedge_tile_duplicate(int D, int W, int q, int m0, int off, int d0, int w0) {
     return wedge_tile_pure(D, W, q, m0, off, d0, w0) && wedge_tile_pure(D, W, q, m0, off, d0 - 4, w0);
 }
+
+using WedgeDesc = snvc_wedge_desc;
+__host__ __device__ __forceinline__ int wedge_first_pure(const WedgeDesc &g, int w0) {
+    const int lo = g.q * (w0 + 32) - g.m0 + g.off + 2;
+    return ((lo > 4 ? lo : 4) + 3) & ~3;
+}
+__host__ __device__ __forceinline__ int wedge_alias_depth(const WedgeDesc &g, int d, int w) {
+    const int w0 = w & ~31, d0 = d & ~3, first = wedge_first_pure(g, w0);
+    return (w0 + 32 < g.W - 1 && d0 > first && d0 + 3 <= g.D - 3) ? first + (d & 3) : d;
+}
+struct F16AliasArgs : F16Args {
+    WedgeDesc in_alias;
+};
+constexpr int SRC_NO_COPY = 1 << 29;
 
 
 template <int KD_, int KH_, int KW_, int STRIDE_, int DIL_, int MI_, int TD_, int TH_, int KCG_, int MODE_, bool DB_, int OCC_,
@@ -1265,8 +1280,9 @@
     asm volatile("s_waitcnt lgkmcnt(%4)" : "+v"(b[0]), "+v"(b[1]), "+v"(b[2]), "+v"(b[3]) : "n"(N) : "memory");
 }
 
+template <int ALIAS = 0>
 __global__ void __launch_bounds__(512, 1)
-conv3d_x3s2q_kernel(const F16Args a, const int total_jobs) {
+conv3d_x3s2q_kernel(const std::conditional_t<ALIAS == 1, F16AliasArgs, F16Args> a, const int total_jobs) {
     using Cfg = X3S2Cfg;
     constexpr int NB = Cfg::NB, TH = Cfg::TH, IN_H = Cfg::IN_H, IN_W = Cfg::IN_W, VOX = Cfg::VOX, NIT = Cfg::NIT, NQ = Cfg::NQ;
     extern __shared__ __attribute__((aligned(16))) char lds[];
@@ -1301,7 +1317,9 @@
             const int ww = pp == 64 ? 64 : (rr_ < 16 ? 2 * (16 * blk + rr_) : 2 * (16 * blk + rr_ - 16) + 1);
             const int gd = id0 + dd, gh = ih0 + hh, gw = iw0 + ww;
             const bool ok = i < VOX && (unsigned)gd < (unsigned)a.Din && (unsigned)gh < (unsigned)a.Hin && (unsigned)gw < (unsigned)a.Win;
-            off[it] = ok ? (unsigned)(gd * in_hw + gh * a.Win + gw) : 0u;
+            int sd = gd;
+            if constexpr (ALIAS) sd = wedge_alias_depth(a.in_alias, gd, gw);
+            off[it] = ok ? (unsigned)(sd * in_hw + gh * a.Win + gw) : 0u;
             vmask |= (ok ? 1u : 0u) << it;
         }
     };
@@ -1877,9 +1895,10 @@
     out[i] = pl == 0 ? hi : (_Float16)(v - (float)hi);
 }
 
-__global__ void __launch_bounds__(256)
-deconv_tail_gather_kernel(const float *__restrict__ t, const float *__restrict__ bias, const float *__restrict__ res, float *__restrict__ y,
-                          int nd, int nh, int nw, int64_t t_bs, int64_t y_bs, int64_t r_bs) {
+template <int ALIAS>
+__device__ __forceinline__ void deconv_tail_gather_body(const float *__restrict__ t, const float *__restrict__ bias, const float *__restrict__ res,
+                                                        float *__restrict__ y, int nd, int nh, int nw, int64_t t_bs, int64_t y_bs, int64_t r_bs,
+                                                        const WedgeDesc &ra) {
     const int OD = 4 * nd, OH = 4 * nh;
     const int64_t total = (int64_t)OD * OH * nw;
     const int64_t i = (int64_t)blockIdx.x * 256 + threadIdx.x;
@@ -1913,10 +1932,23 @@
     }
     const int64_t sp = ((int64_t)od * OH + oh) * (4 * nw) + 4 * j;
     if (res) {
-        const f32x4 rv = *reinterpret_cast<const f32x4 *>(res + n * r_bs + sp);
+        int64_t rsp = sp;
+        if constexpr (ALIAS) rsp = ((int64_t)wedge_alias_depth(ra, od, 4 * j) * OH + oh) * (4 * nw) + 4 * j;
+        const f32x4 rv = *reinterpret_cast<const f32x4 *>(res + n * r_bs + rsp);
         o0 += rv[0]; o1 += rv[1]; o2 += rv[2]; o3 += rv[3];
     }
     *reinterpret_cast<f32x4 *>(y + n * y_bs + sp) = f32x4{o0, o1, o2, o3};
+}
+
+__global__ void __launch_bounds__(256)
+deconv_tail_gather_kernel(const float *__restrict__ t, const float *__restrict__ bias, const float *__restrict__ res, float *__restrict__ y,
+                          int nd, int nh, int nw, int64_t t_bs, int64_t y_bs, int64_t r_bs) {
+    deconv_tail_gather_body<0>(t, bias, res, y, nd, nh, nw, t_bs, y_bs, r_bs, WedgeDesc{});
+}
+__global__ void __launch_bounds__(256)
+deconv_tail_gather_alias_kernel(const float *__restrict__ t, const float *__restrict__ bias, const float *__restrict__ res, float *__restrict__ y,
+                                int nd, int nh, int nw, int64_t t_bs, int64_t y_bs, int64_t r_bs, const WedgeDesc ra) {
+    deconv_tail_gather_body<1>(t, bias, res, y, nd, nh, nw, t_bs, y_bs, r_bs, ra);
 }
 
 __global__ void __launch_bounds__(256)
@@ -2026,11 +2058,17 @@
     wedge_copy_kernel<<<dim3((unsigned)((r.td1 - r.td0 + 1) * r.ntw), (unsigned)a.tiles_h, (unsigned)a.N), 256, 0, st>>>(w);
 }
 
-void launch_x3s2q(const F16Args &a, const F16Geom &g, hipStream_t st) {
+int x3s2q_workgroups(const F16Geom &g) {
     int wg = device_cu_count();
     if (wg <= 0) wg = 256;
     if (g.jobs < wg) wg = g.jobs >= 8 ? (int)(g.jobs & ~(int64_t)7) : (int)g.jobs;
-    launch_lds<conv3d_x3s2q_kernel>(dim3((unsigned)wg), X3S2Cfg::THREADS, X3S2Cfg::LDS_BYTES, st, a, (int)g.jobs);
+    return wg;
+}
+void launch_x3s2q(const F16Args &a, const F16Geom &g, hipStream_t st) {
+    launch_lds<conv3d_x3s2q_kernel<0>>(dim3((unsigned)x3s2q_workgroups(g)), X3S2Cfg::THREADS, X3S2Cfg::LDS_BYTES, st, a, (int)g.jobs);
+}
+void launch_x3s2q_alias(const F16AliasArgs &a, const F16Geom &g, hipStream_t st) {
+    launch_lds<conv3d_x3s2q_kernel<1>>(dim3((unsigned)x3s2q_workgroups(g)), X3S2Cfg::THREADS, X3S2Cfg::LDS_BYTES, st, a, (int)g.jobs);
 }
 
 template <class Cfg, int... EPI>
@@ -2370,6 +2408,7 @@
     int64_t *stats_slots = nullptr;
     const float *x_mul = nullptr;
     const snvc::F16SrcArgs *src = nullptr;
+    const snvc_wedge_desc *in_alias = nullptr;
     void *stream = nullptr;
 };
 
@@ -2459,11 +2498,22 @@
     if (!f.launch[call] || (resflags && !f.split_res)) return fail(SNVC_ERR_UNSUPPORTED, f.unsupported);
     if (g.jobs >= ((int64_t)1 << 30)) return fail(SNVC_ERR_UNSUPPORTED, "snvc_f16x3_conv3d_forward: too many tiles");
     if (c.src && to_f32) return fail(SNVC_ERR_UNSUPPORTED, "snvc_fused_first_conv3d_forward: a split C8 output");
-    if ((b.v_flags & SRC_DEDUP) && ((c.y_head && (d->Wout % 4 || (reinterpret_cast<uintptr_t>(c.y_head) & 15))) ||
+    if ((b.v_flags & SRC_DEDUP) && ((!(b.v_flags & SRC_NO_COPY) && c.y_head && (d->Wout % 4 || (reinterpret_cast<uintptr_t>(c.y_head) & 15))) ||
                                     wedge_ranges(a.Din, a.Win, b.v_q, b.v_m0, b.v_off, nullptr, nullptr, 0).dups == 0))
         b.v_flags &= ~SRC_DEDUP;
+    if (c.in_alias) {
+        if (&f != &FORM_K3S2XQ || call != TO_C8)
+            return fail(SNVC_ERR_UNSUPPORTED, "snvc_alias_f16x3_conv3d_forward: built for the stride-2 3x3x3 layer on the 16x16x32 form (SNVC_ALGO_X3_Q16) with a split C8 result");
+        if (c.in_alias->D != d->Din || c.in_alias->W != d->Win || (c.in_alias->q != 1 && c.in_alias->q != 2))
+            return fail(SNVC_ERR_INVALID_ARGUMENT, "snvc_alias_f16x3_conv3d_forward: in_alias describes a [Din][.][Win] tensor, q = 1 | 2");
+        F16AliasArgs al{};
+        static_cast<F16Args &>(al) = a;
+        al.in_alias = *c.in_alias;
+        launch_x3s2q_alias(al, g, st);
+        return check_launch("snvc_alias_f16x3_conv3d_forward");
+    }
     f.launch[call](b, g, st);
-    if (b.v_flags & SRC_DEDUP) launch_wedge_copy(b, st);
+    if ((b.v_flags & SRC_DEDUP) && !(b.v_flags & SRC_NO_COPY)) launch_wedge_copy(b, st);
     return check_launch("snvc_f16x3_conv3d_forward");
 }
 
@@ -2485,7 +2535,7 @@
 static int fused_first_forward(const snvc_conv3d_desc *d, const void *packed_weight, const float *scale, const float *bias, void *y_hi,
                                void *y_lo, const float *head, float *y_head, float head_mul, int *overflow, const float *gi,
                                int64_t pitch, int64_t lp, const float *p_il, const float *v_scale, const float *v_bias, int q, int m0,
-                               int off, int off2, int v_flags, bool dedup, void *stream) {
+                               int off, int off2, int v_flags, int dedup, void *stream) {
     using namespace snvc;
     if (!d || !gi || !p_il || !v_scale || !v_bias) return fail(SNVC_ERR_INVALID_ARGUMENT, "snvc_fused_first_conv3d_forward: null pointer");
     if (d->transposed || d->ksize != 3 || d->stride != 1 || d->pad != 1 || d->dilation != 1 || d->Cin % 8 || d->Din < 1 || d->Hin < 1 || d->Win < 1 ||
@@ -2503,7 +2553,7 @@
     F16SrcArgs s{};
     s.gi = gi; s.p_il = p_il; s.v_scale = v_scale; s.v_bias = v_bias; s.gi_bs = 6 * CG * H * pitch * 8;
     s.v_pitch = (int)pitch; s.v_lp = (int)lp; s.v_q = q; s.v_m0 = m0; s.v_off = off; s.v_off2 = off2;
-    s.v_flags = v_flags | (dedup ? SRC_DEDUP : 0);
+    s.v_flags = v_flags | dedup;
     F16x3Call c;
     c.packed_weight = packed_weight; c.scale = scale; c.bias = bias; c.y_hi = y_hi; c.y_lo = y_lo;
     c.head = head; c.y_head = y_head; c.head_mul = head_mul; c.res_mul = 1.0f; c.overflow = overflow; c.src = &s; c.stream = stream;
@@ -2515,7 +2565,7 @@
                                     int64_t pitch, int64_t lp, const float *p_il, const float *v_scale, const float *v_bias, int q, int m0,
                                     int off, int off2, int v_flags, void *stream) {
     return fused_first_forward(d, packed_weight, scale, bias, y_hi, y_lo, head, y_head, head_mul, overflow, gi, pitch, lp, p_il, v_scale, v_bias,
-                               q, m0, off, off2, v_flags, false, stream);
+                               q, m0, off, off2, v_flags, 0, stream);
 }
 
 int snvc_dedup_abi_version(void) { return 1; }
@@ -2525,7 +2575,7 @@
                                           const float *gi, int64_t pitch, int64_t lp, const float *p_il, const float *v_scale,
                                           const float *v_bias, int q, int m0, int off, int off2, int v_flags, void *stream) {
     return fused_first_forward(d, packed_weight, scale, bias, y_hi, y_lo, head, y_head, head_mul, overflow, gi, pitch, lp, p_il, v_scale, v_bias,
-                               q, m0, off, off2, v_flags, true, stream);
+                               q, m0, off, off2, v_flags, snvc::SRC_DEDUP, stream);
 }
 
 int64_t snvc_dedup_fused_first_tiles(const snvc_conv3d_desc *d, int q, int m0, int off, int64_t *first_td, int64_t *last_td, int max_tw) {
@@ -2536,6 +2586,34 @@
     }
     for (int tw = 0; tw < max_tw; ++tw) first_td[tw] = last_td[tw] = -1;
     return wedge_ranges((int)d->Din, (int)d->Win, q, m0, off, first_td, last_td, max_tw).dups;
+}
+
+int snvc_alias_abi_version(void) { return 1; }
+
+int64_t snvc_alias_depth(const snvc_wedge_desc *w, int64_t d, int64_t x) {
+    using namespace snvc;
+    if (!w || (w->q != 1 && w->q != 2) || d < 0 || d >= w->D || x < 0 || x >= w->W) {
+        fail(SNVC_ERR_INVALID_ARGUMENT, "snvc_alias_depth: a desc with q = 1 | 2 and (d, w) inside [0, D) x [0, W)");
+        return -1;
+    }
+    return wedge_alias_depth(*w, (int)d, (int)x);
+}
+
+int snvc_alias_fused_first_conv3d_forward(const snvc_conv3d_desc *d, const void *packed_weight, const float *scale, const float *bias,
+                                          void *y_hi, void *y_lo, const float *head, float *y_head, float head_mul, int *overflow,
+                                          const float *gi, int64_t pitch, int64_t lp, const float *p_il, const float *v_scale,
+                                          const float *v_bias, int q, int m0, int off, int off2, int v_flags, void *stream) {
+    return fused_first_forward(d, packed_weight, scale, bias, y_hi, y_lo, head, y_head, head_mul, overflow, gi, pitch, lp, p_il, v_scale, v_bias,
+                               q, m0, off, off2, v_flags, snvc::SRC_DEDUP | snvc::SRC_NO_COPY, stream);
+}
+
+int snvc_alias_f16x3_conv3d_forward(const snvc_conv3d_desc *d, const void *x_hi, const void *x_lo, const void *packed_weight,
+                                    const float *scale, const float *bias, void *y_hi, void *y_lo, int *overflow,
+                                    const snvc_wedge_desc *in_alias, void *stream) {
+    F16x3Call c;
+    c.x_hi = x_hi; c.x_lo = x_lo; c.packed_weight = packed_weight; c.scale = scale; c.bias = bias;
+    c.y_hi = y_hi; c.y_lo = y_lo; c.head_mul = 1.0f; c.res_mul = 1.0f; c.overflow = overflow; c.in_alias = in_alias; c.stream = stream;
+    return f16x3_forward(d, c);
 }
 
 int64_t snvc_f16x3_conv3d_stats_workspace_bytes(const snvc_conv3d_desc *d) {
@@ -2791,9 +2869,11 @@
     return f16x3_forward(d, c);
 }
 
-int snvc_deconv_tail_gather(const float *t, const float *bias, const float *residual, float *y, int64_t n, int64_t nd, int64_t nh,
-                            int64_t nw, void *stream) {
+static int tail_gather(const float *t, const float *bias, const float *residual, float *y, int64_t n, int64_t nd, int64_t nh, int64_t nw,
+                       const snvc_wedge_desc *res_alias, void *stream) {
     using namespace snvc;
+    if (res_alias && (!residual || res_alias->D != 4 * nd || res_alias->W != 4 * nw || (res_alias->q != 1 && res_alias->q != 2)))
+        return fail(SNVC_ERR_INVALID_ARGUMENT, "snvc_alias_deconv_tail_gather: res_alias describes the residual [4 nd][.][4 nw], q = 1 | 2");
     if (n < 0 || nd <= 0 || nh <= 0 || nw <= 0) return fail(SNVC_ERR_INVALID_ARGUMENT, "snvc_deconv_tail_gather: sizes must be positive");
     if (n == 0) return SNVC_OK;
     if (!t || !y) return fail(SNVC_ERR_INVALID_ARGUMENT, "snvc_deconv_tail_gather: null pointer");
@@ -2803,9 +2883,23 @@
     if (threads >= ((int64_t)1 << 31) * 255 || n > 65535 || 27 * 8 * nd * nh * nw >= ((int64_t)1 << 40))
         return fail(SNVC_ERR_UNSUPPORTED, "snvc_deconv_tail_gather: tensor too large");
     const dim3 grid((unsigned)ceil_div<int64_t>(threads, 256), (unsigned)n);
-    deconv_tail_gather_kernel<<<grid, 256, 0, as_stream(stream)>>>(t, bias, residual, y, (int)nd, (int)nh, (int)nw, 27 * 8 * nd * nh * nw,
-                                                                   out_vox, out_vox);
+    if (res_alias)
+        deconv_tail_gather_alias_kernel<<<grid, 256, 0, as_stream(stream)>>>(t, bias, residual, y, (int)nd, (int)nh, (int)nw,
+                                                                             27 * 8 * nd * nh * nw, out_vox, out_vox, *res_alias);
+    else
+        deconv_tail_gather_kernel<<<grid, 256, 0, as_stream(stream)>>>(t, bias, residual, y, (int)nd, (int)nh, (int)nw, 27 * 8 * nd * nh * nw,
+                                                                       out_vox, out_vox);
     return check_launch("snvc_deconv_tail_gather");
 }
 
-}
+int snvc_deconv_tail_gather(const float *t, const float *bias, const float *residual, float *y, int64_t n, int64_t nd, int64_t nh,
+                            int64_t nw, void *stream) {
+    return tail_gather(t, bias, residual, y, n, nd, nh, nw, nullptr, stream);
+}
+
+int snvc_alias_deconv_tail_gather(const float *t, const float *bias, const float *residual, float *y, int64_t n, int64_t nd, int64_t nh,
+                                  int64_t nw, const snvc_wedge_desc *res_alias, void *stream) {
+    return tail_gather(t, bias, residual, y, n, nd, nh, nw, res_alias, stream);
+}
+
+}
diff --git a/snvc_amd/models/stereo_volume.py b/snvc_amd/models/stereo_volume.py
--- a/snvc_amd/models/stereo_volume.py
+++ b/snvc_amd/models/stereo_volume.py
@@ -127,6 +127,7 @@
     stream_out = False
     fused_first = True
     dedup_wedge = True
+    alias_wedge = True
     split_prep = True
     fused_tail = True
 
@@ -203,17 +204,24 @@
         hg = self.hg_conv3d
         _mark(timing, "conv2", 0)
         v2_out = self._buffer("v2s", (n, 2, 4, d, h, w, 8), dev, torch.float16)
+        alias = None
         if fused is not None:
+            if self._alias_route(st, n, (d, h, w), fused[2]):
+                alias = ops.wedge_desc(d, w, fused[2]["q"], fused[2]["m0"], fused[2]["off"])
             v2s, hv = L["conv2"].forward_fused_first(n=n, in_sp=(d, h, w), x_exp=E["v1"], scale=A["conv2"][0], bias=A["conv2"][1], flags=EPI_RELU,
                                                      out_exp=E["conv2"], head=self.classifier.weight, overflow=flag, out=v2_out,
-                                                     dedup=bool(self.dedup_wedge), **fused[2])
+                                                     dedup=bool(self.dedup_wedge), alias=alias is not None, **fused[2])
             _ROUTES["fused_first_conv"] += 1
+            _ROUTES["wedge_alias"] += alias is not None
         else:
             v2s, hv = L["conv2"](v1s, E["v1"], *A["conv2"], flags=EPI_RELU, out_exp=E["conv2"], head=self.classifier.weight, overflow=flag,
                                  out=v2_out)
         _mark(timing, "conv2", 1)
         _ROUTES["side_head"] += 1
-        o = L["h1"](v2s, E["conv2"], *A["h1"], flags=EPI_RELU, out_exp=E["h1"], overflow=flag)
+        if alias is not None:
+            o = L["h1"].forward_aliased(v2s, alias, E["conv2"], *A["h1"], flags=EPI_RELU, out_exp=E["h1"], overflow=flag)
+        else:
+            o = L["h1"](v2s, E["conv2"], *A["h1"], flags=EPI_RELU, out_exp=E["h1"], overflow=flag)
         pre = L["h2"](o, E["h1"], *A["h2"], flags=EPI_RELU, out_exp=E["h2"], overflow=flag)
         o = L["h3"](pre, E["h2"], *A["h3"], flags=EPI_RELU, out_exp=E["h3"], overflow=flag)
         o = L["h4"](o, E["h3"], *A["h4"], flags=EPI_RELU, out_exp=E["h4"], overflow=flag)
@@ -221,7 +229,7 @@
         if st["tail"] is not None and self.fused_tail:
             t = L["h5"].forward_tail(o, E["h4"], *A["h5"], st["tail"], residual=pre, res_exp=E["h2"], flags=EPI_RELU | ops.EPI_ADD_PRE,
                                      out_exp=E["post"], overflow=flag, out=self._buffer("tail_t", (n, 27, 8) + tuple(o.shape[3:6]), dev))
-            cost = ops.deconv_tail_gather(t, st["tail_bias"], hv)
+            cost = ops.deconv_tail_gather(t, st["tail_bias"], hv, res_alias=alias)
             _ROUTES["x3_fused_tail"] += 1
         else:
             post = L["h5"](o, E["h4"], *A["h5"], residual=pre, flags=EPI_RELU | ops.EPI_ADD_PRE, out_exp=E["h2"], to_f32=True)
@@ -230,6 +238,13 @@
         if self.overflow_check == "call" and st["guard"].wait():
             raise SplitOverflow()
         return cost
+
+    def _alias_route(self, st, n, sp, src) -> bool:
+        if not (self.alias_wedge and self.dedup_wedge and st["tail"] is not None and self.fused_tail):
+            return False
+        if not st["layers"]["h1"].aliased_form(n, sp):
+            return False
+        return ops.fused_first_wedge_dups(int(sp[0]), int(sp[2]), int(src["q"]), int(src["m0"]), int(src["off"])) > 0
 
     def _tail(self, v, hv=None):
         cost, _, _ = self.hg_conv3d(v, None, None, residual=v, head=self.classifier, head_residual=hv)
diff --git a/snvc_amd/ops.py b/snvc_amd/ops.py
--- a/snvc_amd/ops.py
+++ b/snvc_amd/ops.py
@@ -1,5 +1,6 @@
 import contextlib
 import ctypes
+import functools
 import math
 import threading
 import time
@@ -7,7 +8,7 @@
 
 import torch
 
-from . import _dedup, _derived, _fused, _lib
+from . import _alias, _dedup, _derived, _fused, _lib
 from ._lib import (EPI_ADD_POST, EPI_ADD_PRE, EPI_RELU, EPI_SIGMOID, EPI_STREAM_OUT, F32, F64, Conv3dDesc,
                    Unsupported, check)
 
@@ -1436,6 +1437,11 @@
     return hi - lo + 1, -lo
 
 
+@functools.lru_cache(maxsize=64)
+def fused_first_wedge_dups(d: int, w: int, q: int, m0: int, off: int) -> int:
+    return fused_first_wedge_tiles(d, w, q, m0, off)[0]
+
+
 def fused_first_wedge_tiles(d: int, w: int, q: int, m0: int, off: int):
     desc = _lib.Conv3dDesc()
     desc.Din, desc.Win = int(d), int(w)
@@ -1445,6 +1451,17 @@
     if dups < 0:
         raise ValueError(_lib.lib().snvc_last_error_string().decode())
     return dups, list(first), list(last)
+
+
+def wedge_desc(d: int, w: int, q: int, m0: int, off: int) -> "_alias.WedgeDesc":
+    return _alias.WedgeDesc(int(d), int(w), int(q), int(m0), int(off))
+
+
+def wedge_alias_depth(desc: "_alias.WedgeDesc", d: int, w: int) -> int:
+    got = int(_alias.lib().snvc_alias_depth(ctypes.byref(desc), int(d), int(w)))
+    if got < 0:
+        raise ValueError(_lib.lib().snvc_last_error_string().decode())
+    return got
 
 
 def sheared_prep_x3_il(right, q: int, wu: int, off: int, wu_col: int, off_col: int, lay_g: "Conv2dLayerX3", lay_col: "Conv2dLayerX3", ws: dict,
@@ -1665,9 +1682,15 @@
         return (self.ksize == 3 and self.stride == 1 and not self.transposed and self.w_mul_dev is None and self.cin % 8 == 0
                 and x3_form(self.cout, 3, 1, self.dilation, False, n, tuple(sp), True, False, self.forced_algo) == _lib.ALGO_X3_Q16)
 
+    def aliased_form(self, n: int, sp) -> bool:
+        sp = tuple(int(v) for v in sp)
+        return (self.ksize == 3 and self.stride == 2 and not self.transposed and self.w_mul_dev is None
+                and x3_form(self.cout, self.ksize, self.stride, self.dilation, self.transposed, n, self.out_spatial(sp), True, True,
+                            self.forced_algo) == _lib.ALGO_X3_Q16)
+
     def forward_fused_first(self, gi, pitch: int, lp: int, p_il, v_scale, v_bias, q: int, m0: int, off: int, off_col: int, v_flags: int,
                             n: int, in_sp, x_exp: int = 0, scale=None, bias=None, flags: int = 0, out=None, out_exp: int = 0, head=None,
-                            overflow=None, dedup: bool = False):
+                            overflow=None, dedup: bool = False, alias: bool = False, head_out=None):
         in_sp = tuple(int(v) for v in in_sp)
         if not self.fused_first_form(n, in_sp):
             raise Unsupported("forward_fused_first: the layer does not run on the 16x16x32 form at this size")
@@ -1679,18 +1702,37 @@
         y_head = None
         if head is not None:
             head = head.detach().reshape(-1).float().contiguous()
-            y_head = torch.empty((n, 1) + out_sp, dtype=torch.float32, device=gi.device)
+            y_head = _result(head_out, (n, 1) + out_sp, torch.float32, gi.device, "`head_out` must be a contiguous float32 [N,1,D,H,W] tensor")
         sc, bi = self.folded(scale, bias, x_exp, out_exp)
         if n == 0:
             return (out, y_head) if head is not None else out
         d = self._desc(n, in_sp, flags, algo, 0, _batch_stride(out), 0)
-        entry = (_dedup.lib().snvc_dedup_fused_first_conv3d_forward if dedup else _fused.lib().snvc_fused_first_conv3d_forward)
+        name = ("snvc_alias_fused_first_conv3d_forward" if alias else "snvc_dedup_fused_first_conv3d_forward" if dedup
+                else "snvc_fused_first_conv3d_forward")
+        entry = getattr((_alias if alias else _dedup if dedup else _fused).lib(), name)
         with torch.cuda.device(gi.device):
             check(entry(ctypes.byref(d), _ptr(packed), _ptr(sc), _ptr(bi), _ptr(out), _lo_ptr(out), _ptr(head), _ptr(y_head),
                         float(2.0 ** -out_exp), _ptr(overflow), _ptr(gi), int(pitch), int(lp), _ptr(p_il), _ptr(v_scale), _ptr(v_bias), int(q),
-                        int(m0), int(off), int(off_col), int(v_flags), _stream(gi)),
-                  "snvc_dedup_fused_first_conv3d_forward" if dedup else "snvc_fused_first_conv3d_forward")
+                        int(m0), int(off), int(off_col), int(v_flags), _stream(gi)), name)
         return (out, y_head) if head is not None else out
+
+    def forward_aliased(self, x, in_alias: "_alias.WedgeDesc", x_exp: int = 0, scale=None, bias=None, flags: int = 0, out=None,
+                        out_exp: int = 0, overflow=None):
+        _split_check(x, "x")
+        if x.size(2) * 8 != self.cin:
+            raise RuntimeError(f"conv3d input must have {self.cin} channels (split C8), got {x.size(2) * 8}")
+        n, in_sp, out_sp, algo, packed = self._launch(x, plain=True, split_out=True)
+        out = _result(out, (n, 2, self.cout // 8) + out_sp + (8,), torch.float16, x.device,
+                      "conv3d `out` must be a split C8 tensor of the output shape", _split_check)
+        sc, bi = self.folded(scale, bias, x_exp, out_exp)
+        if n == 0:
+            return out
+        d = self._desc(n, in_sp, flags, algo, _batch_stride(x), _batch_stride(out), 0)
+        with torch.cuda.device(x.device):
+            check(_alias.lib().snvc_alias_f16x3_conv3d_forward(ctypes.byref(d), _ptr(x), _lo_ptr(x), _ptr(packed), _ptr(sc), _ptr(bi), _ptr(out),
+                                                               _lo_ptr(out), _ptr(overflow), ctypes.byref(in_alias), _stream(x)),
+                  "snvc_alias_f16x3_conv3d_forward")
+        return out
 
     def forward_f32(self, x, x_mul_dev, residual_f32: Optional[torch.Tensor] = None, relu: bool = False):
         _split_check(x, "x")
@@ -1777,7 +1819,8 @@
                   "snvc_f16x3_tail_pack_weights")
 
 
-def deconv_tail_gather(t: torch.Tensor, bias: Optional[torch.Tensor] = None, residual: Optional[torch.Tensor] = None, out=None):
+def deconv_tail_gather(t: torch.Tensor, bias: Optional[torch.Tensor] = None, residual: Optional[torch.Tensor] = None, out=None,
+                       res_alias: Optional["_alias.WedgeDesc"] = None):
     _gpu(t, "t")
     if t.dtype != torch.float32 or t.dim() != 6 or t.size(1) != 27 or t.size(2) != 8 or not t.is_contiguous():
         raise RuntimeError("t must be a contiguous float32 [N, 27, 8, nd, nh, nw] tensor")
@@ -1796,8 +1839,12 @@
     if bias is not None:
         bias = bias.detach().reshape(-1)[:1].float().contiguous()
     with torch.cuda.device(t.device):
-        check(_lib.lib().snvc_deconv_tail_gather(_ptr(t), _ptr(bias), _ptr(residual), _ptr(out), n, nd, nh, nw, _stream(t)),
-              "snvc_deconv_tail_gather")
+        if res_alias is not None:
+            check(_alias.lib().snvc_alias_deconv_tail_gather(_ptr(t), _ptr(bias), _ptr(residual), _ptr(out), n, nd, nh, nw,
+                                                             ctypes.byref(res_alias), _stream(t)), "snvc_alias_deconv_tail_gather")
+        else:
+            check(_lib.lib().snvc_deconv_tail_gather(_ptr(t), _ptr(bias), _ptr(residual), _ptr(out), n, nd, nh, nw, _stream(t)),
+                  "snvc_deconv_tail_gather")
     return out
 
 
```

Result: faster. 554.5 (median of 6 runs) (+1.8%).
